# Jing-yilin/GAN-FFN

Hardware: AMD Instinct MI355X
Metric: utterances/sec per GAN train step, IEMOCAP tri-modal (higher is better)
Workload: dtype f32; 1 GPU; IEMOCAP tri-modal batch=32 per GPU fp32 on 1xMI355X, full G+D step (12 sub-steps: 6 train_disc + 6 train_gen, train-mode dropout, BCE, Adam); dialogues_per_gpu=32, seq_len=94, parallelism=dp1, launch=eager, streams=3, rccl_ranks=0, communicators=0

## Files before the change

gan_ffn_amd/_lib.py:

```python
import ctypes as C
import os

_HERE = os.path.dirname(os.path.abspath(__file__))
LIB_PATH = os.environ.get("GANFFN_LIB") or os.path.join(_HERE, "lib", "libganffn.so")


class EncCfg(C.Structure):
    _fields_ = [("S", C.c_int32), ("B", C.c_int32), ("E", C.c_int32), ("H", C.c_int32), ("F", C.c_int32),
                ("L", C.c_int32), ("p_pe", C.c_float), ("p_enc", C.c_float), ("ln_eps", C.c_float),
                ("train", C.c_int32)]


class LstmCfg(C.Structure):
    _fields_ = [("S", C.c_int32), ("B", C.c_int32), ("In", C.c_int32), ("H", C.c_int32)]


class LstmStackCfg(C.Structure):
    _fields_ = [("S", C.c_int32), ("B", C.c_int32), ("In", C.c_int32), ("H", C.c_int32), ("L", C.c_int32), ("p", C.c_float),
                ("train", C.c_int32)]


class HeadCfg(C.Structure):
    _fields_ = [("T", C.c_int32), ("E", C.c_int32), ("D1", C.c_int32), ("D2", C.c_int32), ("kind", C.c_int32),
                ("p", C.c_float), ("train", C.c_int32)]
# ... 45 lines not shown
SIGNATURES = {
    "ganffn_version": (_I, []),
    "ganffn_last_error": (C.c_char_p, []),
    "ganffn_layer_param_count": (_L, [_I, _I]),
    "ganffn_layer_param_offsets": (_I, [_I, _I, C.POINTER(C.c_int64)]),
    "ganffn_encoder_saved_floats": (_L, [_PE]),
    "ganffn_encoder_saved_hidden_offset": (_L, [_PE, _I]),
    "ganffn_encoder_workspace_floats": (_L, [_PE]),
    "ganffn_head_saved_floats": (_L, [_PH]),
    "ganffn_head_workspace_floats": (_L, [_PH]),
    "ganffn_rng_advance": (_I, [_P, _U64, _P]),
    "ganffn_pe_table": (_I, [_P, _I, _I, _P]),
    "ganffn_encoder_fwd": (_I, [_PE, _P, _P, _P, _P, _P, _P, _P, _U64, _P]),
    "ganffn_encoder_fwd_pair_supported": (_I, [_PE]),
    "ganffn_encoder_fwd_pair_workspace_floats": (_L, [_PE]),
    "ganffn_encoder_fwd_pair": (_I, [_PE, _P, _P, _P, _P, _P, _P, _P, _P, _U64, _P]),
    "ganffn_encoder_bwd": (_I, [_PE, _I, _I, _P, _P, _P, _P, _P, _P, _U64, _P]),
    "ganffn_encoder_bwd2": (_I, [_PE, _I, _I, _P, _P, _P, _P, _P, _P, _U64, _I, _P]),
    "ganffn_head_fwd": (_I, [_PH, _P, _P, _P, _P, _P, _P, _P, _P, _P, _P, _P, _U64, _P]),
    "ganffn_head_bwd": (_I, [_PH, _P, _P, _P, _P, _P, _P, _P, _P, _P, _P, _P, _P, _P, _P, _P, _U64, _P]),
    "ganffn_linear_fwd": (_I, [_P, _P, _P, _P, _I, _I, _I, _P]),
    "ganffn_linear_bwd_workspace_floats": (_L, [_I, _I, _I]),
    "ganffn_linear_bwd": (_I, [_P, _P, _P, _P, _P, _P, _I, _I, _I, _P, _L, _P]),
    "ganffn_bce_fwd": (_I, [_P, _F, _I, _F, _P, _I, _P]),
    "ganffn_bce_bwd": (_I, [_P, _F, _I, _F, _P, _P]),
    "ganffn_bce2_fwd": (_I, [_P, _F, _F, _I, _I, _I, _F, _P, _I, _P]),
    "ganffn_bce2_bwd": (_I, [_P, _F, _F, _I, _I, _I, _F, _P, _P]),
    "ganffn_adam_step": (_I, [_P, _P, _P, _P, _P, _L, _F, _F, _F, _F, _F, _F, _P]),
    "ganffn_lstm_saved_floats": (_L, [C.POINTER(LstmCfg)]),
    "ganffn_lstm_workspace_floats": (_L, [C.POINTER(LstmCfg)]),
    "ganffn_lstm_layer_fwd": (_I, [C.POINTER(LstmCfg), _P, _P, _P, _P, _P, _P, _P, _P, _P]),
    "ganffn_lstm_layer_bwd": (_I, [C.POINTER(LstmCfg), _P, _P, _P, _P, _P, _P, _P, _P, _P, _P, _P, _P, _P]),
    "ganffn_lstm_stack_saved_floats": (_L, [C.POINTER(LstmStackCfg)]),
    "ganffn_lstm_stack_workspace_floats": (_L, [C.POINTER(LstmStackCfg)]),
    "ganffn_lstm_stack_fwd": (_I, [C.POINTER(LstmStackCfg)] + [_P] * 9 + [_U64, _P]),
    "ganffn_lstm_stack_bwd": (_I, [C.POINTER(LstmStackCfg)] + [_P] * 13 + [_U64, _P]),
    "ganffn_lstm_batch_saved_floats": (_L, [C.POINTER(LstmCfg)]),
    "ganffn_lstm_batch_workspace_floats": (_L, [C.POINTER(LstmCfg)]),
    "ganffn_lstm_batch_layer_fwd": (_I, [C.POINTER(LstmCfg), _P, _P, _P, _P, _P, _P, _P, _P, _P]),
    "ganffn_lstm_batch_layer_bwd": (_I, [C.POINTER(LstmCfg), _P, _P, _P, _P, _P, _P, _P, _P, _P, _P, _P, _P, _P]),
    "ganffn_lstm_stack_batch_saved_floats": (_L, [C.POINTER(LstmStackCfg)]),
    "ganffn_lstm_stack_batch_workspace_floats": (_L, [C.POINTER(LstmStackCfg)]),
    "ganffn_lstm_stack_batch_fwd": (_I, [C.POINTER(LstmStackCfg)] + [_P] * 9 + [_U64, _P]),
    "ganffn_lstm_stack_batch_bwd": (_I, [C.POINTER(LstmStackCfg)] + [_P] * 13 + [_U64, _P]),
    "ganffn_meld_head_fwd": (_I, [_P, _P, _P, _P, _P, _P, _I, _I, _I, _P]),
    "ganffn_meld_head_bwd": (_I, [_P, _P, _P, _P, _P, _P, _P, _P, _P, _I, _I, _I, _P]),
    "ganffn_zero_floats": (_I, [_P, _L, _P]),
    "ganffn_adam_step_parts": (_I, [_P, _P, _P, _P, _P, _L, _F, _F, _F, _F, _F, _F, _P, _L, _I, _L, _L, _L, _P]),
    "ganffn_encoder_bwd_parts_supported": (_I, [_PE]),
    "ganffn_encoder_bwd_parts_covered": (_L, [_I, _I]),
    "ganffn_encoder_bwd_parts": (_I, [_PE, _P, _P, _P, _P, _P, _P, _U64, _I, C.POINTER(C.c_int64), C.POINTER(C.c_int64), C.POINTER(C.c_int), _P]),
    "ganffn_adam_update": (_I, [_P, _P, _P, _P, _P, _L, _F, _F, _F, _F, _F, _F, _P]),
    "ganffn_adam_bump": (_I, [_P, _P]),
    "ganffn_add3": (_I, [_P, _P, _P, _P, _L, _P]),
    "ganffn_logsoftmax_nll": (_I, [_P, _P, _P, _P, _P, _P, _P, _P, _I, _I, _I, _P]),
    "ganffn_gemm_nt": (_I, [_P, _P, _P, _P, _I, _I, _I, _P]),
    "ganffn_gemm_nn": (_I, [_P, _P, _P, _I, _I, _I, _P]),
    "ganffn_gemm_tn_acc": (_I, [_P, _P, _P, _P, _I, _I, _I, _P]),
    "ganffn_ffn_linear1_fwd": (_I, [_P, _P, _P, _P, _I, _I, _I, _F, _U32, _P, _U64, _I, _P]),
    "ganffn_gemm_tn_grouped_workspace_floats": (_L, []),
    "ganffn_gemm_tn_grouped": (_I, [_I, _P, _P, _P, _P, _P, _P, _P, _P, _L, _P]),
    "ganffn_attention_fwd": (_I, [_P, _P, _P, _I, _I, _I, _I, _F, _U32, _P, _U64, _P]),
    "ganffn_attention_bwd": (_I, [_P, _P, _P, _P, _P, _I, _I, _I, _I, _F, _U32, _P, _U64, _P]),
    "ganffn_gemm_hook": (_I, [_I, _I, _P, _P, _P, _P, _P, _L, _I, _I, _I, _F, _U32, _P, _U64, _I, _I, _P, _P]),
    "ganffn_ffn_k100_hook": (_I, [_I, _P, _P, _P, _P, _P, _P, _I, _F, _U32, _P, _U64, _I, _P]),
    "ganffn_attention_keep_words": (_L, [_I, _I]),
    "ganffn_attention_fwd_keep": (_I, [_P, _P, _P, _P, _I, _I, _I, _I, _F, _U32, _P, _U64, _P]),
    "ganffn_attention_bwd_keep": (_I, [_P, _P, _P, _P, _P, _P, _I, _I, _I, _I, _F, _U32, _P, _U64, _P]),
    "ganffn_add_dropout_layernorm_fwd": (_I, [_P, _P, _P, _P, _P, _P, _P, _I, _I, _F, _F, _U32, _P, _U64, _P]),
    "ganffn_add_dropout_layernorm_bwd": (_I, [_P, _P, _P, _P, _P, _P, _P, _P, _I, _I, _F, _U32, _P, _U64, _P]),
    "ganffn_general2_attention_fwd": (_I, [_P, _P, _P, _P, _P, _P, _I, _I, _I, _P]),
    "ganffn_general2_attention_bwd": (_I, [_P, _P, _P, _P, _P, _P, _P, _P, _P, _I, _I, _I, _P]),
    "ganffn_gemm_n100": (_I, [_P, _P, _I, _P, _P, _L, _I, _I, _I, C.POINTER(C.c_int), _P]),
    "ganffn_debug_set_ffn_mode": (_I, [_I]),
    "ganffn_drnn_skinny": (_I, [_I, _I, _P, _P, _P, _I, _I, _I, _P]),
    "ganffn_drnn_skinny_batch": (_I, [_I, _I, _P, _P, _P, _I, _I, _I, _P]),
    "ganffn_drnn_saved_floats": (_L, [C.POINTER(DrnnCfg)]),
    "ganffn_drnn_workspace_floats": (_L, [C.POINTER(DrnnCfg)]),
    "ganffn_drnn_fwd": (_I, [C.POINTER(DrnnCfg), _I, _P, _P, _P, _P, _P, _P, _P, _P, _P, _U64, _P]),
    "ganffn_drnn_bwd": (_I, [C.POINTER(DrnnCfg), _I, _P, _P, _P, _P, _P, _P, _P, _P, _P, _P, _P, _U64, _P]),
    "ganffn_drnn_listener_saved_floats": (_L, [C.POINTER(DrnnCfg)]),
    "ganffn_drnn_listener_workspace_floats": (_L, [C.POINTER(DrnnCfg)]),
    "ganffn_drnn_listener_fwd": (_I, [C.POINTER(DrnnCfg), _I, _P, _P, _P, _P, _P, _P, _P, _P, _P, _P, _U64, _P]),
    "ganffn_drnn_listener_bwd": (_I, [C.POINTER(DrnnCfg), _I, _P, _P, _P, _P, _P, _P, _P, _P, _P, _P, _P, _P, _P, _U64, _P]),
    "ganffn_drnn_att_saved_floats": (_L, [C.POINTER(DrnnCfg), C.POINTER(DrnnAtt), _I]),
    "ganffn_drnn_att_workspace_floats": (_L, [C.POINTER(DrnnCfg), C.POINTER(DrnnAtt), _I]),
    "ganffn_drnn_att_fwd": (_I, [C.POINTER(DrnnCfg), C.POINTER(DrnnAtt), _I] + [_P] * 11 + [_U64, _P]),
    "ganffn_drnn_att_bwd": (_I, [C.POINTER(DrnnCfg), C.POINTER(DrnnAtt), _I] + [_P] * 15 + [_U64, _P]),
    "ganffn_drnn_party_saved_floats": (_L, [C.POINTER(DrnnCfg), C.POINTER(DrnnAtt), _I, _I]),
    "ganffn_drnn_party_workspace_floats": (_L, [C.POINTER(DrnnCfg), C.POINTER(DrnnAtt), _I, _I]),
    "ganffn_drnn_party_fwd": (_I, [C.POINTER(DrnnCfg), C.POINTER(DrnnAtt), _I, _I] + [_P] * 11 + [_U64, _P]),
    "ganffn_drnn_party_bwd": (_I, [C.POINTER(DrnnCfg), C.POINTER(DrnnAtt), _I, _I] + [_P] * 15 + [_U64, _P]),
    "ganffn_drnn_batch_saved_floats": (_L, [C.POINTER(DrnnCfg), C.POINTER(DrnnAtt), _I, _I]),
    "ganffn_drnn_batch_workspace_floats": (_L, [C.POINTER(DrnnCfg), C.POINTER(DrnnAtt), _I, _I]),
    "ganffn_drnn_batch_fwd": (_I, [C.POINTER(DrnnCfg), C.POINTER(DrnnAtt), _I, _I] + [_P] * 11 + [_U64, _P]),
    "ganffn_drnn_batch_bwd": (_I, [C.POINTER(DrnnCfg), C.POINTER(DrnnAtt), _I, _I] + [_P] * 15 + [_U64, _P]),
    "ganffn_dropout": (_I, [_P, _P, _I, _I, _F, _U32, _P, _U64, _P]),
    "ganffn_seq_reverse": (_I, [_P, _P, _P, _I, _I, _I, _I, _P]),
    "ganffn_drnn_join_fwd": (_I, [_P, _P, _P, _P, _I, _I, _I, _F, _U32, _U32, _P, _U64, _I, _P]),
    "ganffn_drnn_join_bwd": (_I, [_P, _P, _P, _P, _I, _I, _I, _F, _U32, _U32, _P, _U64, _I, _P]),
    "ganffn_mask_pos_inplace": (_I, [_P, _P, _F, _L, _P]),
    "ganffn_batch_gather": (_I, [_P, _I, _P, _P, _L, _P, _P, _P, _I, _I, _I, _P]),
    "ganffn_epoch_record": (_I, [_P, _P, _P, _P, _I, _I, _I, _P, _P, _P, _L, _L, _P, _P, _I, _I, _P]),
}

_lib = None
# ... 35 lines not shown
```

gan_ffn_amd/csrc/api.hip:

```cpp
#include "common.h"

#include <string.h>

namespace ganffn {

static thread_local char g_err[512] = "";
char* err_buf() { return g_err; }
int fail(int code, const char* fmt, ...) {
    va_list ap;
    va_start(ap, fmt);
    vsnprintf(g_err, sizeof(g_err), fmt, ap);
    va_end(ap);
    return code;
}

int launch_gelu_bwd_drop(const float* d, const float* u, float* out, int R, int C, float p, uint32_t site,
                         const uint64_t* rng, uint64_t add, int train, hipStream_t st);
int launch_disc_tail_fwd(const float* a2, const float* w3, const float* b3, float* prob, int T, int D2, float p,
                         const uint64_t* rng, uint64_t add, int train, hipStream_t st);
int launch_disc_tail_bwd(const float* dprob, const float* prob, const float* a2, const float* u2, const float* w3,
                         float* d_pre2, float* gw3, float* gb3, int T, int D2, float p, const uint64_t* rng, uint64_t add,
                         int train, hipStream_t st, float* gpart);
int launch_disc_tail_reduce(const float* gpart, int nblk_, int D2, float* gw3, float* gb3, hipStream_t st);
bool disc_head_fused_supported(int E, int D1, int D2);
// ... 304 lines not shown
            ea.bias = P + lo.out_b;
            int osplits = md.outproj_nosplit() ? 1 : gemm_splitk_factor(T, E, E);
            const GemmSeg1 g1{s1v + so.attn_o, tmp1, nullptr, train};
            GF_TRY(launch_gemm_nt_pair(sv0 + so.attn_o, E, P + lo.out_w, E, tmp0, E, T, E, E, EPI_NONE, ea, g1, st, &osplits, TE));
            const LnFwdSeg1 n1{X1, tmp1, s1v + so.x1, s1v + so.xhat1, s1v + so.rstd1, train};
            GF_TRY(launch_add_drop_ln_fwd(X0, tmp0, P + lo.n1w, P + lo.n1b, sv0 + so.x1, sv0 + so.xhat1, sv0 + so.rstd1, T, E, c->ln_eps,
                                          c->p_enc, site + 1, rng, add, 0, st, osplits, TE, &n1));
        }
        int splits = 1;
        {
            EpiArgs e1;
            e1.bias = P + lo.b1; e1.p = c->p_enc; e1.site = site + 2; e1.rng = rng; e1.rng_add = add; e1.train = 0;
            const GemmSeg1 g1{s1v + so.x1, s1v + so.h, reinterpret_cast<uint16_t*>(s1v + so.hmask), train};
            GF_TRY(launch_gemm_nt_pair(sv0 + so.x1, E, P + lo.w1, E, sv0 + so.h, F, T, F, E, EPI_RELU_DROP, e1, g1, st));
            if (n100_supported(E, F) && !md.n100_off()) {
                splits = MAX_SPLITS;
                GF_TRY(launch_gemm_n100(sv0 + so.h, F, P + lo.w2, F, 0, P + lo.b2, tmp0, TE, T, F, &splits, st, s1v + so.h, tmp1));
            } else {
                ea.bias = P + lo.b2;
                splits = gemm_splitk_factor(T, E, F);
                const GemmSeg1 g2{s1v + so.h, tmp1, nullptr, train};
                GF_TRY(launch_gemm_nt_pair(sv0 + so.h, F, P + lo.w2, F, tmp0, E, T, E, F, EPI_NONE, ea, g2, st, &splits, TE));
            }
        }
        if (rc) {
            const float* Pn = (l + 1 < L) ? P + lo.total : nullptr;
            RcFwdSeg1 s1{};
            s1.y = tmp1; s1.x = s1v + so.x1; s1.out = Xn1; s1.xhat = s1v + so.xhat2; s1.rstd = s1v + so.rstd2;
            s1.post_out = Pn ? sv1(l + 1) + so.qkv : nullptr; s1.train = train;
            GF_TRY(launch_rc_ln_inproj_fwd(tmp0, splits, TE, sv0 + so.x1, P + lo.n2w, P + lo.n2b, Xn0, sv0 + so.xhat2, sv0 + so.rstd2,
                                           Pn ? Pn + lo.in_w : nullptr, Pn ? Pn + lo.in_b : nullptr, Pn ? sv0 + so.qkv : nullptr, T,
                                           c->ln_eps, c->p_enc, site + 3, rng, add, 0, st, &s1));
        } else {
            const LnFwdSeg1 n2{s1v + so.x1, tmp1, Xn1, s1v + so.xhat2, s1v + so.rstd2, train};
            GF_TRY(launch_add_drop_ln_fwd(sv0 + so.x1, tmp0, P + lo.n2w, P + lo.n2b, Xn0, sv0 + so.xhat2, sv0 + so.rstd2, T, E, c->ln_eps,
                                          c->p_enc, site + 3, rng, add, 0, st, splits, TE, &n2));
        }
        X0 = Xn0;
        X1 = Xn1;
    }
    return 0;
}

extern "C" int ganffn_encoder_bwd2(const ganffn_enc_cfg* c, int layer_lo, int layer_hi, float* dx, const float* params,
                                   float* grads, const float* saved, float* workspace, const uint64_t* rng, uint64_t add,
                                   int need_dx_in, void* stream);
extern "C" int ganffn_encoder_bwd(const ganffn_enc_cfg* c, int layer_lo, int layer_hi, float* dx, const float* params,
                                  float* grads, const float* saved, float* workspace, const uint64_t* rng, uint64_t add,
                                  void* stream) {
    return ganffn_encoder_bwd2(c, layer_lo, layer_hi, dx, params, grads, saved, workspace, rng, add, 1, stream);
}
static int encoder_bwd_impl(const ganffn_enc_cfg* c, int layer_lo, int layer_hi, float* dx, const float* params,
                            float* grads, const float* saved, float* workspace, const uint64_t* rng, uint64_t add,
                            int need_dx_in, void* stream, TnSlabs* slabs);
extern "C" int ganffn_encoder_bwd2(const ganffn_enc_cfg* c, int layer_lo, int layer_hi, float* dx, const float* params,
                                   float* grads, const float* saved, float* workspace, const uint64_t* rng, uint64_t add,
                                   int need_dx_in, void* stream) {
    return encoder_bwd_impl(c, layer_lo, layer_hi, dx, params, grads, saved, workspace, rng, add, need_dx_in, stream, nullptr);
}
static bool bwd_parts_supported(const ganffn_enc_cfg* c, const Mode md) {
    return rc_supported(c->E) && !md.rc_off() && !md.tn100_off() && !md.tn100_in_kernel_sum() && !md.adam_slabs_off() && c->F == 2048 &&
           4 * c->L <= 40;
}
extern "C" int ganffn_encoder_bwd_parts_supported(const ganffn_enc_cfg* c) {
    if (check_cfg(c) != 0) return -1;
    return bwd_parts_supported(c, mode()) ? 1 : 0;
}
extern "C" int64_t ganffn_encoder_bwd_parts_covered(int E, int F) { return layer_off(E, F).n1w; }
extern "C" int ganffn_encoder_bwd_parts(const ganffn_enc_cfg* c, float* dx, const float* params, float* grads, const float* saved,
                                        float* workspace, const uint64_t* rng, uint64_t add, int need_dx_in, int64_t* part_offset,
                                        int64_t* part_stride, int* n_parts, void* stream) {
    GF_TRY(check_cfg(c));
    GF_CHECK_ARG(grads && part_offset && part_stride && n_parts, "encoder_bwd_parts: null pointer");
    GF_CHECK_ARG(bwd_parts_supported(c, mode()), "encoder_bwd_parts: this stack's weight gradients are reduced in the launch (ask ganffn_encoder_bwd_parts_supported)");
    TnSlabs sl{grads, (long)c->L * layer_off(c->E, c->F).total, 1, nullptr, 0};
    GF_TRY(encoder_bwd_impl(c, 0, c->L, dx, params, grads, saved, workspace, rng, add, need_dx_in, stream, &sl));
    *n_parts = sl.n_parts;
    *part_offset = sl.part ? sl.part - workspace : 0;
    *part_stride = sl.part_stride;
    return 0;
}
static int encoder_bwd_impl(const ganffn_enc_cfg* c, int layer_lo, int layer_hi, float* dx, const float* params,
                            float* grads, const float* saved, float* workspace, const uint64_t* rng, uint64_t add,
                            int need_dx_in, void* stream, TnSlabs* slabs) {
    const Mode md = mode();
    GF_TRY(check_cfg(c));
    GF_CHECK_ARG(dx && params && saved && workspace, "encoder_bwd: null pointer");
    GF_CHECK_ARG(0 <= layer_lo && layer_lo < layer_hi && layer_hi <= c->L, "encoder_bwd: bad layer range [%d,%d)", layer_lo, layer_hi);
    GF_CHECK_ARG(aligned16(dx) && aligned16(params) && aligned16(saved) && aligned16(workspace) && (!grads || aligned16(grads)),
                 "encoder_bwd: buffers must be 16-byte aligned");
    const bool drop = c->train && (c->p_pe > 0.f || c->p_enc > 0.f);
    GF_CHECK_ARG(!drop || rng, "encoder_bwd: rng required in train mode");
    hipStream_t st = (hipStream_t)stream;
    const int S = c->S, B = c->B, E = c->E, H = c->H, F = c->F, T = S * B;
    const int64_t TE = (int64_t)T * E, TF = (int64_t)T * F;
    const LayerOff lo = layer_off(E, F);
    const SavedOff so = saved_off(c);
    const int train = c->train;
    const float pdrop = (train ? c->p_enc : 0.f);

    const int64_t SET = TF + 5 * TE;
    float* set0 = workspace;
    float* dz2 = set0 + (int64_t)c->L * SET;
    float* dz1 = dz2 + TE;
    float* d_attn = dz1 + TE;
    float* tmp = d_attn + TE;
    float* lnp0 = tmp + (int64_t)MAX_SPLITS * TE;
    const int64_t LNP = ln_part_floats(c);
    float* tnp = lnp0 + (int64_t)c->L * 2 * LNP;
    tnp = reinterpret_cast<float*>((reinterpret_cast<uintptr_t>(tnp) + 15) & ~(uintptr_t)15);
    const bool rc = rc_supported(E) && !md.rc_off();
    float* rcw = reinterpret_cast<float*>((reinterpret_cast<uintptr_t>(tnp + gemm_tn_grouped_part_floats()) + 15) & ~(uintptr_t)15);
    const int64_t RCW = rc_pack_floats();
    if (rc) GF_TRY(launch_rc_pack(params + (int64_t)layer_lo * lo.total, lo.total, lo.in_w, lo.out_w, rcw, layer_hi - layer_lo, st));
    const int lnblk = rc ? rc_blocks(T) : ln_bwd_blocks(T);
    TnDesc tn[40];
    int ntn = 0;
    float* r_gw[2 * 64]; float* r_gb[2 * 64]; const float* r_part[2 * 64]; int r_nb[2 * 64];
    int nred = 0;

    const float* dxin = dx;
    int dxin_slabs = 1;
    for (int l = layer_hi - 1; l >= layer_lo; --l) {
        const float* P = params + (int64_t)l * lo.total;
        float* G = grads ? grads + (int64_t)l * lo.total : nullptr;
        const float* sv = saved + so.layers + (int64_t)l * so.per_layer;
        const float* Xl = saved + so.X + (int64_t)l * TE;
        const uint32_t site = SITE_LAYER0 + 4 * l;
        float* bs = set0 + (int64_t)(l - layer_lo) * SET;
        float* dh = bs;
        float* dyA = dh + TF;
        float* dyB = dyA + TE;
        float* d_qkv = dyB + TE;
        float* lnp2 = lnp0 + (int64_t)(2 * (l - layer_lo)) * LNP;
        float* lnp1 = lnp2 + LNP;
        EpiArgs none;
        if (rc) {
            if (l == layer_hi - 1)
                GF_TRY(launch_rc_ln_bwd(nullptr, nullptr, dx, 1, 0, nullptr, sv + so.xhat2, sv + so.rstd2, P + lo.n2w, dz2, dyA,
                                        G ? lnp2 : nullptr, nullptr, nullptr, T, c->p_enc, site + 3, rng, add, train, st));
            else
                GF_TRY(launch_rc_ln_bwd(bs + SET + TF + 2 * TE, rcw + (int64_t)(l + 1 - layer_lo) * RCW, nullptr, 0, 0, dz1,
                                        sv + so.xhat2, sv + so.rstd2, P + lo.n2w, dz2, dyA, G ? lnp2 : nullptr, nullptr, nullptr, T,
                                        c->p_enc, site + 3, rng, add, train, st));
        } else {
            GF_TRY(launch_add_drop_ln_bwd(dxin, sv + so.xhat2, sv + so.rstd2, P + lo.n2w, dz2, dyA, G ? G + lo.n2w : nullptr,
                                          G ? G + lo.n2b : nullptr, T, E, c->p_enc, site + 3, rng, add, train, st, dxin_slabs, TE,
                                          nullptr, G ? lnp2 : nullptr));
        }
        if (G) { r_gw[nred] = G + lo.n2w; r_gb[nred] = G + lo.n2b; r_part[nred] = lnp2; r_nb[nred] = lnblk; ++nred; }
        if (G) tn[ntn++] = TnDesc{dyA, E, sv + so.h, F, G + lo.w2, F, G + lo.b2, E, F, T};
        const float mscale = (pdrop > 0.f) ? 1.0f / (1.0f - pdrop) : 1.0f;
        int splits = 1;
        {
            EpiArgs em;
            em.aux_in = sv + so.h;
            em.mscale = mscale;
            if (!md.mask_float()) em.mask_in = reinterpret_cast<const uint16_t*>(sv + so.hmask);
            GF_TRY(launch_gemm_nn(dyA, E, P + lo.w2, F, dh, F, T, F, E, EPI_MASK_POS, em, st));
        }
        if (G) tn[ntn++] = TnDesc{dh, F, sv + so.x1, E, G + lo.w1, E, G + lo.b1, F, E, T};
        {
            if (n100_supported(E, F) && !md.n100_off()) {
                splits = MAX_SPLITS;
                GF_TRY(launch_gemm_n100(dh, F, P + lo.w1, E, 1, nullptr, tmp, TE, T, F, &splits, st));
            } else {
                splits = gemm_splitk_factor(T, E, F);
                GF_TRY(launch_gemm_nn(dh, F, P + lo.w1, E, tmp, E, T, E, F, EPI_NONE, none, st, &splits, TE));
            }
        }
        if (rc) {
            GF_TRY(launch_rc_ln_bwd(nullptr, nullptr, tmp, splits, TE, dz2, sv + so.xhat1, sv + so.rstd1, P + lo.n1w, dz1, dyB,
                                    G ? lnp1 : nullptr, rcw + (int64_t)(l - layer_lo) * RCW + 3 * (int64_t)E * E, d_attn, T, c->p_enc,
                                    site + 1, rng, add, train, st));
        } else {
            GF_TRY(launch_add_drop_ln_bwd(tmp, sv + so.xhat1, sv + so.rstd1, P + lo.n1w, dz1, dyB, G ? G + lo.n1w : nullptr,
                                          G ? G + lo.n1b : nullptr, T, E, c->p_enc, site + 1, rng, add, train, st, splits, TE, dz2,
                                          G ? lnp1 : nullptr));
        }
        if (G) { r_gw[nred] = G + lo.n1w; r_gb[nred] = G + lo.n1b; r_part[nred] = lnp1; r_nb[nred] = lnblk; ++nred; }
        if (G) tn[ntn++] = TnDesc{dyB, E, sv + so.attn_o, E, G + lo.out_w, E, G + lo.out_b, E, E, T};
        if (!rc) GF_TRY(launch_gemm_nn(dyB, E, P + lo.out_w, E, d_attn, E, T, E, E, EPI_NONE, none, st));
        GF_TRY(launch_attention_bwd(sv + so.qkv, sv + so.attn_o, sv + so.lse, d_attn, reinterpret_cast<const uint32_t*>(sv + so.keep), d_qkv, S, B, E,
                                    H, c->p_enc, site + 0, rng, add, train, st));
        if (G) tn[ntn++] = TnDesc{d_qkv, 3 * E, Xl, E, G + lo.in_w, E, G + lo.in_b, 3 * E, E, T};
        if (ntn == 40 || (l == layer_lo && ntn > 0)) {
            GF_TRY(launch_gemm_tn_grouped(tn, ntn, st, tnp, gemm_tn_grouped_part_floats(), slabs));
            ntn = 0;
        }
        EpiArgs eadd;
        eadd.aux_in = dz1;
        if (l > layer_lo && rc) {
        } else if (l > layer_lo) {
            int sp = inproj_dgrad_splits(T, E);
            GF_TRY(launch_gemm_nn(d_qkv, 3 * E, P + lo.in_w, E, tmp, E, T, E, 3 * E, EPI_NONE, eadd, st, &sp, TE));
            dxin = tmp;
            dxin_slabs = sp;
        } else if (layer_lo > 0 || need_dx_in) {
            GF_TRY(launch_gemm_nn(d_qkv, 3 * E, P + lo.in_w, E, dx, E, T, E, 3 * E, EPI_NONE, eadd, st));
        }
    }
    if (nred > 0) GF_TRY(launch_ln_param_reduce(nred, r_gw, r_gb, r_part, r_nb, E, st, slabs != nullptr));
    if (layer_lo == 0 && need_dx_in) GF_TRY(launch_dropout_bwd_inplace(dx, T, E, c->p_pe, SITE_PE, rng, add, train, st));
    return 0;
}

static int check_head(const ganffn_head_cfg* c) {
    GF_CHECK_ARG(c, "null head cfg");
    GF_CHECK_ARG(c->T >= 1 && c->E >= 4 && (c->E & 3) == 0, "head: bad T=%d E=%d", c->T, c->E);
    GF_CHECK_ARG(c->D1 >= 4 && (c->D1 & 3) == 0 && c->D2 >= 4 && (c->D2 & 3) == 0, "head: D1=%d D2=%d must be multiples of 4", c->D1, c->D2);
    GF_CHECK_ARG(c->kind == 0 || c->kind == 1, "head: kind=%d", c->kind);
    GF_CHECK_ARG(c->kind == 0 || c->D2 <= 32, "disc head: D2=%d > 32", c->D2);
    GF_CHECK_ARG(c->p >= 0.f && c->p < 1.f, "head: p out of [0,1)");
    return 0;
}
extern "C" int64_t ganffn_head_saved_floats(const ganffn_head_cfg* c) {
    if (check_head(c) != 0) return -1;
    const int64_t T = c->T, T4 = (T + 3) & ~int64_t(3);
    int64_t n = T * c->E + 2 * T * c->D1 + T * c->D2;
    if (c->kind == 1) n += T * c->D2 + T4;
    return n;
}
static int64_t head_part2(const ganffn_head_cfg* c) { return a4(gemm_tn_part_floats(c->D2, c->D1, c->T)); }
static int64_t head_part1(const ganffn_head_cfg* c) { return a4(gemm_tn_part_floats(c->D1, c->E, c->T)); }
extern "C" int64_t ganffn_head_workspace_floats(const ganffn_head_cfg* c) {
    if (check_head(c) != 0) return -1;
    const int64_t T = c->T;
    const int64_t tail_blocks = disc_head_blocks((int)T) > (T + 255) / 256 ? disc_head_blocks((int)T) : (T + 255) / 256;
    return a4(T * c->D1) + a4(T * c->D2) + head_part2(c) + head_part1(c) + tail_blocks * 36 + 64;
}

extern "C" int ganffn_head_fwd(const ganffn_head_cfg* c, const float* x, const float* w1, const float* b1, const float* w2,
                               const float* b2, const float* w3, const float* b3, float* out, float* saved, float* workspace,
                               const uint64_t* rng, uint64_t add, void* stream) {
    GF_TRY(check_head(c));
    const Mode md = mode();
    GF_CHECK_ARG(x && w1 && b1 && w2 && b2 && out && saved, "head_fwd: null pointer");
    GF_CHECK_ARG(c->kind == 0 || (w3 && b3), "head_fwd: disc needs fc3");
    GF_CHECK_ARG(!(c->train && c->p > 0.f) || rng, "head_fwd: rng required in train mode");
    hipStream_t st = (hipStream_t)stream;
    const int T = c->T, E = c->E, D1 = c->D1, D2 = c->D2, train = c->train;
    float* s0 = saved;
    float* u1 = s0 + (int64_t)T * E;
    float* a1 = u1 + (int64_t)T * D1;
    float* u2 = a1 + (int64_t)T * D1;
    EpiArgs e;
    e.p = c->p; e.rng = rng; e.rng_add = add; e.train = train;
    if (c->kind == 0) {
        GF_TRY(launch_gelu_drop_fwd(x, s0, T, E, c->p, SITE_HEAD0, rng, add, train, st));
        e.bias = b1; e.site = SITE_HEAD1; e.aux_out = u1;
        GF_TRY(launch_gemm_nt(s0, E, w1, E, a1, D1, T, D1, E, EPI_DROP_GELU, e, st));
        e.bias = b2; e.site = SITE_HEAD2; e.aux_out = u2;
        GF_TRY(launch_gemm_nt(a1, D1, w2, D1, out, D2, T, D2, D1, EPI_DROP_GELU, e, st));
    } else if (disc_head_fused_supported(E, D1, D2) && !md.dhead_off()) {
        float* a2 = u2 + (int64_t)T * D2;
        float* prob = a2 + (int64_t)T * D2;
        GF_TRY(launch_disc_head_fwd(x, w1, b1, w2, b2, w3, b3, s0, u1, a1, u2, a2, prob, out, T, c->p, rng, add, train, st));
    } else {
        float* a2 = u2 + (int64_t)T * D2;
        float* prob = a2 + (int64_t)T * D2;
        GF_TRY(launch_gelu_drop_fwd(x, s0, T, E, 0.f, SITE_HEAD0, rng, add, 0, st));
        e.bias = b1; e.site = SITE_HEAD1; e.aux_out = u1;
        GF_TRY(launch_gemm_nt(s0, E, w1, E, a1, D1, T, D1, E, EPI_DROP_GELU, e, st));
        e.bias = b2; e.site = SITE_HEAD2; e.aux_out = u2;
        GF_TRY(launch_gemm_nt(a1, D1, w2, D1, a2, D2, T, D2, D1, EPI_DROP_GELU, e, st));
        GF_TRY(launch_disc_tail_fwd(a2, w3, b3, prob, T, D2, c->p, rng, add, train, st));
        hipError_t er = hipMemcpyAsync(out, prob, (size_t)T * sizeof(float), hipMemcpyDeviceToDevice, st);
        if (er != hipSuccess) return fail((int)er, "head_fwd: memcpy failed");
    }
    (void)workspace;
    return 0;
}

extern "C" int ganffn_head_bwd(const ganffn_head_cfg* c, const float* d_out, const float* x, const float* w1, const float* w2,
                               const float* w3, float* gw1, float* gb1, float* gw2, float* gb2, float* gw3, float* gb3,
                               float* dx, const float* saved, float* workspace, const uint64_t* rng, uint64_t add,
                               void* stream) {
    GF_TRY(check_head(c));
    const Mode md = mode();
    GF_CHECK_ARG(d_out && x && w1 && w2 && dx && saved && workspace, "head_bwd: null pointer");
    GF_CHECK_ARG(aligned16(workspace), "head_bwd: workspace must be 16-byte aligned");
    GF_CHECK_ARG(c->kind == 0 || w3, "head_bwd: disc needs fc3");
    GF_CHECK_ARG(!(c->train && c->p > 0.f) || rng, "head_bwd: rng required in train mode");
    hipStream_t st = (hipStream_t)stream;
    const int T = c->T, E = c->E, D1 = c->D1, D2 = c->D2, train = c->train;
    const float* s0 = saved;
    const float* u1 = s0 + (int64_t)T * E;
    const float* a1 = u1 + (int64_t)T * D1;
    const float* u2 = a1 + (int64_t)T * D1;
    float* d_pre1 = workspace;
    float* d_pre2 = d_pre1 + a4((int64_t)T * D1);
    float* part2 = d_pre2 + a4((int64_t)T * D2);
    float* part1 = part2 + head_part2(c);
    float* tailp = part1 + head_part1(c);
    if (c->kind == 1 && disc_head_fused_supported(E, D1, D2) && !md.dhead_off()) {
        const float* a2 = u2 + (int64_t)T * D2;
        const float* prob = a2 + (int64_t)T * D2;
        GF_TRY(launch_disc_head_bwd(d_out, x, w1, w2, w3, u1, u2, a2, prob, dx, gw1 ? d_pre1 : nullptr, gw2 ? d_pre2 : nullptr,
                                    gw3 ? tailp : nullptr, T, c->p, rng, add, train, st));
        if (gw3) GF_TRY(launch_disc_tail_reduce(tailp, disc_head_blocks(T), D2, gw3, gb3, st));
        if (gw2) GF_TRY(launch_gemm_tn_acc(d_pre2, D2, a1, D1, gw2, D1, gb2, D2, D1, T, st, part2, head_part2(c)));
        if (gw1) GF_TRY(launch_gemm_tn_acc(d_pre1, D1, s0, E, gw1, E, gb1, D1, E, T, st, part1, head_part1(c)));
        return 0;
    }
    if (c->kind == 0) {
        GF_TRY(launch_gelu_bwd_drop(d_out, u2, d_pre2, T, D2, c->p, SITE_HEAD2, rng, add, train, st));
    } else {
        const float* a2 = u2 + (int64_t)T * D2;
        const float* prob = a2 + (int64_t)T * D2;
        GF_TRY(launch_disc_tail_bwd(d_out, prob, a2, u2, w3, d_pre2, gw3, gb3, T, D2, c->p, rng, add, train, st, tailp));
    }
    if (gw2) GF_TRY(launch_gemm_tn_acc(d_pre2, D2, a1, D1, gw2, D1, gb2, D2, D1, T, st, part2, head_part2(c)));
    EpiArgs e;
    e.p = c->p; e.rng = rng; e.rng_add = add; e.train = train;
    e.aux_in = u1; e.site = SITE_HEAD1;
    GF_TRY(launch_gemm_nn(d_pre2, D2, w2, D1, d_pre1, D1, T, D1, D2, EPI_GELU_BWD_DROP, e, st));
    if (gw1) GF_TRY(launch_gemm_tn_acc(d_pre1, D1, s0, E, gw1, E, gb1, D1, E, T, st, part1, head_part1(c)));
    e.aux_in = x;
    if (c->kind == 0) {
        e.site = SITE_HEAD0;
        GF_TRY(launch_gemm_nn(d_pre1, D1, w1, E, dx, E, T, E, D1, EPI_GELU_BWD_DROP, e, st));
    } else {
        GF_TRY(launch_gemm_nn(d_pre1, D1, w1, E, dx, E, T, E, D1, EPI_GELU_BWD, e, st));
    }
    return 0;
}
// ... 138 lines not shown
```

gan_ffn_amd/csrc/common.h:

```cpp
#pragma once
#include <hip/hip_runtime.h>
#include <stdint.h>
#include <stdio.h>
#include <stdarg.h>
#include <atomic>

#include "../../include/ganffn.h"

#ifdef GANFFN_LAB
#define GF_LAB_ONLY(...) __VA_ARGS__
#else
#define GF_LAB_ONLY(...)
#endif

namespace ganffn {

struct Mode {
    uint32_t bits;
    bool rc_off() const { return bits & 2u; }
    bool n100_off() const { return bits & 4u; }
    bool tn100_off() const { return bits & 8u; }
    bool tn100_in_kernel_sum() const { return bits & 16u; }
    bool dhead_off() const { return bits & 32u; }
    bool pe_off() const { return bits & 64u; }
// ... 148 lines not shown
}

__device__ __forceinline__ float gelu_f(float x) {
    return 0.5f * x * (1.0f + erff(x * 0.70710678118654752440f));
}
__device__ __forceinline__ float gelu_grad_f(float x) {
    const float cdf = 0.5f * (1.0f + erff(x * 0.70710678118654752440f));
    const float pdf = 0.39894228040143267794f * __expf(-0.5f * x * x);
    return cdf + x * pdf;
}

__device__ __forceinline__ float wave_sum(float v) {
#pragma unroll
    for (int o = 32; o > 0; o >>= 1) v += __shfl_xor(v, o, 64);
    return v;
}
__device__ __forceinline__ float wave_max(float v) {
#pragma unroll
    for (int o = 32; o > 0; o >>= 1) v = fmaxf(v, __shfl_xor(v, o, 64));
    return v;
}

enum Epilogue : int {
    EPI_NONE = 0,
    EPI_RELU_DROP = 1,
    EPI_DROP_GELU = 2,
    EPI_MASK_POS = 3,
    EPI_GELU_BWD_DROP = 4,
    EPI_GELU_BWD = 5,
    EPI_GELU_BWD_DROP0 = 6
};

struct EpiArgs {
    const float* bias = nullptr;
    float* aux_out = nullptr;
    const float* aux_in = nullptr;
    float mscale = 1.f;
    uint16_t* mask_out = nullptr;
    const uint16_t* mask_in = nullptr;
    float p = 0.f;
    uint32_t site = 0;
    const uint64_t* rng = nullptr;
    uint64_t rng_add = 0;
    int train = 0;
};

inline long epi_mask_words(long M, long N) { return ((M + 31) / 32) * N * 2; }

int launch_gemm_nt(const float* A, int lda, const float* W, int ldw, float* C, int ldc, int M, int N, int K,
                   int epi, const EpiArgs& ea, hipStream_t st, int* splits_io = nullptr, long slab_stride = 0);
int gemm_splitk_factor(int M, int N, int K);
struct GemmSeg1 {
    const float* A; float* C; uint16_t* mask_out; int train;
};
int launch_gemm_nt_pair(const float* A, int lda, const float* W, int ldw, float* C, int ldc, int M, int N, int K, int epi,
                        const EpiArgs& ea, const GemmSeg1& s1, hipStream_t st, int* splits_io = nullptr, long slab_stride = 0);
int launch_gemm_nn(const float* A, int lda, const float* Bm, int ldb, float* C, int ldc, int M, int N, int K,
                   int epi, const EpiArgs& ea, hipStream_t st, int* splits_io = nullptr, long slab_stride = 0);
long gemm_tn_part_floats(int M, int N, int K);
int launch_gemm_tn_acc(const float* At, int lda, const float* Bm, int ldb, float* C, int ldc, float* colsum,
                       int M, int N, int K, hipStream_t st, float* part_ws = nullptr, long part_floats = 0);

struct SkinnyProb {
    const float* A; int lda;
    const float* W; int ldw;
    const float* Cin; int ldcin;
    const float* Cin2;
    const float* bias;
    float* C; int ldc;
    int M, N, K;
};
struct SkinnyGroup {
    SkinnyProb p[8];
};
int launch_skinny(const SkinnyGroup& grp, int nprob, bool nn, hipStream_t st);

struct TnDesc {
    const float* At; int lda;
    const float* B; int ldb;
    float* C; int ldc;
    float* colsum;
    int M, N, K;
};
struct TnSlabs {
    float* grad_base; long range_floats;
    int n_parts; float* part; long part_stride;
};
int launch_gemm_tn_grouped(const TnDesc* d, int n, hipStream_t st, float* part_ws = nullptr, long part_floats = 0, TnSlabs* slabs = nullptr);
bool tn100_supported(const TnDesc* d, int n);
int launch_gemm_tn100_grouped(const TnDesc* d, int n, hipStream_t st, float* part_ws, long part_floats, TnSlabs* slabs = nullptr);
long gemm_tn_grouped_part_floats();

constexpr int ATTN_KEEP_WORDS = 28 * 16;
struct AttnFwdSeg1 {
    const float* qkv; float* o; float* lse; uint32_t* keep; int train;
};
int launch_attention_fwd(const float* qkv, float* o, float* lse, uint32_t* keep, int S, int B, int E, int H, float p, uint32_t site,
                         const uint64_t* rng, uint64_t add, int train, hipStream_t st, const AttnFwdSeg1* seg1 = nullptr);
int launch_attention_bwd(const float* qkv, const float* o, const float* lse, const float* d_o, const uint32_t* keep, float* d_qkv,
                         int S, int B, int E, int H, float p, uint32_t site, const uint64_t* rng, uint64_t add, int train,
                         hipStream_t st);
bool attn16_supported(int E, int H, int S);
int launch_attn16_fwd(const float* qkv, float* o, float* lse, uint32_t* keepw, int S, int B, int E, int H, float p, uint32_t site,
                      const uint64_t* rng, uint64_t add, int train, hipStream_t st, const AttnFwdSeg1* seg1 = nullptr);
int launch_attn16_bwd(const float* qkv, const float* o, const float* lse, const float* d_o, const uint32_t* keepw, float* d_qkv,
                      int S, int B, int E, int H, float p, uint32_t site, const uint64_t* rng, uint64_t add, int train,
                      hipStream_t st);

int launch_pe_dropout(const float* x, const float* pe, float* out, int S, int B, int E, float p,
                      const uint64_t* rng, uint64_t add, int train, hipStream_t st, float* out1 = nullptr, int train1 = 0);
int launch_dropout_bwd_inplace(float* dx, int R, int C, float p, uint32_t site, const uint64_t* rng, uint64_t add,
                               int train, hipStream_t st);
int launch_dropout(const float* x, float* out, int R, int C, float p, uint32_t site, const uint64_t* rng,
                   uint64_t add, int train, hipStream_t st);
struct LnFwdSeg1 {
    const float* x; const float* y; float* out; float* xhat; float* rstd; int train;
};
int launch_add_drop_ln_fwd(const float* x, const float* y, const float* w, const float* b, float* out, float* xhat,
                           float* rstd, int T, int E, float eps, float p, uint32_t site, const uint64_t* rng,
                           uint64_t add, int train, hipStream_t st, int nslab = 1, long slab_stride = 0,
                           const LnFwdSeg1* s1 = nullptr);
int ln_bwd_blocks(int T);
int launch_add_drop_ln_bwd(const float* d_out, const float* xhat, const float* rstd, const float* w, float* dz,
                           float* dy, float* gw, float* gb, int T, int E, float p, uint32_t site,
                           const uint64_t* rng, uint64_t add, int train, hipStream_t st, int nslab = 1,
                           long slab_stride = 0, const float* addend = nullptr, float* gpart = nullptr);
int launch_ln_param_reduce(int n, float* const* gw, float* const* gb, const float* const* part, const int* nblk, int E,
                           hipStream_t st, bool overwrite = false);
int launch_add_inplace(float* a, const float* b, int64_t n, hipStream_t st);

bool n100_supported(int N, int K);
int n100_splits(int T, int K, int max_splits, int w_kmajor);
int launch_gemm_n100(const float* A, int lda, const float* W, int ldw, int w_kmajor, const float* bias, float* C, long slab_stride,
                     int T, int K, int* splits_io, hipStream_t st, const float* A1 = nullptr, float* C1 = nullptr);

bool rc_supported(int E);
long rc_pack_floats();
int rc_blocks(int T);
int launch_rc_pack(const float* params, long layer_stride, long off_in, long off_out, float* wt, int nl, hipStream_t st);
struct RcFwdSeg1 {
    const float* pre_a; const float* y; const float* x;
    float* out; float* xhat; float* rstd; float* post_out;
    int train;
};
int launch_rc_outproj_ln_fwd(const float* attn_o, const float* wo, const float* bo, const float* x, const float* gamma,
                             const float* beta, float* out, float* xhat, float* rstd, int T, float eps, float p, uint32_t site,
                             const uint64_t* rng, uint64_t add, int train, hipStream_t st, const RcFwdSeg1* s1 = nullptr);
int launch_rc_pe_inproj_fwd(const float* x_in, const float* pe, float* out, const float* w_in, const float* b_in, float* qkv, int T,
                            int B, float p, const uint64_t* rng, uint64_t add, int train, hipStream_t st,
                            const RcFwdSeg1* s1 = nullptr);
int launch_rc_ln_inproj_fwd(const float* y, int nslab, long slab_stride, const float* x, const float* gamma, const float* beta,
                            float* out, float* xhat, float* rstd, const float* w_in, const float* b_in, float* qkv, int T,
                            float eps, float p, uint32_t site, const uint64_t* rng, uint64_t add, int train, hipStream_t st,
                            const RcFwdSeg1* s1 = nullptr);
int launch_rc_ln_bwd(const float* d_qkv, const float* w_in_t, const float* d_out, int nslab, long slab_stride, const float* addend,
                     const float* xhat, const float* rstd, const float* gamma, float* dz, float* dy, float* gpart,
                     const float* wo_t, float* d_attn, int T, float p, uint32_t site, const uint64_t* rng, uint64_t add, int train,
                     hipStream_t st);
int launch_gelu_drop_fwd(const float* x, float* out, int R, int C, float p, uint32_t site, const uint64_t* rng,
                         uint64_t add, int train, hipStream_t st);

}
```

gan_ffn_amd/csrc/elementwise.hip:

```cpp
#include "common.h"

#pragma clang fp contract(off)

namespace ganffn {

template <bool PAIR>
__global__ void pe_dropout_kernel(const float* __restrict__ x, const float* __restrict__ pe, float* __restrict__ out,
                                  int T, int B, int E, float p, const uint64_t* __restrict__ rng, uint64_t add,
                                  int train, float* out1, int train1, int nb0) {
    const int G = (T + 3) >> 2;
    int bid = blockIdx.x;
    if constexpr (PAIR) {
        if (bid >= nb0) {
            bid -= nb0;
            out = out1; train = train1;
        }
    }
    const long idx = (long)bid * blockDim.x + threadIdx.x;
    if (idx >= (long)G * E) return;
    const int rg = (int)(idx / E), c = (int)(idx - (long)rg * E);
    const DropCtx dc = make_drop(rng, add, SITE_PE, p, train);
    float mult[4];
    drop_mult4(dc, (uint32_t)rg, (uint32_t)E, (uint32_t)c, mult);
#pragma unroll
    for (int q = 0; q < 4; ++q) {
        const int t = rg * 4 + q;
        if (t < T) {
            const int s = t / B;
            out[(size_t)t * E + c] = (x[(size_t)t * E + c] + pe[(size_t)s * E + c]) * mult[q];
        }
    }
}

template <int MODE>
__global__ void drop_kernel(const float* __restrict__ x, const float* __restrict__ u, float* __restrict__ out, int R,
                            int C, float p, uint32_t site, const uint64_t* __restrict__ rng, uint64_t add, int train) {
    const int G = (R + 3) >> 2;
    const long idx = (long)blockIdx.x * blockDim.x + threadIdx.x;
    if (idx >= (long)G * C) return;
    const int rg = (int)(idx / C), c = (int)(idx - (long)rg * C);
    const DropCtx dc = make_drop(rng, add, site, p, train);
    float mult[4];
    drop_mult4(dc, (uint32_t)rg, (uint32_t)C, (uint32_t)c, mult);
#pragma unroll
    for (int q = 0; q < 4; ++q) {
        const int t = rg * 4 + q;
        if (t < R) {
            const size_t o = (size_t)t * C + c;
            float v = x[o];
            if (MODE == 1) v = gelu_f(v);
            if (MODE == 2) v = v * gelu_grad_f(u[o]);
            out[o] = v * mult[q];
        }
    }
}

__global__ void add_inplace_kernel(float* __restrict__ a, const float* __restrict__ b, long n4) {
    const long i = (long)blockIdx.x * blockDim.x + threadIdx.x;
    if (i >= n4) return;
    float4 x = reinterpret_cast<float4*>(a)[i];
    const float4 y = reinterpret_cast<const float4*>(b)[i];
    x.x += y.x; x.y += y.y; x.z += y.z; x.w += y.w;
    reinterpret_cast<float4*>(a)[i] = x;
}

__global__ void add3_kernel(const float* __restrict__ a, const float* __restrict__ b, const float* __restrict__ c,
                            float* __restrict__ o, long n) {
    const long i = (long)blockIdx.x * blockDim.x + threadIdx.x;
    if (i < n) o[i] = a[i] + b[i] + c[i];
}

constexpr int LN_MAXC = 10;
constexpr int LN_MAXSLAB = 16;

template <int NC, int NSB, bool PAIR = false>
__global__ __launch_bounds__(256) void add_drop_ln_fwd_kernel(const float* __restrict__ x, const float* __restrict__ y,
                                                              const float* __restrict__ w, const float* __restrict__ b,
                                                              float* __restrict__ out, float* __restrict__ xhat,
                                                              float* __restrict__ rstd, int T, int E, float eps, float p,
                                                              uint32_t site, const uint64_t* __restrict__ rng,
                                                              uint64_t add, int train, int nslab, long slab_stride, LnFwdSeg1 s1,
                                                              int nb0) {
    const int lane = threadIdx.x & 63;
    int bid = blockIdx.x;
    if constexpr (PAIR) {
        if (bid >= nb0) {
            bid -= nb0;
            x = s1.x; y = s1.y; out = s1.out; xhat = s1.xhat; rstd = s1.rstd; train = s1.train;
        }
    }
    const int rg = bid * 4 + (threadIdx.x >> 6);
    if (rg * 4 >= T) return;
    const DropCtx dc = make_drop(rng, add, site, p, train);
    size_t off[NC][4];
    bool okc[NC], okr[4];
#pragma unroll
    for (int q = 0; q < 4; ++q) okr[q] = rg * 4 + q < T;
#pragma unroll
    for (int k = 0; k < NC; ++k) {
        const int c = lane + 64 * k;
        okc[k] = c < E;
#pragma unroll
        for (int q = 0; q < 4; ++q) off[k][q] = (size_t)min(rg * 4 + q, T - 1) * E + min(c, E - 1);
    }
    float xv[NC][4], yy[NC][4];
#pragma unroll
    for (int k = 0; k < NC; ++k)
// ... 249 lines not shown
            a = a2[o];
            d_pre2[o] = dpre3 * w3[k] * gelu_grad_f(u2[o]) * drop_mult1(d2, (uint32_t)t, (uint32_t)D2, (uint32_t)k);
        }
        if (gw3) {
            const float s = wave_sum(dpre3 * a);
            if (lane == 0) red[wv][k] = s;
        }
    }
    if (gw3) {
        const float s = wave_sum(dpre3);
        if (lane == 0) red[wv][32] = s;
        __syncthreads();
        if (threadIdx.x < D2) gpart[blockIdx.x * 36 + threadIdx.x] = red[0][threadIdx.x] + red[1][threadIdx.x] + red[2][threadIdx.x] + red[3][threadIdx.x];
        if (threadIdx.x == 32) gpart[blockIdx.x * 36 + 32] = red[0][32] + red[1][32] + red[2][32] + red[3][32];
    }
}
__global__ __launch_bounds__(1024) void disc_tail_reduce_kernel(const float* __restrict__ gpart, int nblk, int D2, float* __restrict__ gw3,
                                                                float* __restrict__ gb3) {
    const int lane = threadIdx.x & 63, w = threadIdx.x >> 6;
    for (int k = w; k <= D2; k += 16) {
        const int slot = k < D2 ? k : 32;
        float s = 0.f;
        for (int b = lane; b < nblk; b += 64) s += gpart[b * 36 + slot];
        s = wave_sum(s);
        if (lane == 0) {
            if (k < D2) gw3[k] += s; else gb3[0] += s;
        }
    }
}

__global__ __launch_bounds__(1024) void bce_fwd_kernel(const float* __restrict__ prob, float target_a, float target_b,
                                                       int period, int split, int n, float scale, float* __restrict__ loss,
                                                       int accumulate) {
    __shared__ float red[16];
    float s = 0.f;
    for (int i = threadIdx.x; i < n; i += 1024) {
        const float target = (period > 0 && (i % period) >= split) ? target_b : target_a;
        const float p = prob[i];
        const float lp = fmaxf(logf(p), -100.f);
        const float l1p = fmaxf(logf(1.0f - p), -100.f);
        s -= target * lp + (1.0f - target) * l1p;
    }
    s = wave_sum(s);
    if ((threadIdx.x & 63) == 0) red[threadIdx.x >> 6] = s;
    __syncthreads();
    if (threadIdx.x == 0) {
        float t = 0.f;
        for (int w = 0; w < 16; ++w) t += red[w];
        t = t * scale / (float)n;
        loss[0] = accumulate ? loss[0] + t : t;
    }
}

__global__ void bce_bwd_kernel(const float* __restrict__ prob, float target_a, float target_b, int period, int split, int n,
                               float scale, float* __restrict__ dprob) {
    const int i = blockIdx.x * blockDim.x + threadIdx.x;
    if (i >= n) return;
    const float target = (period > 0 && (i % period) >= split) ? target_b : target_a;
    const float p = prob[i];
    dprob[i] = scale / (float)n * (p - target) / fmaxf(p * (1.0f - p), 1e-12f);
}

__device__ __forceinline__ void adam_one(float& pi, float gi, float& mi, float& vi, float lr_bc1, float rs_bc2, float b1,
                                         float b2, float eps, float wd, float gscale) {
    gi *= gscale;
    if (wd != 0.f) gi += wd * pi;
    mi = b1 * mi + (1.0f - b1) * gi;
    vi = b2 * vi + (1.0f - b2) * gi * gi;
    const float denom = sqrtf(vi) / rs_bc2 + eps;
    pi = pi - lr_bc1 * (mi / denom);
}

constexpr int ADAM_MAX_EXTRA = 7;
template <int VEC>
__global__ __launch_bounds__(256) void adam_kernel(float* __restrict__ p, const float* __restrict__ g, float* __restrict__ m,
                                                   float* __restrict__ v, const int32_t* __restrict__ step, long n, float lr,
                                                   float b1, float b2, float eps, float wd, float gscale) {
    const long i = ((long)blockIdx.x * blockDim.x + threadIdx.x) * VEC;
    if (i >= n) return;
    const float t = (float)(*step + 1);
    const float bc1 = 1.0f - powf(b1, t);
    const float bc2 = 1.0f - powf(b2, t);
    const float lr_bc1 = lr / bc1, rs_bc2 = sqrtf(bc2);
    if (VEC == 4) {
        float4 pp = *reinterpret_cast<float4*>(p + i), mm = *reinterpret_cast<float4*>(m + i), vv = *reinterpret_cast<float4*>(v + i);
        const float4 gg = *reinterpret_cast<const float4*>(g + i);
        adam_one(pp.x, gg.x, mm.x, vv.x, lr_bc1, rs_bc2, b1, b2, eps, wd, gscale);
        adam_one(pp.y, gg.y, mm.y, vv.y, lr_bc1, rs_bc2, b1, b2, eps, wd, gscale);
        adam_one(pp.z, gg.z, mm.z, vv.z, lr_bc1, rs_bc2, b1, b2, eps, wd, gscale);
        adam_one(pp.w, gg.w, mm.w, vv.w, lr_bc1, rs_bc2, b1, b2, eps, wd, gscale);
        *reinterpret_cast<float4*>(m + i) = mm;
        *reinterpret_cast<float4*>(v + i) = vv;
        *reinterpret_cast<float4*>(p + i) = pp;
    } else {
        float pi = p[i], mi = m[i], vi = v[i];
        adam_one(pi, g[i], mi, vi, lr_bc1, rs_bc2, b1, b2, eps, wd, gscale);
        m[i] = mi; v[i] = vi; p[i] = pi;
    }
}
__global__ __launch_bounds__(256) void adam_parts_kernel(float* __restrict__ p, const float* __restrict__ g, float* __restrict__ m,
                                                         float* __restrict__ v, const int32_t* __restrict__ step, long n, float lr,
                                                         float b1, float b2, float eps, float wd, float gscale,
                                                         const float* __restrict__ part, long part_stride, int n_extra,
                                                         long enc_floats, long layer_floats, long covered) {
    const long i = ((long)blockIdx.x * blockDim.x + threadIdx.x) * 4;
    if (i >= n) return;
    const float t = (float)(*step + 1);
    const float bc1 = 1.0f - powf(b1, t);
    const float bc2 = 1.0f - powf(b2, t);
    const float lr_bc1 = lr / bc1, rs_bc2 = sqrtf(bc2);
    float4 pp = *reinterpret_cast<float4*>(p + i), mm = *reinterpret_cast<float4*>(m + i), vv = *reinterpret_cast<float4*>(v + i);
    float4 gg = *reinterpret_cast<const float4*>(g + i);
    const bool cov = i < enc_floats && (i % layer_floats) < covered;
    if (cov) {
        float4 e[ADAM_MAX_EXTRA];
#pragma unroll
        for (int z = 0; z < ADAM_MAX_EXTRA; ++z) e[z] = *reinterpret_cast<const float4*>(part + (size_t)min(z, n_extra - 1) * part_stride + i);
#pragma unroll
        for (int z = 0; z < ADAM_MAX_EXTRA; ++z)
            if (z < n_extra) { gg.x += e[z].x; gg.y += e[z].y; gg.z += e[z].z; gg.w += e[z].w; }
    }
    adam_one(pp.x, gg.x, mm.x, vv.x, lr_bc1, rs_bc2, b1, b2, eps, wd, gscale);
    adam_one(pp.y, gg.y, mm.y, vv.y, lr_bc1, rs_bc2, b1, b2, eps, wd, gscale);
    adam_one(pp.z, gg.z, mm.z, vv.z, lr_bc1, rs_bc2, b1, b2, eps, wd, gscale);
    adam_one(pp.w, gg.w, mm.w, vv.w, lr_bc1, rs_bc2, b1, b2, eps, wd, gscale);
    *reinterpret_cast<float4*>(m + i) = mm;
    *reinterpret_cast<float4*>(v + i) = vv;
    *reinterpret_cast<float4*>(p + i) = pp;
}
__global__ void adam_step_inc(int32_t* step) { *step += 1; }

__global__ void rng_advance_kernel(uint64_t* rng, uint64_t delta) { rng[1] += delta; }

__global__ void pe_table_kernel(float* __restrict__ pe, int max_len, int E) {
    const int idx = blockIdx.x * blockDim.x + threadIdx.x;
    if (idx >= max_len * (E / 2)) return;
    const int pos = idx / (E / 2), i = idx % (E / 2);
    const float c = (float)(-9.210340371976184 / (double)E);
    const float div = expf((float)(2 * i) * c);
    const float a = (float)pos * div;
    pe[(size_t)pos * E + 2 * i] = sinf(a);
    pe[(size_t)pos * E + 2 * i + 1] = cosf(a);
}

__global__ __launch_bounds__(1024) void logsoftmax_nll_kernel(const float* __restrict__ logits, const int64_t* __restrict__ labels,
                                                              const float* __restrict__ umask, const float* __restrict__ cw,
                                                              float* __restrict__ logp, float* __restrict__ acc2, int S, int B,
                                                              int C) {
    __shared__ float red[2][16];
    float num = 0.f, den = 0.f;
    for (int t = threadIdx.x; t < S * B; t += 1024) {
        const int s = t / B, b = t - s * B;
        const float* x = logits + (size_t)t * C;
        float m = x[0];
        for (int c = 1; c < C; ++c) m = fmaxf(m, x[c]);
        float sum = 0.f;
        for (int c = 0; c < C; ++c) sum += expf(x[c] - m);
        const float ls = logf(sum);
        for (int c = 0; c < C; ++c) logp[(size_t)t * C + c] = (x[c] - m) - ls;
        if (labels) {
// ... 69 lines not shown
            a[u] = dy[(size_t)t * N + n];
            b[u] = x[(size_t)t * K + kc];
        }
#pragma unroll
        for (int u = 0; u < 8; ++u) {
            const float m = (t0 + 16 * u < T) ? 1.f : 0.f;
            acc += m * a[u] * b[u];
            accb += m * a[u];
        }
    }
    red[g][kl] = acc;
    if (kl == 0) red[g][64] = accb;
    __syncthreads();
    if (g == 0) {
        float sw = 0.f;
#pragma unroll
        for (int i = 0; i < 16; ++i) sw += red[i][kl];
        if (k < K) gw[(size_t)n * K + k] += sw;
        if (gb && kl == 0 && blockIdx.y == 0) {
            float sb = 0.f;
#pragma unroll
            for (int i = 0; i < 16; ++i) sb += red[i][64];
            gb[n] += sb;
        }
    }
}

static inline int nblk(long n, int bs) { return (int)((n + bs - 1) / bs); }

int launch_pe_dropout(const float* x, const float* pe, float* out, int S, int B, int E, float p,
                      const uint64_t* rng, uint64_t add, int train, hipStream_t st, float* out1, int train1) {
    const int T = S * B;
    const long n = (long)((T + 3) / 4) * E;
    const int nb = nblk(n, 256);
    if (out1) hipLaunchKernelGGL(pe_dropout_kernel<true>, dim3(2 * nb), dim3(256), 0, st, x, pe, out, T, B, E, p, rng, add, train, out1, train1, nb);
    else hipLaunchKernelGGL(pe_dropout_kernel<false>, dim3(nb), dim3(256), 0, st, x, pe, out, T, B, E, p, rng, add, train, (float*)nullptr, 0, 0);
    GF_LAUNCH_CHECK();
    return 0;
}

int launch_dropout(const float* x, float* out, int R, int C, float p, uint32_t site, const uint64_t* rng,
                   uint64_t add, int train, hipStream_t st) {
    const long n = (long)((R + 3) / 4) * C;
    hipLaunchKernelGGL(drop_kernel<0>, dim3(nblk(n, 256)), dim3(256), 0, st, x, (const float*)nullptr, out, R, C, p, site, rng, add, train);
    GF_LAUNCH_CHECK();
    return 0;
}
int launch_dropout_bwd_inplace(float* dx, int R, int C, float p, uint32_t site, const uint64_t* rng, uint64_t add,
                               int train, hipStream_t st) {
    if (!(train && p > 0.f)) return 0;
    return launch_dropout(dx, dx, R, C, p, site, rng, add, train, st);
}
int launch_gelu_drop_fwd(const float* x, float* out, int R, int C, float p, uint32_t site, const uint64_t* rng,
                         uint64_t add, int train, hipStream_t st) {
    const long n = (long)((R + 3) / 4) * C;
    hipLaunchKernelGGL(drop_kernel<1>, dim3(nblk(n, 256)), dim3(256), 0, st, x, (const float*)nullptr, out, R, C, p, site, rng, add, train);
    GF_LAUNCH_CHECK();
    return 0;
}
int launch_gelu_bwd_drop(const float* d, const float* u, float* out, int R, int C, float p, uint32_t site,
                         const uint64_t* rng, uint64_t add, int train, hipStream_t st) {
    const long n = (long)((R + 3) / 4) * C;
    hipLaunchKernelGGL(drop_kernel<2>, dim3(nblk(n, 256)), dim3(256), 0, st, d, u, out, R, C, p, site, rng, add, train);
    GF_LAUNCH_CHECK();
    return 0;
}

int launch_add_inplace(float* a, const float* b, int64_t n, hipStream_t st) {
    GF_CHECK_ARG((n & 3) == 0 && aligned16(a) && aligned16(b), "add_inplace: n %% 4 and 16-byte alignment required");
    hipLaunchKernelGGL(add_inplace_kernel, dim3(nblk(n / 4, 256)), dim3(256), 0, st, a, b, (long)(n / 4));
    GF_LAUNCH_CHECK();
    return 0;
}

int launch_add_drop_ln_fwd(const float* x, const float* y, const float* w, const float* b, float* out, float* xhat,
                           float* rstd, int T, int E, float eps, float p, uint32_t site, const uint64_t* rng,
                           uint64_t add, int train, hipStream_t st, int nslab, long slab_stride, const LnFwdSeg1* s1) {
    GF_CHECK_ARG(E <= 64 * LN_MAXC, "layernorm: E=%d > %d", E, 64 * LN_MAXC);
    GF_CHECK_ARG(nslab >= 1 && nslab <= LN_MAXSLAB, "layernorm: nslab=%d out of [1,%d]", nslab, LN_MAXSLAB);
    GF_CHECK_ARG(!s1 || (s1->x && s1->y && s1->out), "layernorm: bad second segment");
    const int G = (T + 3) / 4;
    const dim3 grid((G + 3) / 4), grid2(2 * ((G + 3) / 4)), blk(256);
#define GF_LN_FWD(NC, NSB)                                                                                              \
    do {                                                                                                                \
        if (s1) hipLaunchKernelGGL((add_drop_ln_fwd_kernel<NC, NSB, true>), grid2, blk, 0, st, x, y, w, b, out, xhat, rstd, T, E, eps, \
                                   p, site, rng, add, train, nslab, slab_stride, *s1, (int)grid.x);                      \
        else hipLaunchKernelGGL((add_drop_ln_fwd_kernel<NC, NSB>), grid, blk, 0, st, x, y, w, b, out, xhat, rstd, T, E, eps, p, \
                                site, rng, add, train, nslab, slab_stride, LnFwdSeg1{}, 0);                              \
    } while (0)
    if (E <= 64) GF_LN_FWD(1, 8);
    else if (E <= 128) GF_LN_FWD(2, 8);
    else if (E <= 256) GF_LN_FWD(4, 4);
    else if (E <= 320) GF_LN_FWD(5, 4);
    else if (E <= 512) GF_LN_FWD(8, 2);
    else GF_LN_FWD(10, 2);
#undef GF_LN_FWD
    GF_LAUNCH_CHECK();
    return 0;
}

int ln_bwd_blocks(int T) {
    int blocks = ((T + 3) / 4 + 3) / 4;
    return blocks > 256 ? 256 : blocks;
}

int launch_add_drop_ln_bwd(const float* d_out, const float* xhat, const float* rstd, const float* w, float* dz,
                           float* dy, float* gw, float* gb, int T, int E, float p, uint32_t site,
                           const uint64_t* rng, uint64_t add, int train, hipStream_t st, int nslab, long slab_stride,
// ... 74 lines not shown
    }
    if (gw) {
        hipLaunchKernelGGL(small_linear_dw_kernel, dim3(N, (K + 63) / 64), dim3(1024), 0, st, dy, x, gw, gb, T, K, N);
        GF_LAUNCH_CHECK();
    }
    return 0;
}

}

using namespace ganffn;

extern "C" int ganffn_rng_advance(uint64_t* rng, uint64_t delta, void* stream) {
    GF_CHECK_ARG(rng, "rng_advance: null rng");
    hipLaunchKernelGGL(rng_advance_kernel, dim3(1), dim3(1), 0, (hipStream_t)stream, rng, delta);
    GF_LAUNCH_CHECK();
    return 0;
}

extern "C" int ganffn_pe_table(float* pe, int max_len, int E, void* stream) {
    GF_CHECK_ARG(pe && max_len > 0 && E > 0 && (E & 1) == 0, "pe_table: E must be even (model.py:1187-1188)");
    const int n = max_len * (E / 2);
    hipLaunchKernelGGL(pe_table_kernel, dim3((n + 255) / 256), dim3(256), 0, (hipStream_t)stream, pe, max_len, E);
    GF_LAUNCH_CHECK();
    return 0;
}

extern "C" int ganffn_bce_fwd(const float* prob, float target, int n, float scale, float* loss_out, int accumulate,
                              void* stream) {
    return ganffn_bce2_fwd(prob, target, target, 0, 0, n, scale, loss_out, accumulate, stream);
}
extern "C" int ganffn_bce_bwd(const float* prob, float target, int n, float scale, float* dprob, void* stream) {
    return ganffn_bce2_bwd(prob, target, target, 0, 0, n, scale, dprob, stream);
}

extern "C" int ganffn_bce2_fwd(const float* prob, float target_a, float target_b, int period, int split, int n, float scale,
                               float* loss_out, int accumulate, void* stream) {
    GF_CHECK_ARG(prob && loss_out && n > 0 && period >= 0 && split >= 0, "bce_fwd: bad arguments");
    hipStream_t st = (hipStream_t)stream;
    hipLaunchKernelGGL(bce_fwd_kernel, dim3(1), dim3(1024), 0, st, prob, target_a, target_b, period, split, n, scale, loss_out,
                       accumulate);
    GF_LAUNCH_CHECK();
    return 0;
}

extern "C" int ganffn_bce2_bwd(const float* prob, float target_a, float target_b, int period, int split, int n, float scale,
                               float* dprob, void* stream) {
    GF_CHECK_ARG(prob && dprob && n > 0 && period >= 0 && split >= 0, "bce_bwd: bad arguments");
    hipLaunchKernelGGL(bce_bwd_kernel, dim3((n + 255) / 256), dim3(256), 0, (hipStream_t)stream, prob, target_a, target_b, period, split, n, scale, dprob);
    GF_LAUNCH_CHECK();
    return 0;
}

extern "C" int ganffn_adam_bump(int32_t* step, void* stream) {
    GF_CHECK_ARG(step, "adam_bump: null step");
    hipLaunchKernelGGL(adam_step_inc, dim3(1), dim3(1), 0, (hipStream_t)stream, step);
    GF_LAUNCH_CHECK();
    return 0;
}

extern "C" int ganffn_adam_step(float* params, const float* grads, float* exp_avg, float* exp_avg_sq, int32_t* step,
                                int64_t n, float lr, float beta1, float beta2, float eps, float weight_decay,
                                float grad_scale, void* stream) {
    GF_TRY(ganffn_adam_update(params, grads, exp_avg, exp_avg_sq, step, n, lr, beta1, beta2, eps, weight_decay, grad_scale, stream));
    return ganffn_adam_bump(step, stream);
}

extern "C" int ganffn_adam_update(float* params, const float* grads, float* exp_avg, float* exp_avg_sq, const int32_t* step,
                                  int64_t n, float lr, float beta1, float beta2, float eps, float weight_decay,
                                  float grad_scale, void* stream) {
    GF_CHECK_ARG(params && grads && exp_avg && exp_avg_sq && step && n > 0, "adam_update: bad arguments");
    hipStream_t st = (hipStream_t)stream;
    const bool vec = aligned16(params) && aligned16(grads) && aligned16(exp_avg) && aligned16(exp_avg_sq);
    const long n4 = vec ? ((long)n & ~3L) : 0;
    if (n4 > 0) {
        hipLaunchKernelGGL(adam_kernel<4>, dim3((unsigned)((n4 / 4 + 255) / 256)), dim3(256), 0, st, params, grads, exp_avg,
                           exp_avg_sq, (const int32_t*)step, n4, lr, beta1, beta2, eps, weight_decay, grad_scale);
        GF_LAUNCH_CHECK();
    }
    if (n4 < n) {
        hipLaunchKernelGGL(adam_kernel<1>, dim3((unsigned)((n - n4 + 255) / 256)), dim3(256), 0, st, params + n4, grads + n4,
                           exp_avg + n4, exp_avg_sq + n4, (const int32_t*)step, (long)n - n4, lr, beta1, beta2, eps,
                           weight_decay, grad_scale);
        GF_LAUNCH_CHECK();
    }
    return 0;
}

extern "C" int ganffn_adam_step_parts(float* params, const float* grads, float* exp_avg, float* exp_avg_sq, int32_t* step, int64_t n,
                                      float lr, float beta1, float beta2, float eps, float weight_decay, float grad_scale,
                                      const float* parts, int64_t part_stride, int n_parts, int64_t enc_floats, int64_t layer_floats,
                                      int64_t covered_per_layer, void* stream) {
    GF_CHECK_ARG(params && grads && exp_avg && exp_avg_sq && step && n > 0, "adam_step_parts: bad arguments");
    GF_CHECK_ARG(n_parts >= 1 && n_parts <= ADAM_MAX_EXTRA + 1, "adam_step_parts: n_parts=%d out of [1,%d]", n_parts, ADAM_MAX_EXTRA + 1);
    if (n_parts == 1) return ganffn_adam_step(params, grads, exp_avg, exp_avg_sq, step, n, lr, beta1, beta2, eps, weight_decay, grad_scale, stream);
    GF_CHECK_ARG(parts && aligned16(parts) && (part_stride & 3) == 0 && part_stride >= enc_floats, "adam_step_parts: bad partial slabs");
    GF_CHECK_ARG((n & 3) == 0 && aligned16(params) && aligned16(grads) && aligned16(exp_avg) && aligned16(exp_avg_sq),
                 "adam_step_parts: slabs must be 16-byte aligned and a multiple of 4 floats");
    GF_CHECK_ARG(layer_floats > 0 && (layer_floats & 3) == 0 && (covered_per_layer & 3) == 0 && covered_per_layer <= layer_floats &&
                     enc_floats % layer_floats == 0 && enc_floats <= n, "adam_step_parts: bad layer geometry");
    hipStream_t st = (hipStream_t)stream;
    hipLaunchKernelGGL(adam_parts_kernel, dim3((unsigned)((n / 4 + 255) / 256)), dim3(256), 0, st, params, grads, exp_avg, exp_avg_sq,
                       (const int32_t*)step, (long)n, lr, beta1, beta2, eps, weight_decay, grad_scale, parts, (long)part_stride,
                       n_parts - 1, (long)enc_floats, (long)layer_floats, (long)covered_per_layer);
    GF_LAUNCH_CHECK();
    return ganffn_adam_bump(step, stream);
}

extern "C" int ganffn_add3(const float* a, const float* b, const float* c, float* out, int64_t n, void* stream) {
    GF_CHECK_ARG(a && b && c && out && n > 0, "add3: bad arguments");
    hipLaunchKernelGGL(add3_kernel, dim3((unsigned)((n + 255) / 256)), dim3(256), 0, (hipStream_t)stream, a, b, c, out, (long)n);
    GF_LAUNCH_CHECK();
    return 0;
}

extern "C" int ganffn_logsoftmax_nll(const float* logits, const int64_t* labels, const float* umask, const float* class_w,
                                     float* log_prob, float* loss_out, float* dlogits, float* workspace2, int S, int B, int C,
                                     void* stream) {
    GF_CHECK_ARG(logits && log_prob && S > 0 && B > 0 && C > 0, "logsoftmax_nll: bad arguments");
    GF_CHECK_ARG(!labels || (umask && loss_out && workspace2), "logsoftmax_nll: labels need umask, loss_out, workspace2");
    hipStream_t st = (hipStream_t)stream;
    const int T = S * B;
    hipLaunchKernelGGL(logsoftmax_nll_kernel, dim3(1), dim3(1024), 0, st, logits, labels, umask, class_w, log_prob,
                       workspace2, S, B, C);
    GF_LAUNCH_CHECK();
    if (labels) {
        hipLaunchKernelGGL(nll_finish_kernel, dim3(1), dim3(1), 0, st, (const float*)workspace2, loss_out);
        GF_LAUNCH_CHECK();
        if (dlogits) {
            hipLaunchKernelGGL(nll_bwd_kernel, dim3((T + 255) / 256), dim3(256), 0, st, (const float*)log_prob, labels, umask,
                               class_w, (const float*)workspace2, dlogits, S, B, C);
            GF_LAUNCH_CHECK();
        }
    }
    return 0;
}

extern "C" int ganffn_dropout(const float* x, float* out, int R, int C, float p, uint32_t site, const uint64_t* rng,
                              uint64_t rng_offset_add, void* stream) {
    GF_CHECK_ARG(x && out && R > 0 && C > 0, "dropout: bad arguments");
    GF_CHECK_ARG(p <= 0.f || rng, "dropout: rng required");
    return launch_dropout(x, out, R, C, p, site, rng, rng_offset_add, 1, (hipStream_t)stream);
}

extern "C" int ganffn_add_dropout_layernorm_fwd(const float* x, const float* y, const float* w, const float* b, float* out,
                                                float* xhat, float* rstd, int T, int E, float eps, float p, uint32_t site,
                                                const uint64_t* rng, uint64_t rng_offset_add, void* stream) {
    GF_CHECK_ARG(x && y && w && b && out && T > 0 && E > 0, "add_dropout_layernorm_fwd: bad arguments");
    GF_CHECK_ARG(p <= 0.f || rng, "add_dropout_layernorm_fwd: rng required");
    return launch_add_drop_ln_fwd(x, y, w, b, out, xhat, rstd, T, E, eps, p, site, rng, rng_offset_add, 1, (hipStream_t)stream);
}

extern "C" int ganffn_add_dropout_layernorm_bwd(const float* d_out, const float* xhat, const float* rstd, const float* w,
                                                float* dz, float* dy, float* gw, float* gb, int T, int E, float p,
                                                uint32_t site, const uint64_t* rng, uint64_t rng_offset_add, void* stream) {
    GF_CHECK_ARG(d_out && xhat && rstd && w && dz && T > 0 && E > 0, "add_dropout_layernorm_bwd: bad arguments");
    GF_CHECK_ARG(p <= 0.f || rng, "add_dropout_layernorm_bwd: rng required");
    return launch_add_drop_ln_bwd(d_out, xhat, rstd, w, dz, dy, gw, gb, T, E, p, site, rng, rng_offset_add, 1,
                                  (hipStream_t)stream, 1, 0, nullptr, nullptr);
// ... 2 lines not shown
```

gan_ffn_amd/csrc/gemm.hip:

```cpp
#include "common.h"

#include <type_traits>

namespace ganffn {

typedef float floatx16 __attribute__((ext_vector_type(16)));

__device__ __forceinline__ uint32_t v_bit_to_mask(uint32_t word, int bit) {
    uint32_t r;
    asm("v_bfe_i32 %0, %1, %2, 1" : "=v"(r) : "v"(word), "n"(bit));
    return r;
}
__device__ __forceinline__ uint32_t v_and_keep(uint32_t a, uint32_t b) {
    uint32_t r;
    asm("v_and_b32 %0, %1, %2" : "=v"(r) : "v"(a), "v"(b));
    return r;
}
__device__ __forceinline__ uint32_t v_nonzero_bit_or(uint32_t x, int bit, uint32_t acc) {
    uint32_t t, r;
    asm("v_min_u32 %0, 1, %1" : "=v"(t) : "v"(x));
    asm("v_lshl_or_b32 %0, %1, %2, %3" : "=v"(r) : "v"(t), "n"(bit), "v"(acc));
    return r;
}


enum { MODE_NT = 0, MODE_NN = 1, MODE_TN = 2 };

struct GemmArgs {
    const float* A; int lda;
    const float* B; int ldb;
    float* C; int ldc;
    float* colsum;
    int M, N, K;
    int kchunk;
    long slab_stride;
    EpiArgs ea;
    float* part = nullptr;
    long part_stride = 0;
};

template <int BK>
__device__ __forceinline__ int kc_off(int row, int slot) {
    constexpr int NS = BK / 4, RPB = 64 / BK;
    return row * BK + 4 * (slot ^ ((row / RPB) % NS));
}

template <int ROWS, int BK, int NTH>
struct KcTile {
    static constexpr int KV = BK / 4;
    static constexpr int LDK = BK;
    static constexpr int TOTALV = ROWS * KV;
    static constexpr int NV = (TOTALV + NTH - 1) / NTH;
    float4 v[NV];
    float f[NV];
    __device__ __forceinline__ void load(const float* __restrict__ P, int ld, int row0, int nrows, int k0, int kend, int tid) {
#pragma unroll
        for (int j = 0; j < NV; ++j) {
            const int i = min(tid + j * NTH, TOTALV - 1);
            const int row = i / KV, kc = (i % KV) << 2;
            const int gk = k0 + kc;
            f[j] = gk < kend ? 1.f : 0.f;
            v[j] = *reinterpret_cast<const float4*>(P + (size_t)min(row0 + row, nrows - 1) * ld + max(min(gk, kend - 4), 0));
        }
    }
    __device__ __forceinline__ void store(float* __restrict__ S, int tid) const {
#pragma unroll
        for (int j = 0; j < NV; ++j) {
            const int i = tid + j * NTH;
            const int row = i / KV, kc = (i % KV) << 2;
            if (TOTALV % NTH == 0 || i < TOTALV)
                *reinterpret_cast<float4*>(S + kc_off<BK>(row, kc >> 2)) = make_float4(v[j].x * f[j], v[j].y * f[j], v[j].z * f[j], v[j].w * f[j]);
        }
    }
};

template <int COLS, int BK, int NTH>
struct KmTile {
    static constexpr int TOTALV = COLS * BK / 4;
    static constexpr int NV = (TOTALV + NTH - 1) / NTH;
    static constexpr int LD = COLS + 4;
    float4 v[NV];
    float f[NV];
    __device__ __forceinline__ void load(const float* __restrict__ P, int ld, int col0, int ncols, int k0, int kend, int tid) {
#pragma unroll
        for (int j = 0; j < NV; ++j) {
            const int i = min(tid + j * NTH, TOTALV - 1);
            const int kr = i / (COLS / 4), c4 = (i % (COLS / 4)) << 2;
            const int gk = k0 + kr;
            f[j] = gk < kend ? 1.f : 0.f;
            v[j] = *reinterpret_cast<const float4*>(P + (size_t)max(min(gk, kend - 1), 0) * ld + max(min(col0 + c4, ncols - 4), 0));
        }
// ... 472 lines not shown
    };

    {
        const int k0 = kbeg + nfull * BK;
        if (MODE == MODE_TN) tail_a_km.load(g.A, g.lda, m0, g.M, k0, kend, tid); else tail_a_kc.load(g.A, g.lda, m0, g.M, k0, kend, tid);
        if (MODE == MODE_NT) tail_b_kc.load(g.B, g.ldb, n0, g.N, k0, kend, tid); else tail_b_km.load(g.B, g.ldb, n0, g.N, k0, kend, tid);
    }
    GF_GLOAD(0, 0)
    if constexpr (PD > 1) GF_GLOAD(1, 1)
    if constexpr (PD > 2) GF_GLOAD(2, 2)
    if constexpr (PD > 3) GF_GLOAD(3, 3)
    DropCtx dc;
    uint32_t keep[TM][TN];
    if constexpr (MODE != MODE_TN) {
        if (epi_has_dropout<EPI>()) dc = make_drop(g.ea.rng, g.ea.rng_add, g.ea.site, g.ea.p, g.ea.train);
        else dc.on = 0;
        gemm_keep_bits<EPI, TM, TN>(g, dc, keep, m0 + wm * WM, n0 + wn * WN, r, h);
    }
    if (nfull > 0) GF_SSTORE_FULL(0, 0) else sstore_tail(0);
    __syncthreads();

#define GF_STEP(U, UN)                                                                  \
    if (t0 + U < nt) {                                                                  \
        GF_GLOAD(U, t0 + U + PD)                                    \
        compute(U & 1);                                                                 \
         \
        if (t0 + U + 1 == nfull) sstore_tail((U + 1) & 1);       \
        else if (t0 + U + 1 < nfull) GF_SSTORE_FULL(UN, (U + 1) & 1)    \
        __syncthreads();                                                                \
    }
    for (int t0 = 0; t0 < nt; t0 += PD) {
        if constexpr (PD == 2) {
            GF_STEP(0, 1)
            GF_STEP(1, 0)
        } else {
            GF_STEP(0, 1)
            GF_STEP(1, 2)
            GF_STEP(2, 3)
            GF_STEP(3, 0)
        }
    }
#undef GF_STEP
#undef GF_GLOAD
#undef GF_SSTORE_FULL

    if (MODE == MODE_TN) {
        float* const slab = g.part ? g.part + (size_t)bz * g.part_stride : nullptr;
#pragma unroll
        for (int a = 0; a < TM; ++a)
#pragma unroll
            for (int b = 0; b < TN; ++b) {
                const int col = n0 + wn * WN + b * 32 + r;
                float old[16];
                if (!slab) {
#pragma unroll
                    for (int i = 0; i < 16; ++i) {
                        const int row = min(m0 + wm * WM + a * 32 + (i & 3) + 8 * (i >> 2) + 4 * h, g.M - 1);
                        old[i] = g.C[(size_t)row * g.ldc + min(col, g.N - 1)];
                    }
                }
#pragma unroll
                for (int i = 0; i < 16; ++i) {
                    const int row = m0 + wm * WM + a * 32 + (i & 3) + 8 * (i >> 2) + 4 * h;
                    if (row < g.M && col < g.N) {
                        if (slab) slab[(size_t)row * g.N + col] = acc[a][b][i];
                        else g.C[(size_t)row * g.ldc + col] = old[i] + acc[a][b][i];
                    }
                }
            }
        if (want_colsum) {
            constexpr int NR = NTH / (BM / 4);
            static_assert(NR * BM <= SM::TOTAL, "colsum scratch must fit the tile buffers");
            *reinterpret_cast<float4*>(smem + (tid / (BM / 4)) * BM + ((tid % (BM / 4)) << 2)) = colsum4;
            __syncthreads();
            if (tid < BM) {
                float sum = 0.f;
#pragma unroll
                for (int i = 0; i < NR; ++i) sum += smem[i * BM + tid];
                if (m0 + tid < g.M) {
                    if (slab) slab[(size_t)g.M * g.N + m0 + tid] = sum;
                    else g.colsum[m0 + tid] += sum;
                }
            }
        }
        return;
    }

    if constexpr (MODE != MODE_TN) gemm_store_epilogue<EPI, TM, TN>(g, acc, m0 + wm * WM, n0 + wn * WN, bz, r, h, dc, keep);
}

template <int MODE, int BM, int BN, int BK, int EPI, int WGM = 2, int WGN = 2, int SHORTK = 0>
__global__ __launch_bounds__(64 * WGM * WGN) void gemm_kernel(GemmArgs g) {
    const int gx = gridDim.x, gy = gridDim.y, per = gx * gy, nwg = per * gridDim.z;
    const int lin = blockIdx.x + gx * (blockIdx.y + gy * blockIdx.z);
    const int q8 = nwg >> 3, r8 = nwg & 7, xl = lin & 7;
    const int b = (xl < r8 ? xl * (q8 + 1) : r8 * (q8 + 1) + (xl - r8) * q8) + (lin >> 3);
    const int bz = b / per, t = b - bz * per, by = t / gx, bx = t - by * gx;
    gemm_body<MODE, BM, BN, BK, EPI, WGM, WGN>(g, bx, by, bz);
}

template <int MODE, int BM, int BN, int BK, int EPI, int WGM = 2, int WGN = 2, int SHORTK = 0>
__global__ __launch_bounds__(64 * WGM * WGN) void gemm_pair_kernel(GemmArgs g, GemmSeg1 s1, int gy0) {
    const int gx = gridDim.x, gy = gridDim.y, per = gx * gy, nwg = per * gridDim.z;
    const int lin = blockIdx.x + gx * (blockIdx.y + gy * blockIdx.z);
    const int q8 = nwg >> 3, r8 = nwg & 7, xl = lin & 7;
    const int b = (xl < r8 ? xl * (q8 + 1) : r8 * (q8 + 1) + (xl - r8) * q8) + (lin >> 3);
    const int bz = b / per, t = b - bz * per;
    int by = t / gx;
    const int bx = t - by * gx;
    if (by >= gy0) {
        by -= gy0;
        g.A = s1.A; g.C = s1.C; g.ea.mask_out = s1.mask_out; g.ea.train = s1.train;
    }
    gemm_body<MODE, BM, BN, BK, EPI, WGM, WGN>(g, bx, by, bz);
}

GF_LAB_ONLY(unsigned long long* g_wres_stamps = nullptr;)

template <int MODE, int EPI, int KC, bool PAIR>
__device__ __forceinline__ void gemm_wres_body(const GemmArgs& g, const int mtiles, const int wg_per_panel, const GemmSeg1& s1
                                               GF_LAB_ONLY(, unsigned long long* stamps)) {
    static_assert(KC % 4 == 0 && KC <= 128, "short K only");
    constexpr int BM = 64, BN = 64;
    constexpr int G8 = (KC + 7) / 8;
    constexpr int LD = 4 * ((KC / 4) | 1);
    constexpr int KV = KC / 4, TOTALV = BM * KV, NV = (TOTALV + 255) / 256;
    extern __shared__ __attribute__((aligned(16))) float smem[];

    const int tid = threadIdx.x, lane = tid & 63, wave = tid >> 6;
    const int wm = wave >> 1, wn = wave & 1, r = lane & 31, h = lane >> 5;
    const int panel = blockIdx.x / wg_per_panel, j0 = blockIdx.x - panel * wg_per_panel;
    const int n0 = panel * BN;
    GF_LAB_ONLY(unsigned long long* const stamp = (stamps && tid == 0) ? stamps + 4 * (size_t)blockIdx.x : nullptr;
                if (stamp) stamp[0] = __builtin_amdgcn_s_memtime();)

    constexpr bool TAIL2 = (KC % 8) == 4;
    constexpr int G8F = TAIL2 ? KC / 8 : G8;
    float wf[G8][4];
    float wtail[2] = {0.f, 0.f};
    {
        const int n = min(n0 + wn * 32 + r, g.N - 1);
        if constexpr (TAIL2) {
            if (MODE == MODE_NT) {
                const float4 q = *reinterpret_cast<const float4*>(g.B + (size_t)n * g.ldb + KC - 4);
                wtail[0] = h ? q.y : q.x;
                wtail[1] = h ? q.w : q.z;
            } else {
                wtail[0] = g.B[(size_t)(KC - 4 + h) * g.ldb + n];
                wtail[1] = g.B[(size_t)(KC - 2 + h) * g.ldb + n];
            }
        }
#pragma unroll
        for (int gq = 0; gq < G8F; ++gq) {
            const int k = 8 * gq + 4 * h;
            const float keepw = k < KC ? 1.f : 0.f;
            const int kc = min(k, KC - 4);
            if (MODE == MODE_NT) {
                const float4 q = *reinterpret_cast<const float4*>(g.B + (size_t)n * g.ldb + kc);
                wf[gq][0] = q.x * keepw; wf[gq][1] = q.y * keepw; wf[gq][2] = q.z * keepw; wf[gq][3] = q.w * keepw;
            } else {
#pragma unroll
                for (int j = 0; j < 4; ++j) wf[gq][j] = g.B[(size_t)(kc + j) * g.ldb + n] * keepw;
            }
        }
    }
// ... 148 lines not shown
        return 0;
    }
    if (per > mtiles) per = mtiles;
    hipLaunchKernelGGL((gemm_wres_kernel<MODE, EPI, KC>), dim3(panels * per), dim3(256), lds, st, g, mtiles, per GF_LAB_ONLY(, g_wres_stamps));
    GF_LAUNCH_CHECK();
    return 0;
}

__global__ __launch_bounds__(256) void tn_reduce_kernel(float* __restrict__ C, float* __restrict__ colsum,
                                                        const float* __restrict__ part, long part_stride, int splits, long nC,
                                                        int nS, int ldc, int N) {
    const long i4 = ((long)blockIdx.x * blockDim.x + threadIdx.x) * 4;
    if (i4 < nC) {
        float4 s = make_float4(0.f, 0.f, 0.f, 0.f);
        for (int z0 = 0; z0 < splits; z0 += 8) {
            float4 v[8];
#pragma unroll
            for (int u = 0; u < 8; ++u) v[u] = *reinterpret_cast<const float4*>(part + (size_t)min(z0 + u, splits - 1) * part_stride + i4);
#pragma unroll
            for (int u = 0; u < 8; ++u) {
                const float m = (z0 + u < splits) ? 1.f : 0.f;
                s.x += m * v[u].x; s.y += m * v[u].y; s.z += m * v[u].z; s.w += m * v[u].w;
            }
        }
        const long row = i4 / N, col = i4 - row * N;
        float* dst = C + row * ldc + col;
        dst[0] += s.x; dst[1] += s.y; dst[2] += s.z; dst[3] += s.w;
    } else if (colsum != nullptr && i4 < nC + 4 * (long)((nS + 3) / 4)) {
        for (int e = 0; e < 4; ++e) {
            const long i = i4 - nC + e;
            if (i < nS) {
                float s = part[nC + i];
                for (int z = 1; z < splits; ++z) s += part[(size_t)z * part_stride + nC + i];
                colsum[i] += s;
            }
        }
    }
}

constexpr int MAXP = 40;
struct TnProblem {
    const float* A; const float* B; float* C; float* colsum;
    int lda, ldb, ldc, M, N, K, kchunk;
    int tiles_n, tiles_mn;
    int block0;
    long part_off;
};
struct TnGroup {
    TnProblem p[MAXP];
    int n;
    float* part;
    long part_stride;
    int splits;
};

template <bool SPLIT, int BN = 64>
__global__ __launch_bounds__(256) void gemm_tn_grouped_kernel(TnGroup grp) {
    int pi = 0;
    const int nwg = gridDim.x, q8 = nwg >> 3, r8 = nwg & 7, xl = blockIdx.x & 7;
    const int b = (xl < r8 ? xl * (q8 + 1) : r8 * (q8 + 1) + (xl - r8) * q8) + (blockIdx.x >> 3);
#pragma unroll 1
    for (int i = 1; i < grp.n; ++i)
        if (b >= grp.p[i].block0) pi = i;
    const TnProblem& q = grp.p[pi];
    const int local = b - q.block0;
    const int bz = local / q.tiles_mn, t2 = local - bz * q.tiles_mn;
    GemmArgs g;
    g.A = q.A; g.lda = q.lda; g.B = q.B; g.ldb = q.ldb; g.C = q.C; g.ldc = q.ldc; g.colsum = q.colsum;
    g.M = q.M; g.N = q.N; g.K = q.K; g.kchunk = q.kchunk; g.slab_stride = 0;
    if constexpr (SPLIT) { g.part = grp.part + q.part_off; g.part_stride = grp.part_stride; }
    constexpr int PW = 8;
    const int tiles_m = q.tiles_mn / q.tiles_n;
    const int panel = t2 / (PW * tiles_m), rem = t2 - panel * PW * tiles_m;
    const int pw = min(PW, q.tiles_n - panel * PW);
    const int mt = rem / pw, nt = panel * PW + rem - mt * pw;
    gemm_body<MODE_TN, 64, BN, 16, EPI_NONE, 2, 2>(g, nt, mt, bz);
}

template <int MODE, int BM, int BN, int BK, int EPI, int WGM = 2, int WGN = 2, int SHORTK = 0>
static int launch_cfg(const GemmArgs& g, int splits, hipStream_t st) {
    dim3 grid((g.N + BN - 1) / BN, (g.M + BM - 1) / BM, splits);
    constexpr size_t lds = Smem<MODE, BM, BN, BK>::TOTAL * sizeof(float);
    GF_TRY((lds_optin<gemm_kernel<MODE, BM, BN, BK, EPI, WGM, WGN, SHORTK>>(lds, "gemm")));
    hipLaunchKernelGGL((gemm_kernel<MODE, BM, BN, BK, EPI, WGM, WGN, SHORTK>), grid, dim3(64 * WGM * WGN), lds, st, g);
    GF_LAUNCH_CHECK();
    return 0;
}

template <int MODE, int BM, int BN, int BK, int EPI, int WGM = 2, int WGN = 2, int SHORTK = 0>
static int launch_cfg_pair(const GemmArgs& g, const GemmSeg1& s1, int splits, hipStream_t st) {
    const int gy0 = (g.M + BM - 1) / BM;
    dim3 grid((g.N + BN - 1) / BN, 2 * gy0, splits);
    constexpr size_t lds = Smem<MODE, BM, BN, BK>::TOTAL * sizeof(float);
    GF_TRY((lds_optin<gemm_pair_kernel<MODE, BM, BN, BK, EPI, WGM, WGN, SHORTK>>(lds, "gemm")));
    hipLaunchKernelGGL((gemm_pair_kernel<MODE, BM, BN, BK, EPI, WGM, WGN, SHORTK>), grid, dim3(64 * WGM * WGN), lds, st, g, s1, gy0);
    GF_LAUNCH_CHECK();
    return 0;
}

template <int EPI>
static int launch_pick_pair(const GemmArgs& g, const GemmSeg1& s1, int splits, hipStream_t st) {
    if (g.K == 100 && g.N >= 1024 && splits == 1 && (g.lda & 3) == 0 && (g.ldb & 3) == 0 &&
        (size_t)g.M * g.lda * 4 < (size_t(1) << 31) && (size_t)g.M * g.ldc * 4 < (size_t(1) << 31)) {
        if constexpr (EPI == EPI_RELU_DROP) return launch_wres<MODE_NT, EPI, true>(g, st, &s1);
        else return fail(-1, "gemm_nt_pair: no two-segment form of the weight-resident kernel for epilogue %d", EPI);
    }
    if (g.K <= 128) return launch_cfg_pair<MODE_NT, 64, 64, 16, EPI, 2, 2, 1>(g, s1, splits, st);
    return launch_cfg_pair<MODE_NT, 64, 64, 16, EPI>(g, s1, splits, st);
}

template <int MODE, int EPI>
static int launch_pick(const GemmArgs& g, int splits, hipStream_t st) {
    if constexpr (MODE != MODE_TN)
        if (g.K == 100 && g.N >= 1024 && splits == 1 && (g.lda & 3) == 0 && ((MODE == MODE_NT) ? (g.ldb & 3) == 0 : true) &&
            (size_t)g.M * g.lda * 4 < (size_t(1) << 31) && (size_t)g.M * g.ldc * 4 < (size_t(1) << 31))
            return launch_wres<MODE, EPI>(g, st);
    if (g.K <= 128) return launch_cfg<MODE, 64, 64, 16, EPI, 2, 2, 1>(g, splits, st);
    return launch_cfg<MODE, 64, 64, 16, EPI>(g, splits, st);
}

static inline bool fits32(long rows, long ld) { return (unsigned long long)rows * (unsigned long long)ld * 4ull < (1ull << 32); }

static int check_common(const float* A, int lda, const float* B, int ldb, const float* C, int M, int N, int K) {
    GF_CHECK_ARG(A && B && C, "gemm: null pointer");
    GF_CHECK_ARG(M > 0 && N > 0 && K > 0, "gemm: bad shape M=%d N=%d K=%d", M, N, K);
    GF_CHECK_ARG((lda & 3) == 0 && (ldb & 3) == 0, "gemm: leading dims must be multiples of 4 (lda=%d ldb=%d)", lda, ldb);
    GF_CHECK_ARG(aligned16(A) && aligned16(B), "gemm: operands must be 16-byte aligned");
    return 0;
}

#define EPI_SWITCH(MODE, g, st)                                                            \
    switch (epi) {                                                                         \
        case EPI_NONE: return launch_pick<MODE, EPI_NONE>(g, splits, st);                  \
        case EPI_RELU_DROP: return launch_pick<MODE, EPI_RELU_DROP>(g, 1, st);             \
        case EPI_DROP_GELU: return launch_pick<MODE, EPI_DROP_GELU>(g, 1, st);             \
        case EPI_MASK_POS: return launch_pick<MODE, EPI_MASK_POS>(g, 1, st);               \
        case EPI_GELU_BWD_DROP:                                                            \
        case EPI_GELU_BWD_DROP0: return launch_pick<MODE, EPI_GELU_BWD_DROP>(g, 1, st);    \
        case EPI_GELU_BWD: return launch_pick<MODE, EPI_GELU_BWD>(g, 1, st);               \
        default: return fail(-1, "gemm: unknown epilogue %d", epi);                        \
    }

int gemm_splitk_factor(int M, int N, int K) {
    const long tiles = (long)((M + 63) / 64) * ((N + 63) / 64);
    if (tiles >= 384 || K < 512) return 1;
    long s = (768 + tiles - 1) / tiles;
    const long maxs = K / 256;
    if (s > maxs) s = maxs;
    if (s > 8) s = 8;
    return s < 1 ? 1 : (int)s;
}

static void set_split(GemmArgs& g, int& splits, long slab_stride) {
    if (splits <= 1) { splits = 1; g.kchunk = g.K; g.slab_stride = 0; return; }
    int kchunk = ((g.K + splits - 1) / splits + 63) / 64 * 64;
    splits = (g.K + kchunk - 1) / kchunk;
    g.kchunk = kchunk;
    g.slab_stride = slab_stride;
}

int launch_gemm_nt(const float* A, int lda, const float* W, int ldw, float* C, int ldc, int M, int N, int K,
                   int epi, const EpiArgs& ea, hipStream_t st, int* splits_io, long slab_stride) {
    GF_TRY(check_common(A, lda, W, ldw, C, M, N, K));
    GF_CHECK_ARG((K & 3) == 0, "gemm_nt: K=%d must be a multiple of 4", K);
    GF_CHECK_ARG(fits32(M, lda) && fits32(N, ldw), "gemm_nt: an operand of 4 GiB or more is not supported");
    GemmArgs g{A, lda, W, ldw, C, ldc, nullptr, M, N, K, K, 0, ea};
    int splits = (splits_io && epi == EPI_NONE) ? *splits_io : 1;
    set_split(g, splits, slab_stride);
    if (splits_io) *splits_io = splits;
    EPI_SWITCH(MODE_NT, g, st)
}

int launch_gemm_nt_pair(const float* A, int lda, const float* W, int ldw, float* C, int ldc, int M, int N, int K, int epi,
                        const EpiArgs& ea, const GemmSeg1& s1, hipStream_t st, int* splits_io, long slab_stride) {
    GF_CHECK_ARG(epi == EPI_RELU_DROP || epi == EPI_NONE, "gemm_nt_pair: epilogue %d has no two-segment form", epi);
    GF_TRY(check_common(A, lda, W, ldw, C, M, N, K));
    GF_CHECK_ARG(s1.A && s1.C && aligned16(s1.A) && ea.aux_in == nullptr, "gemm_nt_pair: bad second segment");
    GF_CHECK_ARG((K & 3) == 0, "gemm_nt: K=%d must be a multiple of 4", K);
    GF_CHECK_ARG(fits32(M, lda) && fits32(N, ldw), "gemm_nt: an operand of 4 GiB or more is not supported");
    GemmArgs g{A, lda, W, ldw, C, ldc, nullptr, M, N, K, K, 0, ea};
    int splits = (splits_io && epi == EPI_NONE) ? *splits_io : 1;
    set_split(g, splits, slab_stride);
    if (splits_io) *splits_io = splits;
    if (epi == EPI_RELU_DROP) return launch_pick_pair<EPI_RELU_DROP>(g, s1, 1, st);
    return launch_pick_pair<EPI_NONE>(g, s1, splits, st);
}

int launch_gemm_nn(const float* A, int lda, const float* Bm, int ldb, float* C, int ldc, int M, int N, int K,
                   int epi, const EpiArgs& ea, hipStream_t st, int* splits_io, long slab_stride) {
    GF_TRY(check_common(A, lda, Bm, ldb, C, M, N, K));
    GF_CHECK_ARG((K & 3) == 0 && (N & 3) == 0, "gemm_nn: K=%d and N=%d must be multiples of 4", K, N);
    GF_CHECK_ARG(fits32(M, lda) && fits32(K, ldb), "gemm_nn: an operand of 4 GiB or more is not supported");
    GemmArgs g{A, lda, Bm, ldb, C, ldc, nullptr, M, N, K, K, 0, ea};
    int splits = (splits_io && epi == EPI_NONE) ? *splits_io : 1;
    set_split(g, splits, slab_stride);
    if (splits_io) *splits_io = splits;
    EPI_SWITCH(MODE_NN, g, st)
}

constexpr long TN_ACC_MAXSPLIT = 16;

long gemm_tn_part_floats(int M, int N, int K) {
    const long tiles = (long)((M + 63) / 64) * ((N + 63) / 64);
    long splits = (768 + tiles - 1) / tiles;
    const long maxsplits = (K + 63) / 64;
    if (splits > maxsplits) splits = maxsplits;
    if (splits > TN_ACC_MAXSPLIT) splits = TN_ACC_MAXSPLIT;
    if (splits <= 1) return 0;
    return splits * ((long)M * N + M);
}

static int launch_tn_reduce(float* C, int ldc, float* colsum, const float* part, long part_stride, int splits, int M, int N,
                            hipStream_t st) {
    const long nC = (long)M * N;
    const long n4 = nC / 4 + (colsum ? (M + 3) / 4 : 0);
    hipLaunchKernelGGL(tn_reduce_kernel, dim3((unsigned)((n4 + 255) / 256)), dim3(256), 0, st, C, colsum, part, part_stride,
                       splits, nC, M, ldc, N);
    GF_LAUNCH_CHECK();
    return 0;
}

int launch_gemm_tn_acc(const float* At, int lda, const float* Bm, int ldb, float* C, int ldc, float* colsum,
                       int M, int N, int K, hipStream_t st, float* part_ws, long part_floats) {
    GF_TRY(check_common(At, lda, Bm, ldb, C, M, N, K));
    GF_CHECK_ARG((M & 3) == 0 && (N & 3) == 0, "gemm_tn: M=%d and N=%d must be multiples of 4", M, N);
    GF_CHECK_ARG(fits32(K, lda) && fits32(K, ldb), "gemm_tn: an operand of 4 GiB or more is not supported");
    EpiArgs ea;
    GemmArgs g{At, lda, Bm, ldb, C, ldc, colsum, M, N, K, K, 0, ea};
    const long tiles = (long)((M + 63) / 64) * ((N + 63) / 64);
    const long per = (long)M * N + M;
    long splits = (768 + tiles - 1) / tiles;
    const long maxsplits = (K + 63) / 64;
    if (splits > maxsplits) splits = maxsplits;
    if (splits > TN_ACC_MAXSPLIT) splits = TN_ACC_MAXSPLIT;
    if (part_ws == nullptr) splits = 1;
    else if (splits * per > part_floats) splits = part_floats / per;
    if (splits < 1) splits = 1;
    int kchunk = (int)(((K + splits - 1) / splits + 63) / 64 * 64);
    splits = (K + kchunk - 1) / kchunk;
    g.kchunk = kchunk;
    if (splits > 1) {
        GF_CHECK_ARG(aligned16(part_ws), "gemm_tn: partial-slab workspace must be 16-byte aligned");
        g.part = part_ws;
        g.part_stride = (per + 3) & ~3L;
        if (splits * g.part_stride > part_floats) { splits = 1; g.part = nullptr; g.kchunk = K; }
    }
    GF_TRY((launch_cfg<MODE_TN, 64, 64, 16, EPI_NONE>(g, (int)splits, st)));
    if (splits > 1) GF_TRY(launch_tn_reduce(C, ldc, colsum, g.part, g.part_stride, (int)splits, M, N, st));
    return 0;
}

constexpr int TN_GROUP_MIN_TILES = 1024;
constexpr int TN_GROUP_TILES = 2560;
constexpr int TN_GROUP_MAXSPLIT = 8;

__global__ __launch_bounds__(256) void tn_reduce_grouped_kernel(TnGroup grp) {
    const TnProblem& q = grp.p[blockIdx.y];
    const float* part = grp.part + q.part_off;
    const long nC = (long)q.M * q.N;
    for (long i4 = ((long)blockIdx.x * 256 + threadIdx.x) * 4; i4 < nC; i4 += (long)gridDim.x * 1024) {
        float4 v[TN_GROUP_MAXSPLIT];
#pragma unroll
        for (int z = 0; z < TN_GROUP_MAXSPLIT; ++z)
            v[z] = *reinterpret_cast<const float4*>(part + (size_t)min(z, grp.splits - 1) * grp.part_stride + i4);
        const long row = i4 / q.N, col = i4 - row * q.N;
        float* dst = q.C + row * q.ldc + col;
        const float4 old = *reinterpret_cast<const float4*>(dst);
        float4 s = v[0];
#pragma unroll
        for (int z = 1; z < TN_GROUP_MAXSPLIT; ++z)
            if (z < grp.splits) { s.x += v[z].x; s.y += v[z].y; s.z += v[z].z; s.w += v[z].w; }
        *reinterpret_cast<float4*>(dst) = make_float4(old.x + s.x, old.y + s.y, old.z + s.z, old.w + s.w);
    }
    if (q.colsum != nullptr)
        for (int i = blockIdx.x * 256 + threadIdx.x; i < q.M; i += gridDim.x * 256) {
            float s = part[nC + i];
            for (int z = 1; z < grp.splits; ++z) s += part[(size_t)z * grp.part_stride + nC + i];
            q.colsum[i] += s;
        }
}

long gemm_tn_grouped_part_floats() { return (long)(TN_GROUP_TILES + 256) * (64 * 64 + 64) + 4 * MAXP; }


int launch_gemm_tn_grouped(const TnDesc* d, int n, hipStream_t st, float* part_ws, long part_floats, TnSlabs* slabs) {
    GF_CHECK_ARG(d && n >= 1 && n <= MAXP, "gemm_tn_grouped: n=%d out of [1,%d]", n, MAXP);
    if (!mode().tn100_off() && part_ws != nullptr && aligned16(part_ws) && tn100_supported(d, n))
        return launch_gemm_tn100_grouped(d, n, st, part_ws, part_floats, slabs);
    GF_CHECK_ARG(slabs == nullptr, "gemm_tn_grouped: unreduced gradient slabs exist only for the d_model-100 kernel");
    TnGroup grp;
    grp.n = n;
    bool wide = true;
    long wtiles = 0;
    for (int i = 0; i < n; ++i) {
        GF_CHECK_ARG(fits32(d[i].K, d[i].lda) && fits32(d[i].K, d[i].ldb), "gemm_tn_grouped: an operand of 4 GiB or more is not supported");
        wide = wide && (d[i].N % 128 == 0);
        wtiles += (long)((d[i].M + 63) / 64) * ((d[i].N + 127) / 128);
    }
    wide = wide && wtiles >= TN_GROUP_MIN_TILES;
    const int BNs = wide ? 128 : 64;
    long tiles = 0, per_split = 0;
    int kmax = 0;
    for (int i = 0; i < n; ++i) {
        GF_TRY(check_common(d[i].At, d[i].lda, d[i].B, d[i].ldb, d[i].C, d[i].M, d[i].N, d[i].K));
        GF_CHECK_ARG((d[i].M & 3) == 0 && (d[i].N & 3) == 0, "gemm_tn_grouped: M, N must be multiples of 4");
        tiles += (long)((d[i].M + 63) / 64) * ((d[i].N + BNs - 1) / BNs);
        per_split += (((long)d[i].M * d[i].N + d[i].M) + 3) & ~3L;
        kmax = d[i].K > kmax ? d[i].K : kmax;
        if (!aligned16(d[i].C) || (d[i].ldc & 3) != 0) part_ws = nullptr;
    }
    int splits = 1;
    if (part_ws != nullptr && tiles < TN_GROUP_MIN_TILES) {
        splits = (int)((TN_GROUP_TILES + tiles - 1) / tiles);
        if (splits > TN_GROUP_MAXSPLIT) splits = TN_GROUP_MAXSPLIT;
        if (splits > kmax / 256) splits = kmax / 256;
        if ((long)splits * per_split > part_floats) splits = (int)(part_floats / per_split);
        if (splits < 2) splits = 1;
    }
    grp.splits = splits;
    grp.part = splits > 1 ? part_ws : nullptr;
    grp.part_stride = per_split;
    GF_CHECK_ARG(splits == 1 || aligned16(part_ws), "gemm_tn_grouped: partial-slab workspace must be 16-byte aligned");
    int total = 0;
    long off = 0;
    for (int i = 0; i < n; ++i) {
        TnProblem& q = grp.p[i];
        q.A = d[i].At; q.B = d[i].B; q.C = d[i].C; q.colsum = d[i].colsum;
        q.lda = d[i].lda; q.ldb = d[i].ldb; q.ldc = d[i].ldc; q.M = d[i].M; q.N = d[i].N; q.K = d[i].K;
        q.kchunk = splits > 1 ? (int)((((long)d[i].K + splits - 1) / splits + 63) / 64 * 64) : d[i].K;
        const int tm = (d[i].M + 63) / 64;
        q.tiles_n = (d[i].N + BNs - 1) / BNs;
        q.tiles_mn = tm * q.tiles_n;
        q.block0 = total;
        q.part_off = off;
        off += (((long)d[i].M * d[i].N + d[i].M) + 3) & ~3L;
        total += q.tiles_mn * splits;
    }
    if (wide && splits == 1) {
        constexpr size_t ldsw = Smem<MODE_TN, 64, 128, 16>::TOTAL * sizeof(float);
        hipLaunchKernelGGL((gemm_tn_grouped_kernel<false, 128>), dim3(total), dim3(256), ldsw, st, grp);
        GF_LAUNCH_CHECK();
        return 0;
    }
    constexpr size_t lds = Smem<MODE_TN, 64, 64, 16>::TOTAL * sizeof(float);
    if (splits > 1) hipLaunchKernelGGL(gemm_tn_grouped_kernel<true>, dim3(total), dim3(256), lds, st, grp);
    else hipLaunchKernelGGL(gemm_tn_grouped_kernel<false>, dim3(total), dim3(256), lds, st, grp);
    GF_LAUNCH_CHECK();
    if (splits > 1) {
        hipLaunchKernelGGL(tn_reduce_grouped_kernel, dim3(64, n), dim3(256), 0, st, grp);
        GF_LAUNCH_CHECK();
    }
    return 0;
}

}
```

gan_ffn_amd/engine.py:

```python
import ctypes as C
import os

import torch

from . import _lib, ops
from ._lib import HeadCfg

SCHEDULE = [
    ("D", "visual", "acoustic"), ("G", "acoustic", "visual"),
    ("D", "visual", "text"), ("G", "text", "visual"),
    ("D", "text", "acoustic"), ("G", "acoustic", "text"),
    ("D", "acoustic", "text"), ("G", "text", "acoustic"),
    ("D", "text", "visual"), ("G", "visual", "text"),
    ("D", "acoustic", "visual"), ("G", "visual", "acoustic"),
]
LOSS_COLUMNS = ["acoustic_G_loss", "visual_G_loss", "text_G_loss", "visual_D_loss", "text_D_loss",
                "acoustic_D_loss"]


class NetState:

    def __init__(self, module, lr, betas, weight_decay=0.0):
        self.m = module
        self.slab = module.slab
# ... 102 lines not shown
        self.works.append((w, lo, hi))

    def finish(self, on_bucket=None):
        for w, lo, hi in self.works:
            w.wait()
            if on_bucket is not None and lo is not None:
                on_bucket(lo, hi)
        self.works = []


def bucket_ranges(enc_floats, obj_floats, total, layer_floats, L, n_buckets):
    out = [(enc_floats + obj_floats, total)]
    per = max(1, (L + n_buckets - 1) // max(1, n_buckets))
    hi = L
    while hi > 0:
        lo = max(0, hi - per)
        out.append((lo * layer_floats, hi * layer_floats))
        hi = lo
    return out


class _Pass:

    def __init__(self, net, S, B, dev, need_bwd, S_cap=None):
        self.net, self.B, self.dev, self.need_bwd = net, B, dev, need_bwd
        self.S_cap = max(S, S_cap or 0)
        self.B_cap = B
        E = net.E
        cfg = ops.enc_cfg(self.S_cap, B, E, net.H, net.L, train=True, p_pe=net.p_pe, p_enc=net.p_enc)
        n_saved, n_ws = ops.enc_sizes(cfg)
        h_saved, h_ws = ops.head_sizes(HeadCfg(self.S_cap * B, E, net.D1, net.D2, net.kind, net.p_head, 1))
        f32 = dict(device=dev, dtype=torch.float32)
        Tc = self.S_cap * B
        self._enc_out = torch.empty(Tc * E, **f32)
        self._saved = torch.empty(n_saved, **f32) if need_bwd else None
        self._hsaved = torch.empty(h_saved, **f32)
        self._out = torch.empty(Tc * (net.D2 if net.kind == 0 else 1), **f32)
        self._dx = torch.empty(Tc * E, **f32) if need_bwd else None
        self.n_ws = max(n_ws, h_ws)
        if ops.encoder_fwd_pair_supported(cfg):
            self.n_ws = max(self.n_ws, ops.encoder_fwd_pair_workspace_floats(cfg))
        self.resize(S)

    def resize(self, S, B=None):
        B = self.B_cap if B is None else B
        assert S <= self.S_cap and B <= self.B_cap
        net = self.net
        self.B = B
        E = net.E
        self.S, self.T = S, S * B
        self.cfg_train = ops.enc_cfg(S, B, E, net.H, net.L, train=True, p_pe=net.p_pe, p_enc=net.p_enc)
        self.cfg_eval = ops.enc_cfg(S, B, E, net.H, net.L, train=False, p_pe=net.p_pe, p_enc=net.p_enc)
        self.pair_ok = ops.encoder_fwd_pair_supported(self.cfg_train)
        n_saved, _ = ops.enc_sizes(self.cfg_train)
        self.hcfg_train = HeadCfg(self.T, E, net.D1, net.D2, net.kind, net.p_head, 1)
        self.hcfg_eval = HeadCfg(self.T, E, net.D1, net.D2, net.kind, net.p_head, 0)
        h_saved, _ = ops.head_sizes(self.hcfg_train)
        Do = net.D2 if net.kind == 0 else 1
        self.enc_out = self._enc_out[:self.T * E].view(S, B, E)
        self.saved = self._saved[:n_saved] if self.need_bwd else None
        self.hsaved = self._hsaved[:h_saved]
        self.out = self._out[:self.T * Do].view(S, B, Do)
        self.dx = self._dx[:self.T * E].view(S, B, E) if self.need_bwd else None


class _Res:

    def __init__(self):
        self.last_write = None
        self.reads = []


STREAM_MAP = {1: [0] * 12,
              2: [0, 0, 1, 1, 0, 0, 1, 1, 0, 0, 1, 1],
              3: [0, 0, 1, 1, 0, 0, 1, 1, 2, 2, 2, 2]}

ADDS_PER_SUBSTEP = 4
SCHEDULE_BIMODAL = [s for s in SCHEDULE if "visual" not in s[1:]]
STREAM_MAP_BIMODAL = {1: [0, 0, 0, 0], 2: [0, 0, 1, 1]}


GEN_PAIR_MAX_UNPAIRED_E = 128


def find_gen_pairs(schedule, stream_map):
    return [i for i in range(len(schedule) - 1)
            if schedule[i][0] == "D" and schedule[i + 1][0] == "G" and schedule[i + 1][1] == schedule[i][2]
            and stream_map[i] == stream_map[i + 1]]


_STREAMS = {}


def _side_streams(dev, prios, tuner=None, work=1):
    key = (str(dev), tuple(prios))
    if os.environ.get("GANFFN_STREAM_CACHE", "1") == "1" and key in _STREAMS and work <= 4 * _STREAMS[key][1]:
        return _STREAMS[key][0]
    if tuner is not None and len(prios) > 1 and os.environ.get("GANFFN_STREAM_TUNE", "1") == "1" and \
            not torch.cuda.is_current_stream_capturing():
        streams = tuner(prios)
    else:
        streams = [torch.cuda.Stream(device=dev, priority=p_) for p_ in prios]
    _STREAMS[key] = (streams, max(1, work))
    return streams


# ... 203 lines not shown
        self._use_scratch(0)

    def _use_scratch(self, i):
        sc = self.scratch[i]
        self.ws, self.x_cat, self.obj_out = sc["ws"], sc["x_cat"], sc["obj_out"]
        self.dprob2, self.dprob1, self.d_real = sc["dprob2"], sc["dprob1"], sc["d_real"]

    def _r(self, key):
        r = self._res.get(key)
        if r is None:
            r = self._res[key] = _Res()
        return r

    def _wait_writers(self, stream, keys):
        for k in keys:
            ev = self._r(k).last_write
            if ev is not None:
                stream.wait_event(ev)

    def _wait_readers(self, stream, keys):
        for k in keys:
            for ev in self._r(k).reads:
                stream.wait_event(ev)

    def _done(self, stream, reads, writes):
        ev = torch.cuda.Event()
        ev.record(stream)
        for k in reads:
            self._r(k).reads.append(ev)
        for k in writes:
            r = self._r(k)
            r.last_write, r.reads = ev, []

    def _next_add(self):
        v = self._adds
        self._adds += 1
        return self._base_add + v

    def _net_fwd(self, net, ps, x, train, save, adds=None):
        cfg = ps.cfg_train if train else ps.cfg_eval
        hcfg = ps.hcfg_train if train else ps.hcfg_eval
        if adds is None:
            a0, a1 = self._next_add(), self._next_add()
        else:
            a0, a1 = self._base_add + adds[0], self._base_add + adds[1]
        ops.encoder_fwd_raw(cfg, x, net.pe, net.slab, ps.enc_out, ps.saved if save else None, self.ws, self.rng.state, a0)
        w = net.w
        w3 = w("fc3.weight") if net.kind == 1 else None
        b3 = w("fc3.bias") if net.kind == 1 else None
        ops.head_fwd_raw(hcfg, ps.enc_out, w("fc1.weight"), w("fc1.bias"), w("fc2.weight"), w("fc2.bias"), w3, b3,
                         ps.out, ps.hsaved, self.ws, self.rng.state, a1)
        return a0, a1

    def _net_bwd(self, net, ps, d_out, train, adds, want_wgrad, reduce_cb=None, need_dx=None, parts=False):
        cfg = ps.cfg_train if train else ps.cfg_eval
        hcfg = ps.hcfg_train if train else ps.hcfg_eval
        a0, a1 = adds
        w = net.w
        g = (lambda n: net.w(n, grad=True)) if want_wgrad else (lambda n: None)
        w3 = w("fc3.weight") if net.kind == 1 else None
        ops.head_bwd_raw(hcfg, d_out, ps.enc_out, w("fc1.weight"), w("fc2.weight"), w3,
                         g("fc1.weight"), g("fc1.bias"), g("fc2.weight"), g("fc2.bias"),
                         g("fc3.weight") if net.kind == 1 else None, g("fc3.bias") if net.kind == 1 else None,
                         ps.dx, ps.hsaved, self.ws, self.rng.state, a1)
        gslab = net.grad if want_wgrad else None
        if need_dx is None:
            need_dx = not want_wgrad
        if parts and want_wgrad and reduce_cb is None:
            return ops.encoder_bwd_parts_raw(cfg, ps.dx, net.slab, gslab, ps.saved, self.ws, self.rng.state, a0, need_dx)
        if reduce_cb is None or not want_wgrad:
            ops.encoder_bwd_raw(cfg, 0, net.L, ps.dx, net.slab, gslab, ps.saved, self.ws, self.rng.state, a0, need_dx)
        else:
            bks = net.buckets(self.n_buckets)
            reduce_cb(*bks[0], last=False)
            for i, (lo_f, hi_f) in enumerate(bks[1:]):
                lo, hi = lo_f // net.layer_floats, hi_f // net.layer_floats
                ops.encoder_bwd_raw(cfg, lo, hi, ps.dx, net.slab, gslab, ps.saved, self.ws, self.rng.state, a0, need_dx)
                reduce_cb(lo_f, hi_f, last=(i == len(bks) - 2))

    def _adam(self, net, parts=None):
        if parts is not None and parts[2] > 1:
            ops.adam_step_parts_raw(net.slab, net.grad, net.exp_avg, net.exp_avg_sq, net.step, net.total, net.lr, net.betas[0],
                                    net.betas[1], parts[0], parts[1], parts[2], net.enc_floats, net.layer_floats, net.covered,
                                    1e-8, net.wd, 1.0 / self.world)
            return
        ops.adam_step_raw(net.slab, net.grad, net.exp_avg, net.exp_avg_sq, net.step, net.total, net.lr,
                          net.betas[0], net.betas[1], 1e-8, net.wd, 1.0 / self.world)

    def _parts_ok(self, net, ps):
        return self.pg is None and os.environ.get("GANFFN_ADAM_PARTS", "1") == "1" and net.total % 4 == 0 and \
            ops.encoder_bwd_parts_supported(ps.cfg_train)

    def _zero_grad(self, net, parts):
        if parts:
            net.grad[net.enc_floats:].zero_()
        else:
            net.grad.zero_()

    def _adam_slice(self, net, lo, hi):
        ops.adam_update_raw(net.slab[lo:hi], net.grad[lo:hi], net.exp_avg[lo:hi], net.exp_avg_sq[lo:hi], net.step, hi - lo,
                            net.lr, net.betas[0], net.betas[1], 1e-8, net.wd, 1.0 / self.world)

    def _make_reducer(self, net):
        if self.pg is None:
            def plain(net_key, parts=None):
                self._pre_write(net_key)
                self._adam(net, parts)
            return None, plain
        if dp_mode() == "inline":
            import torch.distributed as dist
            group = getattr(self, "_cur_pg", None) or self.pg

            def inline(net_key, parts=None):
                dist.all_reduce(net.grad, op=dist.ReduceOp.SUM, group=group, async_op=False)
                self._pre_write(net_key)
                self._adam(net)
            return None, inline
        red = GradReducer(getattr(self, "_cur_pg", None) or self.pg)

        def cb(lo, hi, last):
            red.reduce_async(net.grad[lo:hi], lo, hi)

        def finish_and_step(net_key, parts=None):
            self._pre_write(net_key)
            red.finish(lambda lo, hi: self._adam_slice(net, lo, hi) if hi > lo else None)
            ops.adam_bump_raw(net.step)
        return cb, finish_and_step

    def _gen_pair_fwd(self, net, ps_eval, ps_train, x, adds_eval, adds_train):
        a0, a1 = self._base_add + adds_train[0], self._base_add + adds_train[1]
        ops.encoder_fwd_pair_raw(ps_train.cfg_train, x, net.pe, net.slab, ps_eval.enc_out, ps_train.enc_out, ps_train.saved,
                                 self.ws, self.rng.state, a0)
        w = net.w
        w3 = w("fc3.weight") if net.kind == 1 else None
        b3 = w("fc3.bias") if net.kind == 1 else None
        for hcfg, ps, add in ((ps_eval.hcfg_eval, ps_eval, self._base_add + adds_eval[1]), (ps_train.hcfg_train, ps_train, a1)):
            ops.head_fwd_raw(hcfg, ps.enc_out, w("fc1.weight"), w("fc1.bias"), w("fc2.weight"), w("fc2.bias"), w3, b3,
                             ps.out, ps.hsaved, self.ws, self.rng.state, add)
        return a0, a1

    def _pair_slot(self, i):
        if not self.gen_pair or i not in self._gen_pairs:
            return None
        ps = self.pass_G[self.schedule[i][2]]
        if not ps.pair_ok or (self.gen_pair_mode != "all" and ps.net.E <= GEN_PAIR_MAX_UNPAIRED_E):
            return None
        return i + 1

    def train_disc(self, who, partner, batch, loss_slot, pair_slot=None):
        S, B = batch[who].shape[:2]
        Dn, Gn = self.D[who], self.G[partner]
        pg_, pd = self.pass_G_nosave[partner], self.pass_D2[who]
        a = ADDS_PER_SUBSTEP * loss_slot
        g_adds = None
        if pair_slot is not None:
            ap = ADDS_PER_SUBSTEP * pair_slot
            g_adds = self._gen_pair_fwd(Gn, pg_, self.pass_G[partner], batch[partner], (a, a + 1), (ap, ap + 1))
        else:
            self._net_fwd(Gn, pg_, batch[partner], train=False, save=False, adds=(a, a + 1))
        x_real = batch[who]
        if Dn.has_obj:
            ops.linear_fwd_raw(x_real, Dn.w("object.weight"), Dn.w("object.bias"), self.obj_out, S * B, Dn.obj_in, self.D_h)
            x_real = self.obj_out
        torch.cat((x_real, pg_.out), dim=1, out=self.x_cat)
        adds = self._net_fwd(Dn, pd, self.x_cat, train=True, save=True, adds=(a + 2, a + 3))
        n = S * 2 * B
        ops._lib.call("ganffn_bce2_fwd", ops._ptr(pd.out), C.c_float(1.0), C.c_float(0.0), 2 * B, B, n, C.c_float(1.0),
                      ops._ptr(self.losses[loss_slot:loss_slot + 1]), 0, ops._stream())
        ops._lib.call("ganffn_bce2_bwd", ops._ptr(pd.out), C.c_float(1.0), C.c_float(0.0), 2 * B, B, n, C.c_float(1.0),
                      ops._ptr(self.dprob2), ops._stream())
        parts_mode = self._parts_ok(Dn, pd)
        self._zero_grad(Dn, parts_mode)
        cb, finish = self._make_reducer(Dn)
        parts = self._net_bwd(Dn, pd, self.dprob2, True, adds, True, cb, need_dx=Dn.has_obj, parts=parts_mode)
        if Dn.has_obj:
            self.d_real.copy_(pd.dx[:, :B])
            scratch = self.ws[:parts[3]] if (parts is not None and parts[2] > 1) else self.ws
            ops.linear_bwd_raw(self.d_real, batch[who], Dn.w("object.weight"), None, Dn.w("object.weight", True),
                               Dn.w("object.bias", True), S * B, Dn.obj_in, self.D_h, scratch)
            if cb is not None:
                cb(Dn.enc_floats, Dn.enc_floats + Dn.obj_floats, last=True)
        finish(("D", who), parts)
        return g_adds

    def train_gen_forward(self, who, batch, loss_slot):
        a = ADDS_PER_SUBSTEP * loss_slot
        return self._net_fwd(self.G[who], self.pass_G[who], batch[who], train=True, save=True, adds=(a, a + 1))

    def train_gen(self, who, partner, batch, loss_slot, g_adds=None):
        S, B = batch[who].shape[:2]
        Gn, Dn = self.G[who], self.D[partner]
        pg_, pd = self.pass_G[who], self.pass_D1[partner]
        a = ADDS_PER_SUBSTEP * loss_slot
        if g_adds is None:
            g_adds = self.train_gen_forward(who, batch, loss_slot)
        d_adds = self._net_fwd(Dn, pd, pg_.out, train=False, save=True, adds=(a + 2, a + 3))
        n = S * B
        ops.bce_fwd_raw(pd.out, 1.0, n, 1.0, self.losses[loss_slot:loss_slot + 1], False)
        ops.bce_bwd_raw(pd.out, 1.0, n, 1.0, self.dprob1)
        self._net_bwd(Dn, pd, self.dprob1, False, d_adds, False)
        parts_mode = self._parts_ok(Gn, pg_)
        self._zero_grad(Gn, parts_mode)
        cb, finish = self._make_reducer(Gn)
        parts = self._net_bwd(Gn, pg_, pd.dx, True, g_adds, True, cb, parts=parts_mode)
        finish(("G", who), parts)

    def _pre_write(self, net_key):
        if self.n_streams > 1 and self._cur_stream is not None:
            self._wait_readers(self._cur_stream, [net_key])

    _cur_stream = None

    def _iteration_body(self, batch, device_rng_advance):
        self._adds = 0
        self._check_slabs()
        if not device_rng_advance:
            self._base_add = self.rng.next_add(ADDS_PER_SUBSTEP * len(self.schedule))
        self._adds = ADDS_PER_SUBSTEP * len(self.schedule)
        if self.n_streams == 1:
            paired = {}
            for i, (kind, who, partner) in enumerate(self.schedule):
                j = self._pair_slot(i) if kind == "D" else None
                if j is not None:
                    paired[j] = self.train_disc(who, partner, batch, i, pair_slot=j)
                elif kind == "D":
                    self.train_disc(who, partner, batch, i)
                elif i in paired:
                    self.train_gen(who, partner, batch, i, g_adds=paired[i])
                else:
                    self.train_gen(who, partner, batch, i)
        else:
            origin = torch.cuda.current_stream()
            fork = torch.cuda.Event()
            fork.record(origin)
            smap = self.stream_map
            for st in self.streams:
                st.wait_event(fork)
                for k in self.modalities:
                    if batch[k].is_cuda:
                        batch[k].record_stream(st)
            early = {}
            nsub = len(self.schedule)
            for i, (kind, who, partner) in enumerate(self.schedule):
                st = self.streams[smap[i]]
                j = i + 1
                if self.early_gen and j < nsub and self.schedule[j][0] == "G" and smap[j] == smap[i] and \
                        (kind, who) != ("G", self.schedule[j][1]):
                    gwho = self.schedule[j][1]
                    hs = self.streams[self.n_streams + smap[j]]
                    self._use_scratch(self.n_streams + smap[j])
                    with torch.cuda.stream(hs):
                        self._wait_writers(hs, [("G", gwho), ("buf", "G", gwho)])
                        self._wait_readers(hs, [("buf", "G", gwho)])
                        early[j] = self.train_gen_forward(gwho, batch, j)
                        ev = torch.cuda.Event()
                        ev.record(hs)
                        self._r(("G", gwho)).reads.append(ev)
# ... 628 lines not shown
```

gan_ffn_amd/ops.py:

```python
import ctypes as C

import torch

from . import _lib
from ._lib import EncCfg, HeadCfg, GanffnError

FF = 2048
ENC_DROPOUT = 0.1
PE_DROPOUT = 0.2
LN_EPS = 1e-5
N_LAYERS = 8


def _ptr(t):
    return None if t is None else C.c_void_p(t.data_ptr())


def _stream():
    return C.c_void_p(torch.cuda.current_stream().cuda_stream)


def _need_gpu(*ts):
    for t in ts:
        if t is not None and not t.is_cuda:
# ... 52 lines not shown
    return [(3 * E, E), (3 * E,), (E, E), (E,), (F, E), (F,), (E, F), (E,), (E,), (E,), (E,), (E,)]


def layer_layout(E, F=FF):
    lib = _lib.load()
    offs = (C.c_int64 * 12)()
    _lib.check(lib.ganffn_layer_param_offsets(E, F, offs), "ganffn_layer_param_offsets")
    return int(lib.ganffn_layer_param_count(E, F)), [int(o) for o in offs]


def enc_cfg(S, B, E, H, L=N_LAYERS, F=FF, train=False, p_pe=PE_DROPOUT, p_enc=ENC_DROPOUT):
    return EncCfg(S, B, E, H, F, L, p_pe, p_enc, LN_EPS, 1 if train else 0)


def enc_sizes(cfg):
    lib = _lib.load()
    s = int(lib.ganffn_encoder_saved_floats(C.byref(cfg)))
    w = int(lib.ganffn_encoder_workspace_floats(C.byref(cfg)))
    if s < 0 or w < 0:
        _lib.check(-1, "ganffn_encoder_*_floats")
    return s, w


def head_sizes(cfg):
    lib = _lib.load()
    s = int(lib.ganffn_head_saved_floats(C.byref(cfg)))
    w = int(lib.ganffn_head_workspace_floats(C.byref(cfg)))
    if s < 0 or w < 0:
        _lib.check(-1, "ganffn_head_*_floats")
    return s, w


def encoder_fwd_raw(cfg, x, pe, slab, out, saved, ws, rng, add):
    _lib.call("ganffn_encoder_fwd", C.byref(cfg), _ptr(x), _ptr(pe), _ptr(slab), _ptr(out), _ptr(saved), _ptr(ws),
              _ptr(rng), C.c_uint64(add), _stream())


def encoder_fwd_pair_supported(cfg):
    return int(_lib.load().ganffn_encoder_fwd_pair_supported(C.byref(cfg))) == 1


def encoder_fwd_pair_workspace_floats(cfg):
    w = int(_lib.load().ganffn_encoder_fwd_pair_workspace_floats(C.byref(cfg)))
    if w < 0:
        _lib.check(-1, "ganffn_encoder_fwd_pair_workspace_floats")
    return w


def encoder_fwd_pair_raw(cfg, x, pe, slab, out_eval, out_train, saved_train, ws, rng, add_train):
    _lib.call("ganffn_encoder_fwd_pair", C.byref(cfg), _ptr(x), _ptr(pe), _ptr(slab), _ptr(out_eval), _ptr(out_train),
              _ptr(saved_train), _ptr(ws), _ptr(rng), C.c_uint64(add_train), _stream())


def encoder_bwd_raw(cfg, lo, hi, dx, slab, gslab, saved, ws, rng, add, need_dx_in=True):
    _lib.call("ganffn_encoder_bwd2", C.byref(cfg), lo, hi, _ptr(dx), _ptr(slab), _ptr(gslab), _ptr(saved), _ptr(ws),
              _ptr(rng), C.c_uint64(add), 1 if need_dx_in else 0, _stream())


def encoder_bwd_parts_supported(cfg):
    return int(_lib.load().ganffn_encoder_bwd_parts_supported(C.byref(cfg))) == 1


def encoder_bwd_parts_raw(cfg, dx, slab, gslab, saved, ws, rng, add, need_dx_in=True):
    off, stride, n = C.c_int64(0), C.c_int64(0), C.c_int(0)
    _lib.call("ganffn_encoder_bwd_parts", C.byref(cfg), _ptr(dx), _ptr(slab), _ptr(gslab), _ptr(saved), _ptr(ws), _ptr(rng),
              C.c_uint64(add), 1 if need_dx_in else 0, C.byref(off), C.byref(stride), C.byref(n), _stream())
    return (ws[off.value:] if n.value > 1 else None), stride.value, n.value, off.value


def adam_step_parts_raw(p, g, m, v, step, n, lr, b1, b2, parts, part_stride, n_parts, enc_floats, layer_floats, covered, eps=1e-8,
                        wd=0.0, gscale=1.0):
    _lib.call("ganffn_adam_step_parts", _ptr(p), _ptr(g), _ptr(m), _ptr(v), _ptr(step), C.c_int64(n), C.c_float(lr), C.c_float(b1),
              C.c_float(b2), C.c_float(eps), C.c_float(wd), C.c_float(gscale), _ptr(parts), C.c_int64(part_stride), n_parts,
              C.c_int64(enc_floats), C.c_int64(layer_floats), C.c_int64(covered), _stream())


def head_fwd_raw(cfg, x, w1, b1, w2, b2, w3, b3, out, saved, ws, rng, add):
    _lib.call("ganffn_head_fwd", C.byref(cfg), _ptr(x), _ptr(w1), _ptr(b1), _ptr(w2), _ptr(b2), _ptr(w3), _ptr(b3),
              _ptr(out), _ptr(saved), _ptr(ws), _ptr(rng), C.c_uint64(add), _stream())


def head_bwd_raw(cfg, d_out, x, w1, w2, w3, gw1, gb1, gw2, gb2, gw3, gb3, dx, saved, ws, rng, add):
    _lib.call("ganffn_head_bwd", C.byref(cfg), _ptr(d_out), _ptr(x), _ptr(w1), _ptr(w2), _ptr(w3), _ptr(gw1), _ptr(gb1),
              _ptr(gw2), _ptr(gb2), _ptr(gw3), _ptr(gb3), _ptr(dx), _ptr(saved), _ptr(ws), _ptr(rng), C.c_uint64(add),
              _stream())


def linear_fwd_raw(x, w, b, y, T, K, N):
    _lib.call("ganffn_linear_fwd", _ptr(x), _ptr(w), _ptr(b), _ptr(y), T, K, N, _stream())


def linear_bwd_raw(dy, x, w, dx, gw, gb, T, K, N, ws=None):
    _lib.call("ganffn_linear_bwd", _ptr(dy), _ptr(x), _ptr(w), _ptr(dx), _ptr(gw), _ptr(gb), T, K, N, _ptr(ws),
              C.c_int64(ws.numel() if ws is not None else 0), _stream())


def bce_fwd_raw(prob, target, n, scale, loss, accumulate):
    _lib.call("ganffn_bce_fwd", _ptr(prob), C.c_float(target), n, C.c_float(scale), _ptr(loss), 1 if accumulate else 0,
              _stream())


def bce_bwd_raw(prob, target, n, scale, dprob):
    _lib.call("ganffn_bce_bwd", _ptr(prob), C.c_float(target), n, C.c_float(scale), _ptr(dprob), _stream())


def adam_step_raw(p, g, m, v, step, n, lr, b1, b2, eps=1e-8, wd=0.0, gscale=1.0):
    _lib.call("ganffn_adam_step", _ptr(p), _ptr(g), _ptr(m), _ptr(v), _ptr(step), C.c_int64(n), C.c_float(lr),
              C.c_float(b1), C.c_float(b2), C.c_float(eps), C.c_float(wd), C.c_float(gscale), _stream())


def adam_update_raw(p, g, m, v, step, n, lr, b1, b2, eps=1e-8, wd=0.0, gscale=1.0):
    _lib.call("ganffn_adam_update", _ptr(p), _ptr(g), _ptr(m), _ptr(v), _ptr(step), C.c_int64(n), C.c_float(lr),
              C.c_float(b1), C.c_float(b2), C.c_float(eps), C.c_float(wd), C.c_float(gscale), _stream())


def adam_bump_raw(step):
    _lib.call("ganffn_adam_bump", _ptr(step), _stream())


def rng_advance_raw(rng, delta):
    _lib.call("ganffn_rng_advance", _ptr(rng), C.c_uint64(delta), _stream())


class LinearFn(torch.autograd.Function):

    @staticmethod
    def forward(ctx, x, w, b):
        _need_gpu(x, w, b)
        xc, wc, bc = _f32c(x), _f32c(w), _f32c(b)
        K, N = wc.shape[1], wc.shape[0]
        T = xc.numel() // K
        y = torch.empty(*xc.shape[:-1], N, device=x.device, dtype=torch.float32)
        linear_fwd_raw(xc, wc, bc, y, T, K, N)
        ctx.save_for_backward(xc, wc)
        return y

    @staticmethod
    def backward(ctx, dy):
        xc, wc = ctx.saved_tensors
        dy = _f32c(dy)
        K, N = wc.shape[1], wc.shape[0]
        T = xc.numel() // K
        dx = torch.empty_like(xc) if ctx.needs_input_grad[0] else None
        gw = torch.zeros_like(wc) if ctx.needs_input_grad[1] else None
        gb = torch.zeros(N, device=dy.device, dtype=torch.float32) if gw is not None else None
        linear_bwd_raw(dy, xc, wc, dx, gw, gb, T, K, N)
        return dx, gw, (gb if ctx.needs_input_grad[2] else None)


class EncoderFn(torch.autograd.Function):

    @staticmethod
    def forward(ctx, x, pe, slab, meta, *params):
        _need_gpu(x, slab)
        E, H, L, train = meta["E"], meta["H"], meta["L"], meta["train"]
        S, B = x.shape[0], x.shape[1]
# ... 553 lines not shown
```

include/ganffn.h:

```cpp
#ifndef GANFFN_H
#define GANFFN_H

#include <stdint.h>

#ifdef __cplusplus
extern "C" {
#endif

#define GANFFN_VERSION 100
#define GANFFN_MAX_SEQ 112

typedef struct ganffn_enc_cfg {
    int32_t S, B;
    int32_t E, H, F, L;
    float p_pe;
    float p_enc;
    float ln_eps;
    int32_t train;
} ganffn_enc_cfg;

typedef struct ganffn_head_cfg {
    int32_t T;
    int32_t E;
    int32_t D1, D2;
    int32_t kind;
    float p;
    int32_t train;
} ganffn_head_cfg;

int ganffn_version(void);
const char* ganffn_last_error(void);

int64_t ganffn_layer_param_count(int E, int F);
int ganffn_layer_param_offsets(int E, int F, int64_t* offsets12);

int64_t ganffn_encoder_saved_floats(const ganffn_enc_cfg* cfg);
int64_t ganffn_encoder_workspace_floats(const ganffn_enc_cfg* cfg);
int64_t ganffn_encoder_saved_hidden_offset(const ganffn_enc_cfg* cfg, int layer);
int64_t ganffn_head_saved_floats(const ganffn_head_cfg* cfg);
int64_t ganffn_head_workspace_floats(const ganffn_head_cfg* cfg);

int ganffn_rng_advance(uint64_t* rng, uint64_t delta, void* stream);

int ganffn_pe_table(float* pe, int max_len, int E, void* stream);

int ganffn_encoder_fwd(const ganffn_enc_cfg* cfg, const float* x_in, const float* pe,
                       const float* params, float* out, float* saved, float* workspace,
                       const uint64_t* rng, uint64_t rng_offset_add, void* stream);

int ganffn_encoder_fwd_pair_supported(const ganffn_enc_cfg* cfg);
int64_t ganffn_encoder_fwd_pair_workspace_floats(const ganffn_enc_cfg* cfg);
int ganffn_encoder_fwd_pair(const ganffn_enc_cfg* cfg, const float* x_in, const float* pe, const float* params,
                            float* out_eval, float* out_train, float* saved_train, float* workspace,
                            const uint64_t* rng, uint64_t rng_offset_add_train, void* stream);

int ganffn_encoder_bwd(const ganffn_enc_cfg* cfg, int layer_lo, int layer_hi, float* dx,
                       const float* params, float* grads, const float* saved, float* workspace,
                       const uint64_t* rng, uint64_t rng_offset_add, void* stream);

int ganffn_encoder_bwd2(const ganffn_enc_cfg* cfg, int layer_lo, int layer_hi, float* dx,
                        const float* params, float* grads, const float* saved, float* workspace,
                        const uint64_t* rng, uint64_t rng_offset_add, int need_dx_in, void* stream);

int ganffn_encoder_bwd_parts_supported(const ganffn_enc_cfg* cfg);
int64_t ganffn_encoder_bwd_parts_covered(int E, int F);
int ganffn_encoder_bwd_parts(const ganffn_enc_cfg* cfg, float* dx, const float* params, float* grads, const float* saved,
                             float* workspace, const uint64_t* rng, uint64_t rng_offset_add, int need_dx_in,
                             int64_t* part_offset, int64_t* part_stride, int* n_parts, void* stream);

int ganffn_head_fwd(const ganffn_head_cfg* cfg, const float* x, const float* w1, const float* b1,
                    const float* w2, const float* b2, const float* w3, const float* b3, float* out,
                    float* saved, float* workspace, const uint64_t* rng, uint64_t rng_offset_add,
                    void* stream);
int ganffn_head_bwd(const ganffn_head_cfg* cfg, const float* d_out, const float* x,
                    const float* w1, const float* w2, const float* w3, float* gw1, float* gb1,
                    float* gw2, float* gb2, float* gw3, float* gb3, float* dx, const float* saved,
                    float* workspace, const uint64_t* rng, uint64_t rng_offset_add, void* stream);

int ganffn_linear_fwd(const float* x, const float* w, const float* b, float* y, int T, int K, int N,
                      void* stream);
int64_t ganffn_linear_bwd_workspace_floats(int T, int K, int N);
int ganffn_linear_bwd(const float* dy, const float* x, const float* w, float* dx, float* gw,
                      float* gb, int T, int K, int N, float* workspace, int64_t workspace_floats, void* stream);

int ganffn_bce_fwd(const float* prob, float target, int n, float scale, float* loss_out,
                   int accumulate, void* stream);
int ganffn_bce_bwd(const float* prob, float target, int n, float scale, float* dprob, void* stream);
int ganffn_bce2_fwd(const float* prob, float target_a, float target_b, int period, int split, int n,
                    float scale, float* loss_out, int accumulate, void* stream);
int ganffn_bce2_bwd(const float* prob, float target_a, float target_b, int period, int split, int n,
                    float scale, float* dprob, void* stream);

int ganffn_adam_step(float* params, const float* grads, float* exp_avg, float* exp_avg_sq,
                     int32_t* step, int64_t n, float lr, float beta1, float beta2, float eps,
                     float weight_decay, float grad_scale, void* stream);
int ganffn_adam_step_parts(float* params, const float* grads, float* exp_avg, float* exp_avg_sq, int32_t* step, int64_t n,
                           float lr, float beta1, float beta2, float eps, float weight_decay, float grad_scale,
                           const float* parts, int64_t part_stride, int n_parts, int64_t enc_floats, int64_t layer_floats,
                           int64_t covered_per_layer, void* stream);
int ganffn_adam_update(float* params, const float* grads, float* exp_avg, float* exp_avg_sq,
                       const int32_t* step, int64_t n, float lr, float beta1, float beta2, float eps,
                       float weight_decay, float grad_scale, void* stream);
int ganffn_adam_bump(int32_t* step, void* stream);

int ganffn_add3(const float* a, const float* b, const float* c, float* out, int64_t n, void* stream);
int ganffn_logsoftmax_nll(const float* logits, const int64_t* labels, const float* umask,
                          const float* class_w, float* log_prob, float* loss_out, float* dlogits,
                          float* workspace2, int S, int B, int C, void* stream);

int ganffn_general2_attention_fwd(const float* x, const float* mem, const float* mask, float* att,
                                  float* alpha, float* tanh_s, int S, int B, int D, void* stream);
int ganffn_general2_attention_bwd(const float* d_att, const float* x, const float* mem, const float* mask,
                                  const float* alpha, const float* tanh_s, float* du_ws, float* dx,
                                  float* dmem, int S, int B, int D, void* stream);

typedef struct ganffn_drnn_cfg {
    int32_t S, B;
    int32_t Dm, H, He;
    float p;
    int32_t train;
} ganffn_drnn_cfg;
typedef struct ganffn_drnn_params {
    const float *g_wih, *g_whh, *g_bih, *g_bhh, *p_wih, *p_whh, *p_bih, *p_bhh, *e_wih, *e_whh, *e_bih, *e_bhh, *att_w;
} ganffn_drnn_params;
typedef struct ganffn_drnn_grads {
    float *g_wih, *g_whh, *g_bih, *g_bhh, *p_wih, *p_whh, *p_bih, *p_bhh, *e_wih, *e_whh, *e_bih, *e_bhh, *att_w;
} ganffn_drnn_grads;
int64_t ganffn_drnn_saved_floats(const ganffn_drnn_cfg* cfg);
int64_t ganffn_drnn_workspace_floats(const ganffn_drnn_cfg* cfg);
int ganffn_drnn_fwd(const ganffn_drnn_cfg* cfg, int ndir, const float* const* U, const int32_t* const* spk,
                    const float* const* mval, const ganffn_drnn_params* params, float* const* e_out,
                    float* const* alpha, float* const* saved, float* const* workspace, const uint64_t* rng,
                    uint64_t rng_offset_add, void* stream);
int ganffn_drnn_bwd(const ganffn_drnn_cfg* cfg, int ndir, const float* const* d_e, const float* const* U,
                    const int32_t* const* spk, const float* const* mval, const ganffn_drnn_params* params,
                    const ganffn_drnn_grads* grads, float* const* dU, const float* const* alpha,
                    const float* const* saved, float* const* workspace, const uint64_t* rng,
                    uint64_t rng_offset_add, void* stream);
typedef struct ganffn_drnn_listener_params {
    const float *l_wih, *l_whh, *l_bih, *l_bhh;
} ganffn_drnn_listener_params;
typedef struct ganffn_drnn_listener_grads {
    float *l_wih, *l_whh, *l_bih, *l_bhh;
} ganffn_drnn_listener_grads;
int64_t ganffn_drnn_listener_saved_floats(const ganffn_drnn_cfg* cfg);
int64_t ganffn_drnn_listener_workspace_floats(const ganffn_drnn_cfg* cfg);
int ganffn_drnn_listener_fwd(const ganffn_drnn_cfg* cfg, int ndir, const float* const* U, const int32_t* const* spk,
                             const float* const* mval, const ganffn_drnn_params* params,
                             const ganffn_drnn_listener_params* lparams, float* const* e_out, float* const* alpha,
                             float* const* saved, float* const* workspace, const uint64_t* rng, uint64_t rng_offset_add,
                             void* stream);
int ganffn_drnn_listener_bwd(const ganffn_drnn_cfg* cfg, int ndir, const float* const* d_e, const float* const* U,
                             const int32_t* const* spk, const float* const* mval, const ganffn_drnn_params* params,
                             const ganffn_drnn_listener_params* lparams, const ganffn_drnn_grads* grads,
                             const ganffn_drnn_listener_grads* lgrads, float* const* dU, const float* const* alpha,
                             const float* const* saved, float* const* workspace, const uint64_t* rng,
// ... 191 lines not shown
```

Measured before the change: 53230 utterances/s.

## Fuse BCE loss/grad with step bump, pair head forwards, add store-mode encoder bwd

```diff
diff --git a/gan_ffn_amd/_lib.py b/gan_ffn_amd/_lib.py
--- a/gan_ffn_amd/_lib.py
+++ b/gan_ffn_amd/_lib.py
@@ -121,6 +121,11 @@
     "ganffn_encoder_bwd_parts": (_I, [_PE, _P, _P, _P, _P, _P, _P, _U64, _I, C.POINTER(C.c_int64), C.POINTER(C.c_int64), C.POINTER(C.c_int), _P]),
     "ganffn_adam_update": (_I, [_P, _P, _P, _P, _P, _L, _F, _F, _F, _F, _F, _F, _P]),
     "ganffn_adam_bump": (_I, [_P, _P]),
+    "ganffn_adam_apply": (_I, [_P, _P, _P, _P, _P, _L, _F, _F, _F, _F, _F, _F, _P, _L, _I, _L, _L, _L, _P]),
+    "ganffn_bce2_fused": (_I, [_P, _F, _F, _I, _I, _I, _F, _P, _I, _P, _P, _P]),
+    "ganffn_bce_fused": (_I, [_P, _F, _I, _F, _P, _I, _P, _P, _P]),
+    "ganffn_head_fwd_pair": (_I, [_PH, _P, _P, _P, _P, _P, _P, _P, _P, _P, _P, _P, _U64, _U64, _I, _I, _P]),
+    "ganffn_encoder_bwd_store_supported": (_I, [_PE]),
     "ganffn_add3": (_I, [_P, _P, _P, _P, _L, _P]),
     "ganffn_logsoftmax_nll": (_I, [_P, _P, _P, _P, _P, _P, _P, _P, _I, _I, _I, _P]),
     "ganffn_gemm_nt": (_I, [_P, _P, _P, _P, _I, _I, _I, _P]),
diff --git a/gan_ffn_amd/csrc/api.hip b/gan_ffn_amd/csrc/api.hip
--- a/gan_ffn_amd/csrc/api.hip
+++ b/gan_ffn_amd/csrc/api.hip
@@ -380,11 +380,22 @@
 }
 static int encoder_bwd_impl(const ganffn_enc_cfg* c, int layer_lo, int layer_hi, float* dx, const float* params,
                             float* grads, const float* saved, float* workspace, const uint64_t* rng, uint64_t add,
-                            int need_dx_in, void* stream, TnSlabs* slabs);
+                            int need_dx_in, void* stream, TnSlabs* slabs, bool store = false);
+static bool bwd_store_supported(const ganffn_enc_cfg* c, const Mode md) { return !(c->E == 100 && !md.tn100_off()); }
+extern "C" int ganffn_encoder_bwd_store_supported(const ganffn_enc_cfg* c) {
+    if (check_cfg(c) != 0) return -1;
+    return bwd_store_supported(c, mode()) ? 1 : 0;
+}
 extern "C" int ganffn_encoder_bwd2(const ganffn_enc_cfg* c, int layer_lo, int layer_hi, float* dx, const float* params,
                                    float* grads, const float* saved, float* workspace, const uint64_t* rng, uint64_t add,
                                    int need_dx_in, void* stream) {
-    return encoder_bwd_impl(c, layer_lo, layer_hi, dx, params, grads, saved, workspace, rng, add, need_dx_in, stream, nullptr);
+    const bool store = (need_dx_in & GANFFN_BWD_STORE) != 0;
+    if (store) {
+        GF_TRY(check_cfg(c));
+        GF_CHECK_ARG(grads && layer_lo == 0 && layer_hi == c->L, "encoder_bwd2: store mode covers the whole stack (layers 0..L) of a pass with weight gradients");
+        GF_CHECK_ARG(bwd_store_supported(c, mode()), "encoder_bwd2: no store mode for this stack (ask ganffn_encoder_bwd_store_supported)");
+    }
+    return encoder_bwd_impl(c, layer_lo, layer_hi, dx, params, grads, saved, workspace, rng, add, need_dx_in & 1, stream, nullptr, store);
 }
 static bool bwd_parts_supported(const ganffn_enc_cfg* c, const Mode md) {
     return rc_supported(c->E) && !md.rc_off() && !md.tn100_off() && !md.tn100_in_kernel_sum() && !md.adam_slabs_off() && c->F == 2048 &&
@@ -410,7 +421,7 @@
 }
 static int encoder_bwd_impl(const ganffn_enc_cfg* c, int layer_lo, int layer_hi, float* dx, const float* params,
                             float* grads, const float* saved, float* workspace, const uint64_t* rng, uint64_t add,
-                            int need_dx_in, void* stream, TnSlabs* slabs) {
+                            int need_dx_in, void* stream, TnSlabs* slabs, bool store) {
     const Mode md = mode();
     GF_TRY(check_cfg(c));
     GF_CHECK_ARG(dx && params && saved && workspace, "encoder_bwd: null pointer");
@@ -513,7 +524,7 @@
                                     H, c->p_enc, site + 0, rng, add, train, st));
         if (G) tn[ntn++] = TnDesc{d_qkv, 3 * E, Xl, E, G + lo.in_w, E, G + lo.in_b, 3 * E, E, T};
         if (ntn == 40 || (l == layer_lo && ntn > 0)) {
-            GF_TRY(launch_gemm_tn_grouped(tn, ntn, st, tnp, gemm_tn_grouped_part_floats(), slabs));
+            GF_TRY(launch_gemm_tn_grouped(tn, ntn, st, tnp, gemm_tn_grouped_part_floats(), slabs, store));
             ntn = 0;
         }
         EpiArgs eadd;
@@ -528,7 +539,7 @@
             GF_TRY(launch_gemm_nn(d_qkv, 3 * E, P + lo.in_w, E, dx, E, T, E, 3 * E, EPI_NONE, eadd, st));
         }
     }
-    if (nred > 0) GF_TRY(launch_ln_param_reduce(nred, r_gw, r_gb, r_part, r_nb, E, st, slabs != nullptr));
+    if (nred > 0) GF_TRY(launch_ln_param_reduce(nred, r_gw, r_gb, r_part, r_nb, E, st, slabs != nullptr || store));
     if (layer_lo == 0 && need_dx_in) GF_TRY(launch_dropout_bwd_inplace(dx, T, E, c->p_pe, SITE_PE, rng, add, train, st));
     return 0;
 }
@@ -600,6 +611,39 @@
     return 0;
 }
 
+extern "C" int ganffn_head_fwd_pair(const ganffn_head_cfg* c, const float* x0, const float* x1, const float* w1, const float* b1,
+                                    const float* w2, const float* b2, float* out0, float* out1, float* saved0, float* saved1,
+                                    const uint64_t* rng, uint64_t add0, uint64_t add1, int train0, int train1, void* stream) {
+    GF_TRY(check_head(c));
+    GF_CHECK_ARG(c->kind == 0, "head_fwd_pair: the two-segment form exists for the generator head (kind 0) only");
+    GF_CHECK_ARG(x0 && x1 && w1 && b1 && w2 && b2 && out0 && out1 && saved0 && saved1, "head_fwd_pair: null pointer");
+    GF_CHECK_ARG(saved0 != saved1 && out0 != out1, "head_fwd_pair: the segments need buffers of their own");
+    GF_CHECK_ARG(!((train0 || train1) && c->p > 0.f) || rng, "head_fwd_pair: rng required in train mode");
+    hipStream_t st = (hipStream_t)stream;
+    const int T = c->T, E = c->E, D1 = c->D1, D2 = c->D2;
+    auto u1 = [&](float* s) { return s + (int64_t)T * E; };
+    auto a1 = [&](float* s) { return s + (int64_t)T * E + (int64_t)T * D1; };
+    auto u2 = [&](float* s) { return s + (int64_t)T * E + 2 * (int64_t)T * D1; };
+    const DropSeg1 d1{x1, saved1, add1, train1};
+    GF_TRY(launch_gelu_drop_fwd(x0, saved0, T, E, c->p, SITE_HEAD0, rng, add0, train0, st, &d1));
+    EpiArgs e, f;
+    e.p = f.p = c->p; e.rng = f.rng = rng; e.rng_add = add0; e.train = train0; f.rng_add = add1; f.train = train1;
+    auto fc = [&](const float* in0, const float* in1, const float* w, const float* b, float* pre0, float* pre1, float* o0, float* o1,
+                  int N, int K, uint32_t site) -> int {
+        e.bias = f.bias = b; e.site = f.site = site; e.aux_out = pre0; f.aux_out = pre1;
+        if (gemm_nt_pair_drop_gelu_supported(N, K)) {
+            GemmSeg1 g1{in1, o1, nullptr, train1};
+            g1.aux_out = pre1; g1.rng_add = add1;
+            return launch_gemm_nt_pair(in0, K, w, K, o0, N, T, N, K, EPI_DROP_GELU, e, g1, st);
+        }
+        GF_TRY(launch_gemm_nt(in0, K, w, K, o0, N, T, N, K, EPI_DROP_GELU, e, st));
+        return launch_gemm_nt(in1, K, w, K, o1, N, T, N, K, EPI_DROP_GELU, f, st);
+    };
+    GF_TRY(fc(saved0, saved1, w1, b1, u1(saved0), u1(saved1), a1(saved0), a1(saved1), D1, E, SITE_HEAD1));
+    GF_TRY(fc(a1(saved0), a1(saved1), w2, b2, u2(saved0), u2(saved1), out0, out1, D2, D1, SITE_HEAD2));
+    return 0;
+}
+
 extern "C" int ganffn_head_bwd(const ganffn_head_cfg* c, const float* d_out, const float* x, const float* w1, const float* w2,
                                const float* w3, float* gw1, float* gb1, float* gw2, float* gb2, float* gw3, float* gb3,
                                float* dx, const float* saved, float* workspace, const uint64_t* rng, uint64_t add,
diff --git a/gan_ffn_amd/csrc/common.h b/gan_ffn_amd/csrc/common.h
--- a/gan_ffn_amd/csrc/common.h
+++ b/gan_ffn_amd/csrc/common.h
@@ -224,6 +224,7 @@
 int gemm_splitk_factor(int M, int N, int K);
 struct GemmSeg1 {
     const float* A; float* C; uint16_t* mask_out; int train;
+    float* aux_out = nullptr; uint64_t rng_add = 0;
 };
 int launch_gemm_nt_pair(const float* A, int lda, const float* W, int ldw, float* C, int ldc, int M, int N, int K, int epi,
                         const EpiArgs& ea, const GemmSeg1& s1, hipStream_t st, int* splits_io = nullptr, long slab_stride = 0);
@@ -258,7 +259,8 @@
     float* grad_base; long range_floats;
     int n_parts; float* part; long part_stride;
 };
-int launch_gemm_tn_grouped(const TnDesc* d, int n, hipStream_t st, float* part_ws = nullptr, long part_floats = 0, TnSlabs* slabs = nullptr);
+int launch_gemm_tn_grouped(const TnDesc* d, int n, hipStream_t st, float* part_ws = nullptr, long part_floats = 0, TnSlabs* slabs = nullptr,
+                           bool store = false);
 bool tn100_supported(const TnDesc* d, int n);
 int launch_gemm_tn100_grouped(const TnDesc* d, int n, hipStream_t st, float* part_ws, long part_floats, TnSlabs* slabs = nullptr);
 long gemm_tn_grouped_part_floats();
@@ -329,7 +331,11 @@
                      const float* xhat, const float* rstd, const float* gamma, float* dz, float* dy, float* gpart,
                      const float* wo_t, float* d_attn, int T, float p, uint32_t site, const uint64_t* rng, uint64_t add, int train,
                      hipStream_t st);
+struct DropSeg1 {
+    const float* x; float* out; uint64_t add; int train;
+};
 int launch_gelu_drop_fwd(const float* x, float* out, int R, int C, float p, uint32_t site, const uint64_t* rng,
-                         uint64_t add, int train, hipStream_t st);
-
-}
+                         uint64_t add, int train, hipStream_t st, const DropSeg1* s1 = nullptr);
+bool gemm_nt_pair_drop_gelu_supported(int N, int K);
+
+}
diff --git a/gan_ffn_amd/csrc/elementwise.hip b/gan_ffn_amd/csrc/elementwise.hip
--- a/gan_ffn_amd/csrc/elementwise.hip
+++ b/gan_ffn_amd/csrc/elementwise.hip
@@ -33,10 +33,10 @@
 }
 
 template <int MODE>
-__global__ void drop_kernel(const float* __restrict__ x, const float* __restrict__ u, float* __restrict__ out, int R,
-                            int C, float p, uint32_t site, const uint64_t* __restrict__ rng, uint64_t add, int train) {
+__device__ __forceinline__ void drop_body(const float* __restrict__ x, const float* __restrict__ u, float* __restrict__ out, int R,
+                                          int C, float p, uint32_t site, const uint64_t* __restrict__ rng, uint64_t add, int train,
+                                          const long idx) {
     const int G = (R + 3) >> 2;
-    const long idx = (long)blockIdx.x * blockDim.x + threadIdx.x;
     if (idx >= (long)G * C) return;
     const int rg = (int)(idx / C), c = (int)(idx - (long)rg * C);
     const DropCtx dc = make_drop(rng, add, site, p, train);
@@ -53,6 +53,18 @@
             out[o] = v * mult[q];
         }
     }
+}
+template <int MODE>
+__global__ void drop_kernel(const float* __restrict__ x, const float* __restrict__ u, float* __restrict__ out, int R,
+                            int C, float p, uint32_t site, const uint64_t* __restrict__ rng, uint64_t add, int train) {
+    drop_body<MODE>(x, u, out, R, C, p, site, rng, add, train, (long)blockIdx.x * blockDim.x + threadIdx.x);
+}
+template <int MODE>
+__global__ void drop_pair_kernel(const float* __restrict__ x, float* __restrict__ out, int R, int C, float p, uint32_t site,
+                                 const uint64_t* __restrict__ rng, uint64_t add, int train, DropSeg1 s1, int nb0) {
+    int bx = blockIdx.x;
+    if (bx >= nb0) { bx -= nb0; x = s1.x; out = s1.out; add = s1.add; train = s1.train; }
+    drop_body<MODE>(x, nullptr, out, R, C, p, site, rng, add, train, (long)bx * blockDim.x + threadIdx.x);
 }
 
 __global__ void add_inplace_kernel(float* __restrict__ a, const float* __restrict__ b, long n4) {
@@ -408,6 +420,31 @@
     }
 }
 
+__global__ __launch_bounds__(1024) void bce_fused_kernel(const float* __restrict__ prob, float target_a, float target_b,
+                                                         int period, int split, int n, float scale, float* __restrict__ loss,
+                                                         int accumulate, float* __restrict__ dprob, int32_t* step_bump) {
+    __shared__ float red[16];
+    float s = 0.f;
+    for (int i = threadIdx.x; i < n; i += 1024) {
+        const float target = (period > 0 && (i % period) >= split) ? target_b : target_a;
+        const float p = prob[i];
+        const float lp = fmaxf(logf(p), -100.f);
+        const float l1p = fmaxf(logf(1.0f - p), -100.f);
+        s -= target * lp + (1.0f - target) * l1p;
+        dprob[i] = scale / (float)n * (p - target) / fmaxf(p * (1.0f - p), 1e-12f);
+    }
+    s = wave_sum(s);
+    if ((threadIdx.x & 63) == 0) red[threadIdx.x >> 6] = s;
+    __syncthreads();
+    if (threadIdx.x == 0) {
+        float t = 0.f;
+        for (int w = 0; w < 16; ++w) t += red[w];
+        t = t * scale / (float)n;
+        loss[0] = accumulate ? loss[0] + t : t;
+        if (step_bump != nullptr) *step_bump += 1;
+    }
+}
+
 __global__ void bce_bwd_kernel(const float* __restrict__ prob, float target_a, float target_b, int period, int split, int n,
                                float scale, float* __restrict__ dprob) {
     const int i = blockIdx.x * blockDim.x + threadIdx.x;
@@ -431,10 +468,10 @@
 template <int VEC>
 __global__ __launch_bounds__(256) void adam_kernel(float* __restrict__ p, const float* __restrict__ g, float* __restrict__ m,
                                                    float* __restrict__ v, const int32_t* __restrict__ step, long n, float lr,
-                                                   float b1, float b2, float eps, float wd, float gscale) {
+                                                   float b1, float b2, float eps, float wd, float gscale, int step_add) {
     const long i = ((long)blockIdx.x * blockDim.x + threadIdx.x) * VEC;
     if (i >= n) return;
-    const float t = (float)(*step + 1);
+    const float t = (float)(*step + step_add);
     const float bc1 = 1.0f - powf(b1, t);
     const float bc2 = 1.0f - powf(b2, t);
     const float lr_bc1 = lr / bc1, rs_bc2 = sqrtf(bc2);
@@ -458,10 +495,10 @@
                                                          float* __restrict__ v, const int32_t* __restrict__ step, long n, float lr,
                                                          float b1, float b2, float eps, float wd, float gscale,
                                                          const float* __restrict__ part, long part_stride, int n_extra,
-                                                         long enc_floats, long layer_floats, long covered) {
+                                                         long enc_floats, long layer_floats, long covered, int step_add) {
     const long i = ((long)blockIdx.x * blockDim.x + threadIdx.x) * 4;
     if (i >= n) return;
-    const float t = (float)(*step + 1);
+    const float t = (float)(*step + step_add);
     const float bc1 = 1.0f - powf(b1, t);
     const float bc2 = 1.0f - powf(b2, t);
     const float lr_bc1 = lr / bc1, rs_bc2 = sqrtf(bc2);
@@ -637,8 +674,15 @@
     return launch_dropout(dx, dx, R, C, p, site, rng, add, train, st);
 }
 int launch_gelu_drop_fwd(const float* x, float* out, int R, int C, float p, uint32_t site, const uint64_t* rng,
-                         uint64_t add, int train, hipStream_t st) {
+                         uint64_t add, int train, hipStream_t st, const DropSeg1* s1) {
     const long n = (long)((R + 3) / 4) * C;
+    if (s1) {
+        GF_CHECK_ARG(s1->x && s1->out, "gelu_drop_fwd: bad second segment");
+        const int nb0 = (int)nblk(n, 256);
+        hipLaunchKernelGGL(drop_pair_kernel<1>, dim3(2 * nb0), dim3(256), 0, st, x, out, R, C, p, site, rng, add, train, *s1, nb0);
+        GF_LAUNCH_CHECK();
+        return 0;
+    }
     hipLaunchKernelGGL(drop_kernel<1>, dim3(nblk(n, 256)), dim3(256), 0, st, x, (const float*)nullptr, out, R, C, p, site, rng, add, train);
     GF_LAUNCH_CHECK();
     return 0;
@@ -819,6 +863,19 @@
     return 0;
 }
 
+extern "C" int ganffn_bce2_fused(const float* prob, float target_a, float target_b, int period, int split, int n, float scale,
+                                 float* loss_out, int accumulate, float* dprob, int32_t* step_bump, void* stream) {
+    GF_CHECK_ARG(prob && loss_out && dprob && n > 0 && period >= 0 && split >= 0, "bce_fused: bad arguments");
+    hipLaunchKernelGGL(bce_fused_kernel, dim3(1), dim3(1024), 0, (hipStream_t)stream, prob, target_a, target_b, period, split, n,
+                       scale, loss_out, accumulate, dprob, step_bump);
+    GF_LAUNCH_CHECK();
+    return 0;
+}
+extern "C" int ganffn_bce_fused(const float* prob, float target, int n, float scale, float* loss_out, int accumulate,
+                                float* dprob, int32_t* step_bump, void* stream) {
+    return ganffn_bce2_fused(prob, target, target, 0, 0, n, scale, loss_out, accumulate, dprob, step_bump, stream);
+}
+
 extern "C" int ganffn_adam_bump(int32_t* step, void* stream) {
     GF_CHECK_ARG(step, "adam_bump: null step");
     hipLaunchKernelGGL(adam_step_inc, dim3(1), dim3(1), 0, (hipStream_t)stream, step);
@@ -833,34 +890,43 @@
     return ganffn_adam_bump(step, stream);
 }
 
-extern "C" int ganffn_adam_update(float* params, const float* grads, float* exp_avg, float* exp_avg_sq, const int32_t* step,
-                                  int64_t n, float lr, float beta1, float beta2, float eps, float weight_decay,
-                                  float grad_scale, void* stream) {
+static int adam_update_impl(float* params, const float* grads, float* exp_avg, float* exp_avg_sq, const int32_t* step,
+                            int64_t n, float lr, float beta1, float beta2, float eps, float weight_decay,
+                            float grad_scale, int step_add, void* stream) {
     GF_CHECK_ARG(params && grads && exp_avg && exp_avg_sq && step && n > 0, "adam_update: bad arguments");
     hipStream_t st = (hipStream_t)stream;
     const bool vec = aligned16(params) && aligned16(grads) && aligned16(exp_avg) && aligned16(exp_avg_sq);
     const long n4 = vec ? ((long)n & ~3L) : 0;
     if (n4 > 0) {
         hipLaunchKernelGGL(adam_kernel<4>, dim3((unsigned)((n4 / 4 + 255) / 256)), dim3(256), 0, st, params, grads, exp_avg,
-                           exp_avg_sq, (const int32_t*)step, n4, lr, beta1, beta2, eps, weight_decay, grad_scale);
+                           exp_avg_sq, (const int32_t*)step, n4, lr, beta1, beta2, eps, weight_decay, grad_scale, step_add);
         GF_LAUNCH_CHECK();
     }
     if (n4 < n) {
         hipLaunchKernelGGL(adam_kernel<1>, dim3((unsigned)((n - n4 + 255) / 256)), dim3(256), 0, st, params + n4, grads + n4,
                            exp_avg + n4, exp_avg_sq + n4, (const int32_t*)step, (long)n - n4, lr, beta1, beta2, eps,
-                           weight_decay, grad_scale);
+                           weight_decay, grad_scale, step_add);
         GF_LAUNCH_CHECK();
     }
     return 0;
 }
 
-extern "C" int ganffn_adam_step_parts(float* params, const float* grads, float* exp_avg, float* exp_avg_sq, int32_t* step, int64_t n,
-                                      float lr, float beta1, float beta2, float eps, float weight_decay, float grad_scale,
-                                      const float* parts, int64_t part_stride, int n_parts, int64_t enc_floats, int64_t layer_floats,
-                                      int64_t covered_per_layer, void* stream) {
+extern "C" int ganffn_adam_update(float* params, const float* grads, float* exp_avg, float* exp_avg_sq, const int32_t* step,
+                                  int64_t n, float lr, float beta1, float beta2, float eps, float weight_decay,
+                                  float grad_scale, void* stream) {
+    return adam_update_impl(params, grads, exp_avg, exp_avg_sq, step, n, lr, beta1, beta2, eps, weight_decay, grad_scale, 1, stream);
+}
+
+static int adam_parts_impl(float* params, const float* grads, float* exp_avg, float* exp_avg_sq, int32_t* step, int64_t n,
+                           float lr, float beta1, float beta2, float eps, float weight_decay, float grad_scale,
+                           const float* parts, int64_t part_stride, int n_parts, int64_t enc_floats, int64_t layer_floats,
+                           int64_t covered_per_layer, int step_add, void* stream) {
     GF_CHECK_ARG(params && grads && exp_avg && exp_avg_sq && step && n > 0, "adam_step_parts: bad arguments");
     GF_CHECK_ARG(n_parts >= 1 && n_parts <= ADAM_MAX_EXTRA + 1, "adam_step_parts: n_parts=%d out of [1,%d]", n_parts, ADAM_MAX_EXTRA + 1);
-    if (n_parts == 1) return ganffn_adam_step(params, grads, exp_avg, exp_avg_sq, step, n, lr, beta1, beta2, eps, weight_decay, grad_scale, stream);
+    if (n_parts == 1) {
+        GF_TRY(adam_update_impl(params, grads, exp_avg, exp_avg_sq, step, n, lr, beta1, beta2, eps, weight_decay, grad_scale, step_add, stream));
+        return step_add ? ganffn_adam_bump(step, stream) : 0;
+    }
     GF_CHECK_ARG(parts && aligned16(parts) && (part_stride & 3) == 0 && part_stride >= enc_floats, "adam_step_parts: bad partial slabs");
     GF_CHECK_ARG((n & 3) == 0 && aligned16(params) && aligned16(grads) && aligned16(exp_avg) && aligned16(exp_avg_sq),
                  "adam_step_parts: slabs must be 16-byte aligned and a multiple of 4 floats");
@@ -869,9 +935,23 @@
     hipStream_t st = (hipStream_t)stream;
     hipLaunchKernelGGL(adam_parts_kernel, dim3((unsigned)((n / 4 + 255) / 256)), dim3(256), 0, st, params, grads, exp_avg, exp_avg_sq,
                        (const int32_t*)step, (long)n, lr, beta1, beta2, eps, weight_decay, grad_scale, parts, (long)part_stride,
-                       n_parts - 1, (long)enc_floats, (long)layer_floats, (long)covered_per_layer);
-    GF_LAUNCH_CHECK();
-    return ganffn_adam_bump(step, stream);
+                       n_parts - 1, (long)enc_floats, (long)layer_floats, (long)covered_per_layer, step_add);
+    GF_LAUNCH_CHECK();
+    return step_add ? ganffn_adam_bump(step, stream) : 0;
+}
+extern "C" int ganffn_adam_step_parts(float* params, const float* grads, float* exp_avg, float* exp_avg_sq, int32_t* step, int64_t n,
+                                      float lr, float beta1, float beta2, float eps, float weight_decay, float grad_scale,
+                                      const float* parts, int64_t part_stride, int n_parts, int64_t enc_floats, int64_t layer_floats,
+                                      int64_t covered_per_layer, void* stream) {
+    return adam_parts_impl(params, grads, exp_avg, exp_avg_sq, step, n, lr, beta1, beta2, eps, weight_decay, grad_scale, parts,
+                           part_stride, n_parts, enc_floats, layer_floats, covered_per_layer, 1, stream);
+}
+extern "C" int ganffn_adam_apply(float* params, const float* grads, float* exp_avg, float* exp_avg_sq, int32_t* step, int64_t n,
+                                 float lr, float beta1, float beta2, float eps, float weight_decay, float grad_scale,
+                                 const float* parts, int64_t part_stride, int n_parts, int64_t enc_floats, int64_t layer_floats,
+                                 int64_t covered_per_layer, void* stream) {
+    return adam_parts_impl(params, grads, exp_avg, exp_avg_sq, step, n, lr, beta1, beta2, eps, weight_decay, grad_scale, parts,
+                           part_stride, n_parts < 1 ? 1 : n_parts, enc_floats, layer_floats, covered_per_layer, 0, stream);
 }
 
 extern "C" int ganffn_add3(const float* a, const float* b, const float* c, float* out, int64_t n, void* stream) {
diff --git a/gan_ffn_amd/csrc/gemm.hip b/gan_ffn_amd/csrc/gemm.hip
--- a/gan_ffn_amd/csrc/gemm.hip
+++ b/gan_ffn_amd/csrc/gemm.hip
@@ -37,6 +37,7 @@
     EpiArgs ea;
     float* part = nullptr;
     long part_stride = 0;
+    int tn_store = 0;
 };
 
 template <int BK>
@@ -615,7 +616,10 @@
             for (int b = 0; b < TN; ++b) {
                 const int col = n0 + wn * WN + b * 32 + r;
                 float old[16];
-                if (!slab) {
+                if (!slab && g.tn_store) {
+#pragma unroll
+                    for (int i = 0; i < 16; ++i) old[i] = 0.f;
+                } else if (!slab) {
 #pragma unroll
                     for (int i = 0; i < 16; ++i) {
                         const int row = min(m0 + wm * WM + a * 32 + (i & 3) + 8 * (i >> 2) + 4 * h, g.M - 1);
@@ -642,6 +646,7 @@
                 for (int i = 0; i < NR; ++i) sum += smem[i * BM + tid];
                 if (m0 + tid < g.M) {
                     if (slab) slab[(size_t)g.M * g.N + m0 + tid] = sum;
+                    else if (g.tn_store) g.colsum[m0 + tid] = 0.f + sum;
                     else g.colsum[m0 + tid] += sum;
                 }
             }
@@ -674,6 +679,7 @@
     if (by >= gy0) {
         by -= gy0;
         g.A = s1.A; g.C = s1.C; g.ea.mask_out = s1.mask_out; g.ea.train = s1.train;
+        if constexpr (EPI == EPI_DROP_GELU) { g.ea.aux_out = s1.aux_out; g.ea.rng_add = s1.rng_add; }
     }
     gemm_body<MODE, BM, BN, BK, EPI, WGM, WGN>(g, bx, by, bz);
 }
@@ -928,6 +934,7 @@
     float* part;
     long part_stride;
     int splits;
+    int store;
 };
 
 template <bool SPLIT, int BN = 64>
@@ -943,7 +950,7 @@
     const int bz = local / q.tiles_mn, t2 = local - bz * q.tiles_mn;
     GemmArgs g;
     g.A = q.A; g.lda = q.lda; g.B = q.B; g.ldb = q.ldb; g.C = q.C; g.ldc = q.ldc; g.colsum = q.colsum;
-    g.M = q.M; g.N = q.N; g.K = q.K; g.kchunk = q.kchunk; g.slab_stride = 0;
+    g.M = q.M; g.N = q.N; g.K = q.K; g.kchunk = q.kchunk; g.slab_stride = 0; g.tn_store = grp.store;
     if constexpr (SPLIT) { g.part = grp.part + q.part_off; g.part_stride = grp.part_stride; }
     constexpr int PW = 8;
     const int tiles_m = q.tiles_mn / q.tiles_n;
@@ -979,6 +986,7 @@
     if (g.K == 100 && g.N >= 1024 && splits == 1 && (g.lda & 3) == 0 && (g.ldb & 3) == 0 &&
         (size_t)g.M * g.lda * 4 < (size_t(1) << 31) && (size_t)g.M * g.ldc * 4 < (size_t(1) << 31)) {
         if constexpr (EPI == EPI_RELU_DROP) return launch_wres<MODE_NT, EPI, true>(g, st, &s1);
+        else if constexpr (EPI == EPI_DROP_GELU) return fail(-1, "gemm_nt_pair: no two-segment form of the weight-resident kernel for the head epilogue");
         else return fail(-1, "gemm_nt_pair: no two-segment form of the weight-resident kernel for epilogue %d", EPI);
     }
     if (g.K <= 128) return launch_cfg_pair<MODE_NT, 64, 64, 16, EPI, 2, 2, 1>(g, s1, splits, st);
@@ -1049,7 +1057,9 @@
 
 int launch_gemm_nt_pair(const float* A, int lda, const float* W, int ldw, float* C, int ldc, int M, int N, int K, int epi,
                         const EpiArgs& ea, const GemmSeg1& s1, hipStream_t st, int* splits_io, long slab_stride) {
-    GF_CHECK_ARG(epi == EPI_RELU_DROP || epi == EPI_NONE, "gemm_nt_pair: epilogue %d has no two-segment form", epi);
+    GF_CHECK_ARG(epi == EPI_RELU_DROP || epi == EPI_NONE || epi == EPI_DROP_GELU, "gemm_nt_pair: epilogue %d has no two-segment form", epi);
+    GF_CHECK_ARG(epi != EPI_DROP_GELU || (ea.aux_out && s1.aux_out && gemm_nt_pair_drop_gelu_supported(N, K)),
+                 "gemm_nt_pair: the head epilogue needs both segments' pre-activation outputs and a generic-kernel shape");
     GF_TRY(check_common(A, lda, W, ldw, C, M, N, K));
     GF_CHECK_ARG(s1.A && s1.C && aligned16(s1.A) && ea.aux_in == nullptr, "gemm_nt_pair: bad second segment");
     GF_CHECK_ARG((K & 3) == 0, "gemm_nt: K=%d must be a multiple of 4", K);
@@ -1059,8 +1069,10 @@
     set_split(g, splits, slab_stride);
     if (splits_io) *splits_io = splits;
     if (epi == EPI_RELU_DROP) return launch_pick_pair<EPI_RELU_DROP>(g, s1, 1, st);
+    if (epi == EPI_DROP_GELU) return launch_pick_pair<EPI_DROP_GELU>(g, s1, 1, st);
     return launch_pick_pair<EPI_NONE>(g, s1, splits, st);
 }
+bool gemm_nt_pair_drop_gelu_supported(int N, int K) { return !(K == 100 && N >= 1024); }
 
 int launch_gemm_nn(const float* A, int lda, const float* Bm, int ldb, float* C, int ldc, int M, int N, int K,
                    int epi, const EpiArgs& ea, hipStream_t st, int* splits_io, long slab_stride) {
@@ -1141,7 +1153,7 @@
             v[z] = *reinterpret_cast<const float4*>(part + (size_t)min(z, grp.splits - 1) * grp.part_stride + i4);
         const long row = i4 / q.N, col = i4 - row * q.N;
         float* dst = q.C + row * q.ldc + col;
-        const float4 old = *reinterpret_cast<const float4*>(dst);
+        const float4 old = grp.store ? make_float4(0.f, 0.f, 0.f, 0.f) : *reinterpret_cast<const float4*>(dst);
         float4 s = v[0];
 #pragma unroll
         for (int z = 1; z < TN_GROUP_MAXSPLIT; ++z)
@@ -1152,17 +1164,19 @@
         for (int i = blockIdx.x * 256 + threadIdx.x; i < q.M; i += gridDim.x * 256) {
             float s = part[nC + i];
             for (int z = 1; z < grp.splits; ++z) s += part[(size_t)z * grp.part_stride + nC + i];
-            q.colsum[i] += s;
+            q.colsum[i] = (grp.store ? 0.f : q.colsum[i]) + s;
         }
 }
 
 long gemm_tn_grouped_part_floats() { return (long)(TN_GROUP_TILES + 256) * (64 * 64 + 64) + 4 * MAXP; }
 
 
-int launch_gemm_tn_grouped(const TnDesc* d, int n, hipStream_t st, float* part_ws, long part_floats, TnSlabs* slabs) {
+int launch_gemm_tn_grouped(const TnDesc* d, int n, hipStream_t st, float* part_ws, long part_floats, TnSlabs* slabs, bool store) {
     GF_CHECK_ARG(d && n >= 1 && n <= MAXP, "gemm_tn_grouped: n=%d out of [1,%d]", n, MAXP);
-    if (!mode().tn100_off() && part_ws != nullptr && aligned16(part_ws) && tn100_supported(d, n))
+    if (!mode().tn100_off() && part_ws != nullptr && aligned16(part_ws) && tn100_supported(d, n)) {
+        GF_CHECK_ARG(!store, "gemm_tn_grouped: the d_model-100 kernel has no store mode (its unreduced slabs serve that purpose)");
         return launch_gemm_tn100_grouped(d, n, st, part_ws, part_floats, slabs);
+    }
     GF_CHECK_ARG(slabs == nullptr, "gemm_tn_grouped: unreduced gradient slabs exist only for the d_model-100 kernel");
     TnGroup grp;
     grp.n = n;
@@ -1194,6 +1208,7 @@
         if (splits < 2) splits = 1;
     }
     grp.splits = splits;
+    grp.store = store ? 1 : 0;
     grp.part = splits > 1 ? part_ws : nullptr;
     grp.part_stride = per_split;
     GF_CHECK_ARG(splits == 1 || aligned16(part_ws), "gemm_tn_grouped: partial-slab workspace must be 16-byte aligned");
diff --git a/gan_ffn_amd/engine.py b/gan_ffn_amd/engine.py
--- a/gan_ffn_amd/engine.py
+++ b/gan_ffn_amd/engine.py
@@ -178,6 +178,7 @@
         self.cfg_train = ops.enc_cfg(S, B, E, net.H, net.L, train=True, p_pe=net.p_pe, p_enc=net.p_enc)
         self.cfg_eval = ops.enc_cfg(S, B, E, net.H, net.L, train=False, p_pe=net.p_pe, p_enc=net.p_enc)
         self.pair_ok = ops.encoder_fwd_pair_supported(self.cfg_train)
+        self.store_ok = self.need_bwd and ops.encoder_bwd_store_supported(self.cfg_train)
         n_saved, _ = ops.enc_sizes(self.cfg_train)
         self.hcfg_train = HeadCfg(self.T, E, net.D1, net.D2, net.kind, net.p_head, 1)
         self.hcfg_eval = HeadCfg(self.T, E, net.D1, net.D2, net.kind, net.p_head, 0)
@@ -487,7 +488,7 @@
                          ps.out, ps.hsaved, self.ws, self.rng.state, a1)
         return a0, a1
 
-    def _net_bwd(self, net, ps, d_out, train, adds, want_wgrad, reduce_cb=None, need_dx=None, parts=False):
+    def _net_bwd(self, net, ps, d_out, train, adds, want_wgrad, reduce_cb=None, need_dx=None, parts=False, store=False):
         cfg = ps.cfg_train if train else ps.cfg_eval
         hcfg = ps.hcfg_train if train else ps.hcfg_eval
         a0, a1 = adds
@@ -504,8 +505,10 @@
         if parts and want_wgrad and reduce_cb is None:
             return ops.encoder_bwd_parts_raw(cfg, ps.dx, net.slab, gslab, ps.saved, self.ws, self.rng.state, a0, need_dx)
         if reduce_cb is None or not want_wgrad:
-            ops.encoder_bwd_raw(cfg, 0, net.L, ps.dx, net.slab, gslab, ps.saved, self.ws, self.rng.state, a0, need_dx)
+            ops.encoder_bwd_raw(cfg, 0, net.L, ps.dx, net.slab, gslab, ps.saved, self.ws, self.rng.state, a0, need_dx,
+                                store=store and want_wgrad)
         else:
+            assert not store, "the bucketed backward accumulates layer range by layer range: no store mode"
             bks = net.buckets(self.n_buckets)
             reduce_cb(*bks[0], last=False)
             for i, (lo_f, hi_f) in enumerate(bks[1:]):
@@ -513,7 +516,13 @@
                 ops.encoder_bwd_raw(cfg, lo, hi, ps.dx, net.slab, gslab, ps.saved, self.ws, self.rng.state, a0, need_dx)
                 reduce_cb(lo_f, hi_f, last=(i == len(bks) - 2))
 
-    def _adam(self, net, parts=None):
+    def _adam(self, net, parts=None, folded=False):
+        if folded:
+            has = parts is not None and parts[2] > 1
+            ops.adam_apply_raw(net.slab, net.grad, net.exp_avg, net.exp_avg_sq, net.step, net.total, net.lr, net.betas[0],
+                               net.betas[1], 1e-8, net.wd, 1.0 / self.world, parts[0] if has else None, parts[1] if has else 0,
+                               parts[2] if has else 1, net.enc_floats, net.layer_floats, net.covered)
+            return
         if parts is not None and parts[2] > 1:
             ops.adam_step_parts_raw(net.slab, net.grad, net.exp_avg, net.exp_avg_sq, net.step, net.total, net.lr, net.betas[0],
                                     net.betas[1], parts[0], parts[1], parts[2], net.enc_floats, net.layer_floats, net.covered,
@@ -526,6 +535,13 @@
         return self.pg is None and os.environ.get("GANFFN_ADAM_PARTS", "1") == "1" and net.total % 4 == 0 and \
             ops.encoder_bwd_parts_supported(ps.cfg_train)
 
+    def _store_ok(self, net, ps):
+        return self.pg is None and os.environ.get("GANFFN_WGRAD_STORE", "1") == "1" and ps.store_ok
+
+    def _step_fold(self):
+        return self.pg is None and os.environ.get("GANFFN_STEP_FOLD", "1") == "1" and \
+            os.environ.get("GANFFN_BCE_FUSED", "1") == "1"
+
     def _zero_grad(self, net, parts):
         if parts:
             net.grad[net.enc_floats:].zero_()
@@ -536,12 +552,13 @@
         ops.adam_update_raw(net.slab[lo:hi], net.grad[lo:hi], net.exp_avg[lo:hi], net.exp_avg_sq[lo:hi], net.step, hi - lo,
                             net.lr, net.betas[0], net.betas[1], 1e-8, net.wd, 1.0 / self.world)
 
-    def _make_reducer(self, net):
+    def _make_reducer(self, net, folded=False):
         if self.pg is None:
             def plain(net_key, parts=None):
                 self._pre_write(net_key)
-                self._adam(net, parts)
+                self._adam(net, parts, folded)
             return None, plain
+        assert not folded, "the folded step counter is the single-GPU path's"
         if dp_mode() == "inline":
             import torch.distributed as dist
             group = getattr(self, "_cur_pg", None) or self.pg
@@ -569,6 +586,11 @@
         w = net.w
         w3 = w("fc3.weight") if net.kind == 1 else None
         b3 = w("fc3.bias") if net.kind == 1 else None
+        if net.kind == 0 and os.environ.get("GANFFN_HEAD_PAIR", "1") == "1":
+            ops.head_fwd_pair_raw(ps_train.hcfg_train, ps_eval.enc_out, ps_train.enc_out, w("fc1.weight"), w("fc1.bias"),
+                                  w("fc2.weight"), w("fc2.bias"), ps_eval.out, ps_train.out, ps_eval.hsaved, ps_train.hsaved,
+                                  self.rng.state, self._base_add + adds_eval[1], a1, False, True)
+            return a0, a1
         for hcfg, ps, add in ((ps_eval.hcfg_eval, ps_eval, self._base_add + adds_eval[1]), (ps_train.hcfg_train, ps_train, a1)):
             ops.head_fwd_raw(hcfg, ps.enc_out, w("fc1.weight"), w("fc1.bias"), w("fc2.weight"), w("fc2.bias"), w3, b3,
                              ps.out, ps.hsaved, self.ws, self.rng.state, add)
@@ -600,14 +622,20 @@
         torch.cat((x_real, pg_.out), dim=1, out=self.x_cat)
         adds = self._net_fwd(Dn, pd, self.x_cat, train=True, save=True, adds=(a + 2, a + 3))
         n = S * 2 * B
-        ops._lib.call("ganffn_bce2_fwd", ops._ptr(pd.out), C.c_float(1.0), C.c_float(0.0), 2 * B, B, n, C.c_float(1.0),
-                      ops._ptr(self.losses[loss_slot:loss_slot + 1]), 0, ops._stream())
-        ops._lib.call("ganffn_bce2_bwd", ops._ptr(pd.out), C.c_float(1.0), C.c_float(0.0), 2 * B, B, n, C.c_float(1.0),
-                      ops._ptr(self.dprob2), ops._stream())
+        folded = self._step_fold()
+        if os.environ.get("GANFFN_BCE_FUSED", "1") == "1":
+            ops.bce2_fused_raw(pd.out, 1.0, 0.0, 2 * B, B, n, 1.0, self.losses[loss_slot:loss_slot + 1], False, self.dprob2,
+                               Dn.step if folded else None)
+        else:
+            ops._lib.call("ganffn_bce2_fwd", ops._ptr(pd.out), C.c_float(1.0), C.c_float(0.0), 2 * B, B, n, C.c_float(1.0),
+                          ops._ptr(self.losses[loss_slot:loss_slot + 1]), 0, ops._stream())
+            ops._lib.call("ganffn_bce2_bwd", ops._ptr(pd.out), C.c_float(1.0), C.c_float(0.0), 2 * B, B, n, C.c_float(1.0),
+                          ops._ptr(self.dprob2), ops._stream())
         parts_mode = self._parts_ok(Dn, pd)
-        self._zero_grad(Dn, parts_mode)
-        cb, finish = self._make_reducer(Dn)
-        parts = self._net_bwd(Dn, pd, self.dprob2, True, adds, True, cb, need_dx=Dn.has_obj, parts=parts_mode)
+        store_mode = not parts_mode and self._store_ok(Dn, pd)
+        self._zero_grad(Dn, parts_mode or store_mode)
+        cb, finish = self._make_reducer(Dn, folded)
+        parts = self._net_bwd(Dn, pd, self.dprob2, True, adds, True, cb, need_dx=Dn.has_obj, parts=parts_mode, store=store_mode)
         if Dn.has_obj:
             self.d_real.copy_(pd.dx[:, :B])
             scratch = self.ws[:parts[3]] if (parts is not None and parts[2] > 1) else self.ws
@@ -631,13 +659,19 @@
             g_adds = self.train_gen_forward(who, batch, loss_slot)
         d_adds = self._net_fwd(Dn, pd, pg_.out, train=False, save=True, adds=(a + 2, a + 3))
         n = S * B
-        ops.bce_fwd_raw(pd.out, 1.0, n, 1.0, self.losses[loss_slot:loss_slot + 1], False)
-        ops.bce_bwd_raw(pd.out, 1.0, n, 1.0, self.dprob1)
+        folded = self._step_fold()
+        if os.environ.get("GANFFN_BCE_FUSED", "1") == "1":
+            ops.bce_fused_raw(pd.out, 1.0, n, 1.0, self.losses[loss_slot:loss_slot + 1], False, self.dprob1,
+                              Gn.step if folded else None)
+        else:
+            ops.bce_fwd_raw(pd.out, 1.0, n, 1.0, self.losses[loss_slot:loss_slot + 1], False)
+            ops.bce_bwd_raw(pd.out, 1.0, n, 1.0, self.dprob1)
         self._net_bwd(Dn, pd, self.dprob1, False, d_adds, False)
         parts_mode = self._parts_ok(Gn, pg_)
-        self._zero_grad(Gn, parts_mode)
-        cb, finish = self._make_reducer(Gn)
-        parts = self._net_bwd(Gn, pg_, pd.dx, True, g_adds, True, cb, parts=parts_mode)
+        store_mode = not parts_mode and self._store_ok(Gn, pg_)
+        self._zero_grad(Gn, parts_mode or store_mode)
+        cb, finish = self._make_reducer(Gn, folded)
+        parts = self._net_bwd(Gn, pg_, pd.dx, True, g_adds, True, cb, parts=parts_mode, store=store_mode)
         finish(("G", who), parts)
 
     def _pre_write(self, net_key):
diff --git a/gan_ffn_amd/ops.py b/gan_ffn_amd/ops.py
--- a/gan_ffn_amd/ops.py
+++ b/gan_ffn_amd/ops.py
@@ -128,9 +128,16 @@
               _ptr(saved_train), _ptr(ws), _ptr(rng), C.c_uint64(add_train), _stream())
 
 
-def encoder_bwd_raw(cfg, lo, hi, dx, slab, gslab, saved, ws, rng, add, need_dx_in=True):
+BWD_STORE = 2
+
+
+def encoder_bwd_raw(cfg, lo, hi, dx, slab, gslab, saved, ws, rng, add, need_dx_in=True, store=False):
     _lib.call("ganffn_encoder_bwd2", C.byref(cfg), lo, hi, _ptr(dx), _ptr(slab), _ptr(gslab), _ptr(saved), _ptr(ws),
-              _ptr(rng), C.c_uint64(add), 1 if need_dx_in else 0, _stream())
+              _ptr(rng), C.c_uint64(add), (1 if need_dx_in else 0) | (BWD_STORE if store else 0), _stream())
+
+
+def encoder_bwd_store_supported(cfg):
+    return int(_lib.load().ganffn_encoder_bwd_store_supported(C.byref(cfg))) == 1
 
 
 def encoder_bwd_parts_supported(cfg):
@@ -156,6 +163,12 @@
               _ptr(out), _ptr(saved), _ptr(ws), _ptr(rng), C.c_uint64(add), _stream())
 
 
+def head_fwd_pair_raw(cfg, x0, x1, w1, b1, w2, b2, out0, out1, saved0, saved1, rng, add0, add1, train0, train1):
+    _lib.call("ganffn_head_fwd_pair", C.byref(cfg), _ptr(x0), _ptr(x1), _ptr(w1), _ptr(b1), _ptr(w2), _ptr(b2), _ptr(out0),
+              _ptr(out1), _ptr(saved0), _ptr(saved1), _ptr(rng), C.c_uint64(add0), C.c_uint64(add1), 1 if train0 else 0,
+              1 if train1 else 0, _stream())
+
+
 def head_bwd_raw(cfg, d_out, x, w1, w2, w3, gw1, gb1, gw2, gb2, gw3, gb3, dx, saved, ws, rng, add):
     _lib.call("ganffn_head_bwd", C.byref(cfg), _ptr(d_out), _ptr(x), _ptr(w1), _ptr(w2), _ptr(w3), _ptr(gw1), _ptr(gb1),
               _ptr(gw2), _ptr(gb2), _ptr(gw3), _ptr(gb3), _ptr(dx), _ptr(saved), _ptr(ws), _ptr(rng), C.c_uint64(add),
@@ -178,6 +191,23 @@
 
 def bce_bwd_raw(prob, target, n, scale, dprob):
     _lib.call("ganffn_bce_bwd", _ptr(prob), C.c_float(target), n, C.c_float(scale), _ptr(dprob), _stream())
+
+
+def bce2_fused_raw(prob, target_a, target_b, period, split, n, scale, loss, accumulate, dprob, step_bump=None):
+    _lib.call("ganffn_bce2_fused", _ptr(prob), C.c_float(target_a), C.c_float(target_b), period, split, n, C.c_float(scale),
+              _ptr(loss), 1 if accumulate else 0, _ptr(dprob), _ptr(step_bump), _stream())
+
+
+def bce_fused_raw(prob, target, n, scale, loss, accumulate, dprob, step_bump=None):
+    _lib.call("ganffn_bce_fused", _ptr(prob), C.c_float(target), n, C.c_float(scale), _ptr(loss), 1 if accumulate else 0,
+              _ptr(dprob), _ptr(step_bump), _stream())
+
+
+def adam_apply_raw(p, g, m, v, step, n, lr, b1, b2, eps=1e-8, wd=0.0, gscale=1.0, parts=None, part_stride=0, n_parts=1,
+                   enc_floats=0, layer_floats=0, covered=0):
+    _lib.call("ganffn_adam_apply", _ptr(p), _ptr(g), _ptr(m), _ptr(v), _ptr(step), C.c_int64(n), C.c_float(lr), C.c_float(b1),
+              C.c_float(b2), C.c_float(eps), C.c_float(wd), C.c_float(gscale), _ptr(parts), C.c_int64(part_stride), n_parts,
+              C.c_int64(enc_floats), C.c_int64(layer_floats), C.c_int64(covered), _stream())
 
 
 def adam_step_raw(p, g, m, v, step, n, lr, b1, b2, eps=1e-8, wd=0.0, gscale=1.0):
diff --git a/include/ganffn.h b/include/ganffn.h
--- a/include/ganffn.h
+++ b/include/ganffn.h
@@ -62,6 +62,9 @@
                         const float* params, float* grads, const float* saved, float* workspace,
                         const uint64_t* rng, uint64_t rng_offset_add, int need_dx_in, void* stream);
 
+#define GANFFN_BWD_STORE 2
+int ganffn_encoder_bwd_store_supported(const ganffn_enc_cfg* cfg);
+
 int ganffn_encoder_bwd_parts_supported(const ganffn_enc_cfg* cfg);
 int64_t ganffn_encoder_bwd_parts_covered(int E, int F);
 int ganffn_encoder_bwd_parts(const ganffn_enc_cfg* cfg, float* dx, const float* params, float* grads, const float* saved,
@@ -72,6 +75,9 @@
                     const float* w2, const float* b2, const float* w3, const float* b3, float* out,
                     float* saved, float* workspace, const uint64_t* rng, uint64_t rng_offset_add,
                     void* stream);
+int ganffn_head_fwd_pair(const ganffn_head_cfg* cfg, const float* x0, const float* x1, const float* w1, const float* b1,
+                         const float* w2, const float* b2, float* out0, float* out1, float* saved0, float* saved1,
+                         const uint64_t* rng, uint64_t add0, uint64_t add1, int train0, int train1, void* stream);
 int ganffn_head_bwd(const ganffn_head_cfg* cfg, const float* d_out, const float* x,
                     const float* w1, const float* w2, const float* w3, float* gw1, float* gb1,
                     float* gw2, float* gb2, float* gw3, float* gb3, float* dx, const float* saved,
@@ -90,6 +96,11 @@
                     float scale, float* loss_out, int accumulate, void* stream);
 int ganffn_bce2_bwd(const float* prob, float target_a, float target_b, int period, int split, int n,
                     float scale, float* dprob, void* stream);
+
+int ganffn_bce2_fused(const float* prob, float target_a, float target_b, int period, int split, int n,
+                      float scale, float* loss_out, int accumulate, float* dprob, int32_t* step_bump, void* stream);
+int ganffn_bce_fused(const float* prob, float target, int n, float scale, float* loss_out, int accumulate,
+                     float* dprob, int32_t* step_bump, void* stream);
 
 int ganffn_adam_step(float* params, const float* grads, float* exp_avg, float* exp_avg_sq,
                      int32_t* step, int64_t n, float lr, float beta1, float beta2, float eps,
@@ -102,6 +113,10 @@
                        const int32_t* step, int64_t n, float lr, float beta1, float beta2, float eps,
                        float weight_decay, float grad_scale, void* stream);
 int ganffn_adam_bump(int32_t* step, void* stream);
+int ganffn_adam_apply(float* params, const float* grads, float* exp_avg, float* exp_avg_sq, int32_t* step, int64_t n,
+                      float lr, float beta1, float beta2, float eps, float weight_decay, float grad_scale,
+                      const float* parts, int64_t part_stride, int n_parts, int64_t enc_floats, int64_t layer_floats,
+                      int64_t covered_per_layer, void* stream);
 
 int ganffn_add3(const float* a, const float* b, const float* c, float* out, int64_t n, void* stream);
 int ganffn_logsoftmax_nll(const float* logits, const int64_t* labels, const float* umask,
```

Measured after the change: 53440 utterances/s, median of 6. Within noise of the previous version (+0.4%).
